# do-mpc/do-mpc

Measured on AMD Instinct MI355X. Metric: MPC steps/sec (make_step wall-time), industrial_poly robust multi-stage, higher is better.
Workload: dtype f64

## Files before the change

__graft_entry__.py:

```python
import os
import subprocess
import sys

ROOT = os.path.dirname(os.path.abspath(__file__))
if ROOT not in sys.path:
    sys.path.insert(0, ROOT)

PREBUILT = [
    ("oscillating_masses", {}),
    ("batch_reactor", {}),
    ("batch_reactor", {"n_horizon": 50}),
    ("CSTR", {}),
    ("CSTR", {"n_robust": 0, "collocation_deg": 3}),
    ("CSTR", {"track_sign": -3000.0}),
    ("industrial_poly", {}),
    ("industrial_poly", {"n_robust": 2, "uncertainty": "paired"}),
    ("industrial_poly", {"collocation_deg": 3, "collocation_ni": 2, "n_horizon": 6}),
    ("kinematic_bicycle", {}),
    ("dynamic_bicycle", {}),
    ("kite", {"n_horizon": 20}),
    ("rotating_masses", {}),
    ("CSTR", {"custom_rterm": "default_as_expression"}),
    ("CSTR", {"custom_rterm": "custom"}),
    ("oscillating_masses", {"custom_rterm": "custom"}),
    ("oscillating_masses_dae", {}),
    ("dip", {}),
    ("CSTR", {"n_robust": 0, "nl_cons_check_colloc_points": True}),
    ("dip", {"n_horizon": 40, "nl_cons_check_colloc_points": True}),
    ("CSTR", {"nl_cons_single_slack": True}),
    ("CSTR", {"nl_cons_single_slack": True, "n_robust": 2, "n_horizon": 8, "uncertainty": {"alpha": [1.0, 1.05, 0.95], "beta": [1.0]}}),
    ("CSTR", {"nl_cons_single_slack": True, "n_robust": 0, "nl_cons_check_colloc_points": True}),
    ("CSTR", {"open_loop": True, "uncertainty": {"alpha": [1.0, 1.05, 0.95], "beta": [1.0]}}),
    ("CSTR", {"open_loop": True, "n_robust": 2, "n_horizon": 6, "uncertainty": {"alpha": [1.0, 1.05], "beta": [1.0]}, "soft_T_R": False}),
    ("shape_family:s1", {}), ("shape_family:s2", {}), ("shape_family:s3", {}), ("shape_family:s4", {}), ("shape_family:s5", {}),
    ("shape_family:s6", {}), ("shape_family:s7", {}), ("shape_family:s8", {}), ("shape_family:s9", {}),
]

PREBUILT_BATCH = [
    ("industrial_poly", {}), ("industrial_poly", {"n_robust": 2, "uncertainty": "paired"}),
    ("oscillating_masses", {}), ("CSTR", {}), ("CSTR", {"n_robust": 0, "collocation_deg": 3}), ("batch_reactor", {}), ("batch_reactor", {"n_horizon": 50}),
    ("rotating_masses", {}),
]
PREBUILT_BATCH_MHE = [("rotating_masses", "build_mhe", {}, {}), ("rotating_masses", "build_mhe_w", {"process_noise": True}, {}),
                      ("rotating_masses", "build_mhe_w", {"process_noise": True}, {"scaling": "MHE_W_SCALING"})]


PREBUILT_DEFS = [("CSTR", {}, "DOMPC_FORCE_DENSE=1"), ("batch_reactor", {}, "DOMPC_FORCE_DENSE=1"),
                 ("CSTR", {}, "DOMPC_GJ_U=1e9"), ("industrial_poly", {}, "DOMPC_GJ_U=1e9"),
                 ("batch_reactor", {}, "DOMPC_REG_GJ=0"), ("batch_reactor", {}, "DOMPC_GJ_U=1e9"),
                 ("industrial_poly", {}, "DOMPC_QUAD=0"), ("CSTR", {}, "DOMPC_QUAD=0"), ("CSTR", {"n_horizon": 5, "n_robust": 0}, "DOMPC_QUAD=0")]


PREBUILT_SHARD = [
    ("CSTR", {}),
    ("industrial_poly", {"n_robust": 2, "uncertainty": "paired"}),
]


PREBUILT_MHE = [("rotating_masses", "build_mhe", {}, {}), ("rotating_masses", "build_mhe_w", {"process_noise": True}, {}),
                ("rotating_masses", "build_mhe_w", {"process_noise": True}, {"scaling": "MHE_W_SCALING"}),
                ("rotating_masses", "build_mhe", {"dae": True}, {}), ("rotating_masses", "build_mhe_w", {"process_noise": True, "dae": True}, {}),
                ("oscillating_masses", "build_mhe", {"estimation": True}, {}), ("oscillating_masses", "build_mhe", {"estimation": True, "dae": True}, {}),
                ("rotating_masses", "build_mhe_w", {"process_noise": True}, {"soft_limit": (-0.1, 0.01)}),
                ("rotating_masses", "build_mhe_w", {"process_noise": True}, {"soft_limit": (-0.1, 0.01), "nl_cons_single_slack": True}),
                ("rotating_masses", "build_mhe_w", {"process_noise": True, "input_meas_noise": False}, {})]


PREBUILT_ROUTE = [("oscillating_masses", "docstring", False, False), ("oscillating_masses", "tree", False, False),
                  ("industrial_poly", "tree", False, True), ("CSTR", "tree", False, True), ("batch_reactor", "tree", False, False),
                  ("oscillating_masses_dae", "tree", False, False), ("rotating_masses", "tree", False, False),
                  ("CSTR", "docstring", False, False), ("batch_reactor", "docstring", False, False), ("industrial_poly", "docstring", False, False),
                  ("oscillating_masses", None, True, False), ("CSTR", None, True, False), ("CSTR", "tree", True, False),
                  ("industrial_poly", None, True, False), ("industrial_poly", "tree", True, False), ("batch_reactor", None, True, False),
                  ("rotating_masses", None, True, False)]


def lowered_route_cases():
    from do_mpc_amd import controller
    from do_mpc_amd.examples import CASES
    tests = os.path.join(ROOT, "tests")
    if tests not in sys.path:
        sys.path.insert(0, tests)
    import route_cases as rc
    out = []
    orig = controller.HipIpmSolver
    controller.HipIpmSolver = _NoSolver
    try:
        for name, cost, rows, batch in PREBUILT_ROUTE:
            ex = CASES[name]
            mpc = rc.stopped_before_setup(lambda n: ex.build_mpc(ex.build_model()), name)
            mpc.prepare_nlp()
            if rows:
                rc.rows_at_three_nodes(mpc, name)
            if cost:
                rc.ADDED_COST[cost](mpc)
            mpc.create_nlp()
            out.append((f"{name} + {cost or ''}{' + rows' if rows else ''} (low-level route)", {}, mpc.generated_header, mpc.model_hash, batch))
    finally:
        controller.HipIpmSolver = orig
    return out


PREBUILT_PLANTS = ["oscillating_masses", "batch_reactor", "CSTR", "industrial_poly", "oscillating_masses_dae", "dip", "rotating_masses",
                   "triple_tank", "batch_reactor_lqr_dae", "batch_reactor_lqr_dae:build_dae_model"]
# ... 108 lines not shown
class _NoSolver:

    def __init__(self, *a, **k):
        pass


def lowered_models(which=None):
    from do_mpc_amd import controller
    from do_mpc_amd.examples import CASES
    out = []
    orig = controller.HipIpmSolver
    controller.HipIpmSolver = _NoSolver
    try:
        for name, kw in (PREBUILT if which is None else which):
            ex = CASES[name]
            mpc = ex.build_mpc(ex.build_model(), **kw)
            out.append((name, kw, mpc.generated_header, mpc.model_hash))
        if which is None:
            out += _lower_mhe(PREBUILT_MHE)
    finally:
        controller.HipIpmSolver = orig
    return out


def _lower_mhe(entries):
    from do_mpc_amd.examples import CASES
    out = []
    for name, builder, mkw, bkw in entries:
        ex = CASES[name]
        bkw = {k: (getattr(ex, v) if isinstance(v, str) else v) for k, v in bkw.items()}
        mhe = getattr(ex, builder)(ex.build_model(**mkw), **bkw)
        out.append((f"{name} ({builder})", {**mkw, **{k: "..." for k in bkw}}, mhe._mpc.generated_header, mhe._mpc.model_hash))
    return out


def lowered_mhe(entries):
    from do_mpc_amd import controller
    orig = controller.HipIpmSolver
    controller.HipIpmSolver = _NoSolver
    try:
        return _lower_mhe(entries)
    finally:
        controller.HipIpmSolver = orig


def build() -> None:
    from do_mpc_amd import build as nb
    import do_mpc_amd
    from concurrent.futures import ThreadPoolExecutor
    lib = nb.runtime_library()
    print("[build] runtime:", lib)
    jobs = [(name, kw, header, h, False, False) for name, kw, header, h in lowered_models()]
    jobs += [(name, kw, header, h, True, False) for name, kw, header, h in lowered_models(PREBUILT_SHARD)]
    jobs += [(name, kw, header, h, False, True) for name, kw, header, h in lowered_models(PREBUILT_BATCH)]
    jobs += [(name, kw, header, h, False, True) for name, kw, header, h in lowered_mhe(PREBUILT_BATCH_MHE)]
    route = lowered_route_cases()
    jobs += [(name, kw, header, h, False, False) for name, kw, header, h, _ in route]
    jobs += [(name, kw, header, h, False, True) for name, kw, header, h, batch in route if batch]
    with ThreadPoolExecutor(max_workers=max(1, min(len(jobs), (os.cpu_count() or 2) - 1))) as pool:
        outs = list(pool.map(lambda j: nb.model_code_object(j[2], j[3], shard=j[4], batch_only=j[5]), jobs))
    for (name, kw, _, _, shard, batch), co in zip(jobs, outs):
        print(f"[build] {name} {kw}{' (tree sharding)' if shard else ''}{' (batch only)' if batch else ''}: {co}")
    for name, kw, defs in PREBUILT_DEFS:
        saved = os.environ.get("DOMPC_DEFS")
        os.environ["DOMPC_DEFS"] = defs
        try:
            for _, _, header, h in lowered_models([(name, kw)]):
                print(f"[build] {name} {kw} [{defs}]: {nb.model_code_object(header, h)}")
        finally:
            if saved is None:
                del os.environ["DOMPC_DEFS"]
            else:
                os.environ["DOMPC_DEFS"] = saved
    from do_mpc_amd.examples import CASES
    from do_mpc_amd.simulator import Simulator
    for name in PREBUILT_PLANTS:
        case, _, builder = name.partition(":")
        hdr = Simulator(getattr(CASES[case], builder or "build_model")())._lower()
        co = nb.plant_code_object(hdr, hdr.rsplit('PLANT_MODEL_HASH "', 1)[1].split('"')[0])
        print(f"[build] plant {name}: {co}")
    failed = []
    for entry in PREBUILT_EKF:
        try:
            for name, kw, hdr, h in lowered_ekf([entry]):
                print(f"[build] filter {name} {kw}: {nb.ekf_code_object(hdr, h)}")
        except Exception as e:
            failed.append(entry)
            print(f"[build] filter {entry[0]} {entry[1]}: FAILED\n{e}")
    for entry in PREBUILT_EKF_DAE:
        try:
            for name, hdr, h in lowered_ekf_dae([entry]):
                print(f"[build] filter of a model with algebraic states '{name}': {nb.ekf_code_object(hdr, h)}")
        except Exception as e:
            failed.append(entry)
            print(f"[build] filter of a model with algebraic states '{entry}': FAILED\n{e}")
    failed_lqr = []
    for entry in PREBUILT_LQR:
        try:
            for label, hdr, h in lowered_lqr([entry]):
                print(f"[build] LQR design {label}: {nb.lqr_code_object(hdr, h)}")
        except Exception as e:
            failed_lqr.append(entry)
            print(f"[build] LQR design {entry}: FAILED\n{e}")
    failed_ampc = []
    for entry in PREBUILT_AMPC:
        try:
            for label, hdr, h in lowered_ampc([entry]):
                print(f"[build] approximate MPC network {label}: {nb.ampc_code_object(hdr, h)}")
        except Exception as e:
            failed_ampc.append(entry)
            print(f"[build] approximate MPC network {entry}: FAILED\n{e}")
    failed_asmpc = []
    for entry in PREBUILT_ASMPC:
        try:
            for label, hdr, h in lowered_asmpc([entry]):
                print(f"[build] sensitivity-based MPC law {label}: {nb.asmpc_code_object(hdr, h)}")
        except Exception as e:
            failed_asmpc.append(entry)
            print(f"[build] sensitivity-based MPC law {entry}: FAILED\n{e}")
    mk = os.path.join(ROOT, "oracle", "Makefile")
    if os.path.exists(mk):
        subprocess.run(["make", "-C", os.path.join(ROOT, "oracle")], check=True)
    if failed:
        raise RuntimeError(f"extended Kalman filter code objects that could not be built: {failed}")
    if failed_lqr:
        raise RuntimeError(f"LQR design code objects that could not be built: {failed_lqr}")
# ... 74 lines not shown
```

do_mpc_amd/csrc/dompc_device.hip:

```cpp
#ifndef DOMPC_HOST_EMU
#include <hip/hip_runtime.h>
#define DOMPC_CONSTANT_TABLES 1
#define DOMPC_FN __device__ static inline
#define DOMPC_CONST __device__ static constexpr
#define DOMPC_DEV __device__
#define DOMPC_HD __host__ __device__
#else
#include <stdlib.h>
#define DOMPC_FN static inline
#define DOMPC_CONST static const
#define DOMPC_DEV
#define DOMPC_HD
#endif

#ifndef DOMPC_LB
#define DOMPC_LB 2
#endif
#ifndef DOMPC_SRC_DIGEST
#define DOMPC_SRC_DIGEST 0ULL
#endif

#include DOMPC_MODEL_HEADER
#include "dompc_kernel.h"

namespace dompc {
DOMPC_HD inline void model_info(const int32_t* in, int64_t* out) {
  WsLayout L = ws_layout(in[0], in[1], in[2], in[3], in[4]);
  out[0] = NX; out[1] = NU; out[2] = NP; out[3] = NTVP; out[4] = NE; out[5] = NSE;
  out[6] = DEG; out[7] = NI; out[8] = M;
  out[9] = L.total;
  out[10] = SWEEP_BLOCK;
  out[11] = (int64_t)sizeof(KArgs);
  out[12] = RED_MAX; out[13] = ASM_N; out[14] = CUT1; out[15] = CUT2;
  out[16] = DOMPC_SHARD;
  out[17] = EL_SIZE;
  out[19] = QUAD_EDGE ? 4 : 1;
  out[18] = (int64_t)DOMPC_SRC_DIGEST;
#ifndef DOMPC_HOST_EMU
  out[20] = r16::ENABLED ? 1 : 0;
#else
  out[20] = 0;
#endif
}
}

#ifndef DOMPC_HOST_EMU
extern "C" __global__ void dompc_model_info_kernel(const int32_t* in, int64_t* out, char* hash) {
  if (threadIdx.x == 0 && blockIdx.x == 0) {
    dompc::model_info(in, out);
    const char h[] = DOMPC_MODEL_HASH;
    for (int i = 0; i < (int)sizeof(h); ++i) hash[i] = h[i];
  }
}

#ifndef DOMPC_MAXBLOCK
#define DOMPC_MAXBLOCK 256
#endif
extern "C" __global__ void __launch_bounds__(DOMPC_BLOCK_CONST ? DOMPC_BLOCK_CONST : DOMPC_MAXBLOCK, DOMPC_LB) dompc_solve_kernel(dompc::KArgs A) {
  using namespace dompc;
  const int POOL = A.pool_doubles;
  if (threadIdx.x < 32) lds_prof[threadIdx.x] = 0;
  if (threadIdx.x < 8) lds_flags[threadIdx.x] = 0;
  for (int i = threadIdx.x; i < POOL; i += DOMPC_BDIM) lds_pool[i] = (i >= A.lds_fill_lo && i < A.lds_fill_hi) ? A.lds_fill : 0.0;
  for (int i = threadIdx.x; i < 2 * MAX_FILTER; i += DOMPC_BDIM) lds_filt[i] = 0.0;
  __syncthreads();
  const bool wide = dompc::WIDE_OK && (A.mode == 0 && A.wide > 1);
  const int slot = slot_of_block(A);
  if (wide && slot >= A.batch) return;
  Thr T = make_thr(A);
  T.kp = (const void*)__builtin_amdgcn_kernarg_segment_ptr();
  if (wide && A.mode != 1) dompc::xcd_census(T);
  if (A.mode == 1) {
    const int bq = __builtin_amdgcn_readfirstlane((int)blockIdx.x);
    const int sq = slot_of_block(A);
    if (bq < A.batch) dompc::debug_newton(T, A, bq, sq);
    return;
  }
  bool first = true;
  while (true) {
    int b;
    if (wide) {
      if (!first) break;
      b = slot;
    } else {
      if (threadIdx.x == 0) lds_b = atomicAdd(A.work_counter, 1);
      __syncthreads();
      b = lds_b;
      __syncthreads();
      if (b >= A.batch) break;
    }
    first = false;
    if (A.mode == 2) dompc::sweep_problem(T, A, b, slot);
    else dompc::solve_problem(T, A, b, slot);
  }
}
// ... 65 lines not shown
```

do_mpc_amd/csrc/dompc_driver.h:

```cpp

DOMPC_DEV inline int epsg_off(const KArgs& A) { return A.node_eps_off[0]; }
DOMPC_DEV inline int epsg_n(const KArgs& A) { return A.n_opt_x - A.node_eps_off[0]; }
DOMPC_DEV inline void epsg_grad(const Thr& T, const Prob& Q) {
  const KArgs& A = *Q.A;
  const int o = epsg_off(A), nv = epsg_n(A);
  for (int j = T.tid; j < nv; j += T.nt) {
    double g = 0.0, r = 0.0;
    for (int e = 0; e < A.n_edges; ++e) {
      const int q = j - (A.node_eps_off[A.edge_parent[e]] - o);
      if (q < 0 || q >= NSE) continue;
      g += Q.sf * DOMPC_EPS_PEN[q];
      const double* yd = Q.lam + A.edge_row0[e] + NW + NX;
      for (int i = 0; i < NE; ++i)
        if (nl_slack(i) == q) r -= yd[i] * Q.sgn[e * NE1 + i];
    }
    Q.gf[o + j] = g;
    Q.rd[o + j] = g + r - Q.zl[o + j] + Q.zu[o + j];
  }
  T.sync();
}
DOMPC_DEV inline double epsg_rowsum(const Prob& Q, int j, const double* v, const double* v0) {
  const KArgs& A = *Q.A;
  const int o = epsg_off(A);
  double t = 0.0;
// ... 8 lines not shown
}
DOMPC_DEV inline void epsg_residual(const Thr& T, const Prob& Q, const double* v, int j1) {
  const KArgs& A = *Q.A;
  const int o = epsg_off(A);
  for (int e = T.tid; e < A.n_edges; e += T.nt) {
    const int jo = A.node_eps_off[A.edge_parent[e]] - o;
    const int r0 = A.edge_row0[e] + NW + NX;
    for (int i = 0; i < NE; ++i) {
      const int q = nl_slack(i);
      if (q < 0) continue;
      const double ve = v ? v[jo + q] : ((jo + q == j1) ? 1.0 : 0.0);
      Q.c[r0 + i] = Q.ct[r0 + i] - ve * Q.sgn[e * NE1 + i];
    }
  }
  T.sync();
}

DOMPC_DEV inline void solve_problem(const Thr& T, const KArgs& A, int b, int slot0) {
  const dompc_options& O = A.opt;
  int slot = slot0;
  Prob Q = make_prob(A, slot, A.p + (int64_t)b * A.n_opt_p);
  const double* x0 = A.x0 + (int64_t)b * A.n_opt_x;
  const int nX = A.n_opt_x, nSl = A.n_edges * NE;
  int status = 2, it = 0, n_reg = 0, n_ls_fail = 0, n_sweeps = 0, n_trials = 0, n_soc = 0;

  double cnt[2] = {0.0, 0.0};
  bool singular0;
  {
    double fr[1] = {0.0};
    for (int d = T.tid; d < A.n_dummy; d += T.nt) {
      const int g = A.dummy_idx[d];
      if (!(A.lbx[g] > -INFINITY) && !(A.ubx[g] < INFINITY)) fr[0] += 1.0;
    }
    const int ops[1] = {R_SUM};
    wg_reduce(T, fr, ops);
    singular0 = fr[0] > 0.0;
  }
  for (int g = T.tid; g < nX; g += T.nt) {
    double l = A.lbx[g], u = A.ubx[g];
    if (l > -INFINITY) l -= fmin(O.constr_viol_tol, O.bound_relax_factor * fmax(1.0, fabs(l)));
    if (u < INFINITY) u += fmin(O.constr_viol_tol, O.bound_relax_factor * fmax(1.0, fabs(u)));
    double xv = x0[g];
    const bool hl = l > -INFINITY, hu = u < INFINITY;
    double pl = hl ? O.bound_push * fmax(1.0, fabs(l)) : 0.0;
    double pu = hu ? O.bound_push * fmax(1.0, fabs(u)) : 0.0;
    if (hl && hu) { pl = fmin(pl, O.bound_frac * (u - l)); pu = fmin(pu, O.bound_frac * (u - l)); }
    if (hl) xv = fmax(xv, l + pl);
    if (hu) xv = fmin(xv, u - pu);
    Q.lb_own[g] = l; Q.ub_own[g] = u; Q.x[g] = xv;
    Q.zl[g] = hl ? 1.0 : 0.0; Q.zu[g] = hu ? 1.0 : 0.0;
    if (sh_cnt(A, mk_x(A, g))) cnt[0] += (hl ? 1.0 : 0.0) + (hu ? 1.0 : 0.0);
  }
  for (int r = T.tid; r < A.n_g; r += T.nt) Q.lam[r] = 0.0;
  T.sync();
  for (int d = T.tid; d < A.n_dummy; d += T.nt) {
    const int g = A.dummy_idx[d];
    if (singular0) continue;
    if (sh_cnt(A, mk_x(A, g))) cnt[0] -= (Q.lb_own[g] > -INFINITY ? 1.0 : 0.0) + (Q.ub_own[g] < INFINITY ? 1.0 : 0.0);
    Q.x[g] = fmin(fmax(x0[g], A.lbx[g]), A.ubx[g]);
    Q.lb_own[g] = -INFINITY; Q.ub_own[g] = INFINITY; Q.zl[g] = 0.0; Q.zu[g] = 0.0;
  }
  T.sync();
  if (A.lb_sh) {
    for (int g = T.tid; g < nX; g += T.nt) { A.lb_sh[g] = Q.lb_own[g]; A.ub_sh[g] = Q.ub_own[g]; }
    T.sync();
  }
  auto init_slacks = [&](bool rescale) {
    for (int e = T.tid; e < A.n_edges; e += T.nt) {
      for (int i = 0; i < NE; ++i) { Q.s[e * NE1 + i] = 0.0; if (!rescale) Q.sgn[e * NE1 + i] = 1.0; }
      if (DENSE_EDGE) dae_edge_f(Q, e, Q.x, Q.s, Q.ct); else eval_edge_f(Q, e, Q.x, Q.s, Q.ct);
      for (int i = 0; i < NE; ++i) {
        const int row = A.edge_row0[e] + NW + NX + i, si = e * NE1 + i;
        double l = A.lbg[row], u = A.ubg[row];
        if (l > -INFINITY) l -= fmin(O.constr_viol_tol, O.bound_relax_factor * fmax(1.0, fabs(l)));
        if (u < INFINITY) u += fmin(O.constr_viol_tol, O.bound_relax_factor * fmax(1.0, fabs(u)));
        l *= Q.sgn[si]; u *= Q.sgn[si];
        const bool hl = l > -INFINITY, hu = u < INFINITY;
        double pl = hl ? O.bound_push * fmax(1.0, fabs(l)) : 0.0;
        double pu = hu ? O.bound_push * fmax(1.0, fabs(u)) : 0.0;
        if (hl && hu) { pl = fmin(pl, O.bound_frac * (u - l)); pu = fmin(pu, O.bound_frac * (u - l)); }
        double sv = Q.ct[row];
        if (hl) sv = fmax(sv, l + pl);
        if (hu) sv = fmin(sv, u - pu);
        Q.s[si] = sv; Q.sl[si] = l; Q.su[si] = u;
        Q.zsl[si] = hl ? 1.0 : 0.0; Q.zsu[si] = hu ? 1.0 : 0.0;
        if (!rescale && sh_cnt(A, mk_e(A, e))) cnt[1] += (hl ? 1.0 : 0.0) + (hu ? 1.0 : 0.0);
      }
    }
    T.sync();
  };
  if (NE > 0) init_slacks(false);
  {
    const int ops[2] = {R_SUM, R_SUM};
    wg_reduce(T, cnt, ops);
  }
  const double n_bounds = cnt[0] + cnt[1];
  const double n_dual = (double)(A.n_g - DOMPC_XROW_MASKED) + n_bounds;

  double mu = O.mu_init;
  Q.sf = 1.0;
  long long c_sweep = 0, c_bwd = 0, c_fwd = 0, c_ls = 0, c_meas = 0, c_ftb = 0, c_acc = 0, c_t = 0; const long long c_start = prof_clock();
  unsigned g_sweep = 0, g_bwd = 0, g_fwd = 0, g_ls = 0, g_meas = 0, g_ftb = 0, g_acc = 0, g_t = 0; const unsigned g_start = T.gen;
  if (T.tid == 0) T.fset(6, abort_requested(A));
  auto delta_after = [&](double last) { return last == 0.0 ? O.delta_w_0 : fmax(O.delta_w_min, O.kappa_w_minus * last); };
  const bool ls_init = (NE == 0 || (!EPS_GLOBAL && !FREE_ROOT)) && O.constr_mult_init_max > 0.0;
  auto ls_slacks = [&]() {
// ... 157 lines not shown
    bad = run_sweep(T, Q, b, slot, mu, 0, singular0 ? delta_after(0.0) : 0.0);
    ++n_sweeps;
  }
  const double mu_min = fmin(O.tol, O.compl_inf_tol * Q.sf) / (O.kappa_eps + 1.0);
  double tau = fmax(O.tau_min, 1.0 - mu);
  if (KAPPA_D != 0.0) Q.mu = mu;
  Errs E = measure(T, Q, nullptr);
  const double theta0 = E.theta;
  const double theta_max = 1e4 * fmax(1.0, theta0), theta_min = 1e-4 * fmax(1.0, theta0);
  double bar_sum;
  {
    double bs[1] = {0.0};
    LogAcc La{1.0, 0, 0};
    double lin = 0.0;
    double x_[DOMPC_FW], l_[DOMPC_FW], u2_[DOMPC_FW];
#define L_(u, g) x_[u] = Q.x[g]; l_[u] = Q.lb[g]; u2_[u] = Q.ub[g];
#define B_(u, g)                                                       \
    if (sh_cnt(A, mk_x(A, g))) {                                       \
      if (l_[u] > -INFINITY) logacc_add(La, x_[u] - l_[u]);            \
      if (u2_[u] < INFINITY) logacc_add(La, u2_[u] - x_[u]);           \
      if (KAPPA_D != 0.0) { const double os_ = one_sided(l_[u], u2_[u]); lin += os_ > 0.0 ? x_[u] - l_[u] : (os_ < 0.0 ? u2_[u] - x_[u] : 0.0); } \
    }
    DOMPC_FOR4(nX, L_, B_)
#undef L_
#undef B_
    for (int g = T.tid; g < nSl; g += T.nt) {
      if (!sh_cnt(A, mk_e(A, g / NE1))) continue;
      const int si = (g / NE1) * NE1 + g % NE1;
      if (Q.sl[si] > -INFINITY) logacc_add(La, Q.s[si] - Q.sl[si]);
      if (Q.su[si] < INFINITY) logacc_add(La, Q.su[si] - Q.s[si]);
      if (KAPPA_D != 0.0) { const double os_ = one_sided(Q.sl[si], Q.su[si]); lin += os_ > 0.0 ? Q.s[si] - Q.sl[si] : (os_ < 0.0 ? Q.su[si] - Q.s[si] : 0.0); }
    }
    bs[0] = -logacc_value(La);
    if (KAPPA_D != 0.0) bs[0] += KAPPA_D * lin;
    const int ops[1] = {R_SUM};
    wg_reduce(T, bs, ops);
    bar_sum = bs[0];
  }
  int n_filt = 0;
  double delta_last = 0.0;
  int acc_count = 0;
  const double s_max = 100.0;
  double E0 = 0.0;
  int wd_count = 0, wd_iter = 0, n_watchdog = 0;
  bool in_wd = false, wd_resume = false;
  double wd_theta = 0.0, wd_phi = 0.0, wd_dphi = 0.0, wd_alpha = 0.0, wd_amax = 0.0, wd_az = 0.0, wd_delta = 0.0, wd_delta_last = 0.0, wd_bar = 0.0;
  Errs wd_E = E;
  double delta = 0.0, a_max = 1.0, a_z = 1.0, dphi = 0.0;
  for (int g = T.tid; g < nX; g += T.nt) { Q.xt[g] = Q.x[g]; Q.zlt[g] = Q.zl[g]; Q.zut[g] = Q.zu[g]; }
  for (int g = T.tid; g < A.n_g; g += T.nt) Q.lamt[g] = Q.lam[g];
  for (int g = T.tid; g < nSl; g += T.nt) { Q.st[g] = Q.s[g]; Q.zslt[g] = Q.zsl[g]; Q.zsut[g] = Q.zsu[g]; }
  T.sync();
  Comp Cp{-INFINITY, INFINITY, 0.0};

  while (true) {
    bool skip_first = false;
    if (wd_resume) {
      for (int g = T.tid; g < nX; g += T.nt) { Q.x[g] = Q.x_wd[g]; Q.zl[g] = Q.zl_wd[g]; Q.zu[g] = Q.zu_wd[g]; Q.dx[g] = Q.dx_sv[g]; }
      for (int g = T.tid; g < A.n_g; g += T.nt) { Q.lam[g] = Q.lam_wd[g]; Q.dlam[g] = Q.dlam_sv[g]; }
      for (int g = T.tid; g < nSl; g += T.nt) { Q.s[g] = Q.s_wd[g]; Q.zsl[g] = Q.zsl_wd[g]; Q.zsu[g] = Q.zsu_wd[g]; Q.ds[g] = Q.ds_sv[g]; }
      T.sync();
      E = wd_E; bar_sum = wd_bar; delta = wd_delta; delta_last = wd_delta_last; a_max = wd_amax; a_z = wd_az; dphi = wd_dphi;
      wd_resume = false;
      skip_first = true;
    } else {
    if (bad) { if (in_wd) { bad = 0; wd_resume = true; in_wd = false; wd_count = 0; continue; } status = 3; break; }
    if (T.fget(6)) { status = 6; break; }
    if (((WIDE_OK && T.nwg > 1) || sh_on(A)) && T.fget(7)) { status = 5; break; }
    const double sd = fmax(s_max, (E.sum_y + E.C.sum_z) / fmax(1.0, n_dual)) / s_max;
    const double sc = fmax(s_max, E.C.sum_z / fmax(1.0, n_bounds)) / s_max;
    const double e_c0 = comp_err(E.C, 0.0);
    E0 = fmax(E.e_d / sd, fmax(E.e_p, e_c0 / sc));
    if (!(E0 == E0) || !(E.obj == E.obj)) { if (in_wd) { wd_resume = true; in_wd = false; wd_count = 0; continue; } status = 4; break; }
    if (E0 <= O.tol && E.e_d <= O.dual_inf_tol && E.e_p <= O.constr_viol_tol && e_c0 <= O.compl_inf_tol) {
      status = 0; break;
    }
    if (E0 <= O.acceptable_tol) {
      if (++acc_count >= O.acceptable_iter) { status = 1; break; }
    } else acc_count = 0;
    if (it >= O.max_iter) { status = 2; break; }

    const double mu_before = mu;
    while (true) {
      const double Emu = fmax(E.e_d / sd, fmax(E.e_p, comp_err(E.C, mu) / sc));
      if (Emu <= O.kappa_eps * mu && mu > mu_min) {
        mu = fmax(mu_min, fmin(O.kappa_mu * mu, pow(mu, O.theta_mu)));
        tau = fmax(O.tau_min, 1.0 - mu);
        n_filt = 0;
        in_wd = false; wd_count = 0;
      } else break;
    }
    if (mu != mu_before) {
      if (QUAD_FWD && forward_adjoint(Q, mu) && !Q.lu_ok) {
        ++n_sweeps;
        if (run_sweep(T, Q, b, slot, mu, 4, Q.dsw)) { if (in_wd) { wd_resume = true; in_wd = false; wd_count = 0; continue; } status = 3; break; }
      } else {
        refresh_mu(T, Q, mu - mu_before);
        Q.rp_mu = mu;
      }
    }

    delta = 0.0;
    bool first_try = true, dir_ok = true, recs_dirty = false;
    while (true) {
      c_t = prof_clock(); g_t = T.gen;
      int fail = (singular0 && delta == 0.0) ? 1 : run_backward(T, Q, b, slot, mu, delta);
      if (EPS_GLOBAL && !fail) {
        run_forward(T, Q, b, slot, mu, delta);
        fail = epsg_build(delta);
        recs_dirty = true;
      }
      c_bwd += prof_clock() - c_t; g_bwd += T.gen - g_t;
      if (!fail) break;
      if (delta == 0.0) {
        delta = delta_after(delta_last);
      } else {
        delta *= (delta_last == 0.0 && first_try) ? O.kappa_w_plus_bar : O.kappa_w_plus;
        first_try = false;
        if (delta > O.delta_w_max) { dir_ok = false; break; }
      }
      if ((NW > 0 && delta != Q.dsw) || (EPS_GLOBAL && recs_dirty)) {
        ++n_sweeps;
        if (run_sweep(T, Q, b, slot, mu, 0, delta)) { dir_ok = false; break; }
        recs_dirty = false;
      }
    }
    if (!dir_ok) { if (in_wd) { wd_resume = true; in_wd = false; wd_count = 0; continue; } status = 3; break; }
    if (delta > 0.0) { delta_last = delta; ++n_reg; }
    c_t = prof_clock(); g_t = T.gen;
    if (EPS_GLOBAL) { if (epsg_apply(delta, Q.dlam_e)) { if (in_wd) { wd_resume = true; in_wd = false; wd_count = 0; continue; } status = 3; break; } }
    else run_forward(T, Q, b, slot, mu, delta);
    c_fwd += prof_clock() - c_t; g_fwd += T.gen - g_t;

    c_t = prof_clock(); g_t = T.gen;
    double r5[5];
    run_step_rules(T, Q, b, slot, mu, r5);
    a_max = (r5[0] > tau) ? tau / r5[0] : 1.0; dphi = r5[2];
    a_z = (r5[1] > tau) ? tau / r5[1] : 1.0;
    c_ftb += prof_clock() - c_t; g_ftb += T.gen - g_t;
    }
    auto step_rules = [&](double (&r5)[5]) { run_step_rules(T, Q, b, slot, mu, r5); };
    const double theta = E.theta;
    const double phi = E.obj + mu * bar_sum;

    c_t = prof_clock(); g_t = T.gen;
    const double gamma_theta = 1e-5, gamma_phi = 1e-8, eta_phi = 1e-8, s_theta = 1.1, s_phi = 2.3, gamma_alpha = 0.05;
    const double kappa_soc = 0.99;
    double a_min;
    if (dphi < 0.0 && theta <= theta_min)
      a_min = (theta > 0.0) ? gamma_alpha * fmin(gamma_theta, fmin(gamma_phi * theta / (-dphi),
                                                                    pow(theta, s_theta) / pow(-dphi, s_phi)))
                            : gamma_alpha * gamma_theta;
    else if (dphi < 0.0) a_min = gamma_alpha * fmin(gamma_theta, gamma_phi * theta / (-dphi));
    else a_min = gamma_alpha * gamma_theta;
    a_min = fmax(a_min, 1e-14);
    auto eval_trial = [&](double al, double az, double& obj_o, double& th_o, double& bar_o) {
      run_eval_trial(T, Q, b, slot, al, az, mu, obj_o, th_o, bar_o, Cp);
      ++n_trials;
    };
    auto acceptable_ref = [&](double th_, double ph_, double al, bool& armijo_case, double theta, double phi, double dphi) -> bool {
      armijo_case = false;
      bool ok = (ph_ == ph_) && (th_ == th_) && fabs(ph_) < INFINITY && th_ <= theta_max;
      if (ok) {
        for (int q = 0; q < n_filt; ++q)
          if (th_ >= T.filt[2 * q] && ph_ >= T.filt[2 * q + 1]) { ok = false; break; }
      }
      if (ok) {
        const bool switching = dphi < 0.0 && al * pow(-dphi, s_phi) > pow(theta, s_theta);
        const double eps_m = 10.0 * 2.220446049250313e-16 * fabs(phi);
        if (theta <= theta_min && switching) {
          armijo_case = true;
          ok = (ph_ - phi - eps_m <= eta_phi * al * dphi);
        } else {
          ok = (th_ <= (1.0 - gamma_theta) * theta) || (ph_ - phi - eps_m <= -gamma_phi * theta);
        }
      }
      return ok;
    };
    auto acceptable = [&](double th_, double ph_, double al, bool& armijo_case) -> bool { return acceptable_ref(th_, ph_, al, armijo_case, theta, phi, dphi); };
    auto soc_residual = [&](double al) {
      double c_[DOMPC_FW], ct_[DOMPC_FW];
#define L_(u, g) c_[u] = Q.c[g]; ct_[u] = Q.ct[g];
#define B_(u, g) if (mk_g(A, g)) Q.c[g] = al * c_[u] + ct_[u];
      DOMPC_FOR4(A.n_g, L_, B_)
#undef L_
#undef B_
      T.sync();
    };
    auto keep_direction = [&](bool restore) {
      for (int g = T.tid; g < nX; g += T.nt) { if (restore) Q.dx[g] = Q.dx_sv[g]; else Q.dx_sv[g] = Q.dx[g]; }
      for (int g = T.tid; g < A.n_g; g += T.nt) { if (restore) Q.dlam[g] = Q.dlam_sv[g]; else Q.dlam_sv[g] = Q.dlam[g]; }
      for (int g = T.tid; g < nSl; g += T.nt) { if (restore) Q.ds[g] = Q.ds_sv[g]; else Q.ds_sv[g] = Q.ds[g]; }
      T.sync();
    };
    double alpha = skip_first ? 0.5 * a_max : a_max;
    bool accepted = false, armijo_used = false, stale = false;
    double th_t = 0.0, obj_t = 0.0, bar_t = bar_sum;
    int n_ls = skip_first ? 1 : 0;
    bool wd_done = false, wd_augment_ref = false, wd_no_augment = false;
    if (O.watchdog_shortened_iter_trigger > 0 && !in_wd && !skip_first && wd_count >= O.watchdog_shortened_iter_trigger) {
      in_wd = true; wd_iter = 0; ++n_watchdog;
      for (int g = T.tid; g < nX; g += T.nt) { Q.x_wd[g] = Q.x[g]; Q.zl_wd[g] = Q.zl[g]; Q.zu_wd[g] = Q.zu[g]; Q.dx_sv[g] = Q.dx[g]; }
      for (int g = T.tid; g < A.n_g; g += T.nt) { Q.lam_wd[g] = Q.lam[g]; Q.dlam_sv[g] = Q.dlam[g]; }
      for (int g = T.tid; g < nSl; g += T.nt) { Q.s_wd[g] = Q.s[g]; Q.zsl_wd[g] = Q.zsl[g]; Q.zsu_wd[g] = Q.zsu[g]; Q.ds_sv[g] = Q.ds[g]; }
      T.sync();
      wd_E = E; wd_bar = bar_sum; wd_delta = delta; wd_delta_last = delta_last; wd_amax = a_max; wd_az = a_z;
      wd_theta = theta; wd_phi = phi; wd_dphi = dphi; wd_alpha = a_max;
    }
    if (in_wd) {
      eval_trial(alpha, a_z, obj_t, th_t, bar_t);
// ... 34 lines not shown
          double obj_s = 0.0, th_s = 0.0, bar_s = 0.0;
          eval_trial(a_s, az_s, obj_s, th_s, bar_s);
          bool arm_s = false;
          if (acceptable(th_s, obj_s + mu * bar_s, a_s, arm_s)) {
            accepted = true; armijo_used = arm_s; soc_ok = true;
            alpha = a_s;
            a_z = az_s;
            obj_t = obj_s; th_t = th_s; bar_t = bar_s;
            break;
          }
          if (!(th_s <= kappa_soc * th_old)) break;
          th_old = th_s;
          soc_residual(a_s);
        }
        if (soc_ok) break;
        keep_direction(true);
        stale = true;
      }
      if (!(alpha * 0.5 >= a_min)) break;
      alpha *= 0.5;
      ++n_ls;
    }
    if (bad) { if (in_wd) { bad = 0; wd_resume = true; in_wd = false; wd_count = 0; continue; } status = 3; break; }
    if (!accepted && stale) eval_trial(alpha, a_z, obj_t, th_t, bar_t);
    if (!wd_done) wd_count = n_ls > 0 ? wd_count + 1 : 0;
    if (!accepted) {
      ++n_ls_fail;
      n_filt = 0;
    } else if (!armijo_used && !wd_no_augment) {
      if (T.ltid == 0) {
        int q = n_filt < MAX_FILTER ? n_filt : MAX_FILTER - 1;
        T.filt[2 * q] = (1.0 - gamma_theta) * (wd_augment_ref ? wd_theta : theta);
        T.filt[2 * q + 1] = (wd_augment_ref ? wd_phi : phi) - gamma_phi * (wd_augment_ref ? wd_theta : theta);
      }
      if (n_filt < MAX_FILTER) ++n_filt;
      T.lsync();
    }
    bar_sum = bar_t;
    c_ls += prof_clock() - c_t; g_ls += T.gen - g_t;
    c_t = prof_clock(); g_t = T.gen;
    prob_flip(Q); slot = Q.slot;
    if (A.trace && b == 0 && T.tid == 0 && it < A.trace_cap) {
      double* tr = A.trace + 8 * it;
      tr[0] = it; tr[1] = mu; tr[2] = E0; tr[3] = E.e_p; tr[4] = E.e_d; tr[5] = accepted ? alpha : -alpha;
      tr[6] = delta; tr[7] = E.obj / Q.sf;
    }
    if (T.tid == 0) T.fset(6, abort_requested(A));
    c_acc += prof_clock() - c_t; g_acc += T.gen - g_t;
    ++it;
    c_t = prof_clock(); g_t = T.gen; bad = run_sweep(T, Q, b, slot, mu, 0, singular0 ? delta_after(delta_last) : 0.0); c_sweep += prof_clock() - c_t; g_sweep += T.gen - g_t;
    ++n_sweeps;
    if (EPS_GLOBAL) epsg_grad(T, Q);
    if (KAPPA_D != 0.0) Q.mu = mu;
    c_t = prof_clock(); g_t = T.gen; E = measure(T, Q, &Cp); c_meas += prof_clock() - c_t; g_meas += T.gen - g_t;
  }

  if (slot & SLOT_PARITY) {
    for (int g = T.tid; g < nX; g += T.nt) { Q.xt[g] = Q.x[g]; Q.zlt[g] = Q.zl[g]; Q.zut[g] = Q.zu[g]; }
    for (int g = T.tid; g < A.n_g; g += T.nt) Q.lamt[g] = Q.lam[g];
    for (int g = T.tid; g < nSl; g += T.nt) { Q.st[g] = Q.s[g]; Q.zslt[g] = Q.zsl[g]; Q.zsut[g] = Q.zsu[g]; }
    T.sync();
    prob_flip(Q); slot = Q.slot;
  }
  if (A.trace && b == 0 && T.tid == 0 && A.trace_cap > 8) { double* tr = A.trace + 8 * (A.trace_cap - 1); tr[0] = (double)c_sweep; tr[1] = (double)c_bwd; tr[2] = (double)c_fwd; tr[3] = (double)c_ls; tr[4] = (double)c_meas; tr[5] = (double)(prof_clock() - c_start); tr[6] = (double)c_ftb; tr[7] = (double)c_acc; if (T.prof) { double* t2 = A.trace + 8 * (A.trace_cap - 2); for (int i = 0; i < 8; ++i) t2[i] = (double)T.prof[i]; double* t3 = A.trace + 8 * (A.trace_cap - 3); for (int i = 0; i < 8; ++i) t3[i] = (double)T.prof[8 + i]; double* t4 = A.trace + 8 * (A.trace_cap - 4); for (int i = 0; i < 8; ++i) t4[i] = (double)T.prof[16 + i]; if (A.trace_cap > 12) { double* t5 = A.trace + 8 * (A.trace_cap - 5); for (int i = 0; i < 8; ++i) t5[i] = (double)T.prof[24 + i]; double* t6 = A.trace + 8 * (A.trace_cap - 6); t6[0] = g_sweep; t6[1] = g_bwd; t6[2] = g_fwd; t6[3] = g_ls; t6[4] = g_meas; t6[5] = T.gen - g_start; t6[6] = g_ftb; t6[7] = g_acc; } } }
  const double isf = 1.0 / Q.sf;
  if (A.x_out) for (int g = T.tid; g < nX; g += T.nt) A.x_out[(int64_t)b * nX + g] = sh_cnt(A, mk_x(A, g)) ? Q.x[g] : 0.0;
  if (A.lam_x_out) for (int g = T.tid; g < nX; g += T.nt) A.lam_x_out[(int64_t)b * nX + g] = sh_cnt(A, mk_x(A, g)) ? (Q.zu[g] - Q.zl[g]) * isf : 0.0;
  if (A.lam_g_out) for (int r = T.tid; r < A.n_g; r += T.nt) A.lam_g_out[(int64_t)b * A.n_g + r] = sh_cnt(A, mk_g(A, r)) ? Q.lam[r] * isf : 0.0;
  if (A.lam_g_out && NE > 0) {
    T.sync();
    for (int g = T.tid; g < nSl; g += T.nt) {
      const int e = g / NE1, i = g % NE1;
      if (!sh_cnt(A, mk_e(A, e))) continue;
      const int row = A.edge_row0[e] + NW + NX + i;
      A.lam_g_out[(int64_t)b * A.n_g + row] = Q.lam[row] * Q.sgn[e * NE1 + i] * isf;
    }
  }
  if (A.g_out) {
    for (int r = T.tid; r < A.n_g; r += T.nt) A.g_out[(int64_t)b * A.n_g + r] = sh_cnt(A, mk_g(A, r)) ? Q.c[r] : 0.0;
    T.sync();
    for (int g = T.tid; g < nSl; g += T.nt) {
      const int e = g / NE1, i = g % NE1;
      if (!sh_cnt(A, mk_e(A, e))) continue;
      const int row = A.edge_row0[e] + NW + NX + i;
      A.g_out[(int64_t)b * A.n_g + row] = (Q.c[row] + Q.s[e * NE1 + i]) / Q.sgn[e * NE1 + i];
    }
  }
  if (T.tid == 0) {
    if (A.f_out) A.f_out[b] = E.obj * isf;
    if (A.stats) {
      dompc_stats& S = A.stats[b];
      S.success = (status == 0 || status == 1) ? 1 : 0;
      S.status = status; S.iter_count = it; S.n_reg = n_reg; S.n_ls_fail = n_ls_fail; S.n_sweeps = n_sweeps; S.n_trials = n_trials; S.n_soc = n_soc; S.n_watchdog = n_watchdog; S.reserved0 = 0;
      S.mu = mu; S.obj = E.obj * isf; S.inf_pr = E.e_p; S.inf_du = E.e_d; S.inf_compl = comp_err(E.C, 0.0);
      S.obj_scaling = Q.sf; S.t_wall_total = 0.0;
    }
  }
  T.sync();
}

DOMPC_DEV inline void newton_slack_setup(const Thr& T, const KArgs& A, Prob& Q, int at_solution, double mu, bool reduce, double tol) {
  const dompc_options& O = A.opt;
  if (NE > 0) {
    for (int e = T.tid; e < A.n_edges; e += T.nt) {
      for (int i = 0; i < NE; ++i) { Q.s[e * NE1 + i] = 0.0; Q.sgn[e * NE1 + i] = 1.0; }
      if (DENSE_EDGE) dae_edge_f(Q, e, Q.x, Q.s, Q.ct); else eval_edge_f(Q, e, Q.x, Q.s, Q.ct);
      for (int i = 0; i < NE; ++i) {
        const int row = A.edge_row0[e] + NW + NX + i, si = e * NE1 + i;
        double l = A.lbg[row], u = A.ubg[row];
        double sv = Q.ct[row];
        if (reduce && l != u) {
          const bool act = fabs(sv - l) <= tol || fabs(sv - u) <= tol;
          l = act ? sv : -INFINITY;
          u = act ? sv : INFINITY;
        }
        const bool hl = l > -INFINITY, hu = u < INFINITY;
        double pl = hl ? O.bound_push * fmax(1.0, fabs(l)) : 0.0;
        double pu = hu ? O.bound_push * fmax(1.0, fabs(u)) : 0.0;
        if (hl && hu) { pl = fmin(pl, O.bound_frac * (u - l)); pu = fmin(pu, O.bound_frac * (u - l)); }
        if (at_solution) {
          const double lr = hl ? l - fmin(O.constr_viol_tol, O.bound_relax_factor * fmax(1.0, fabs(l))) : l;
          const double ur = hu ? u + fmin(O.constr_viol_tol, O.bound_relax_factor * fmax(1.0, fabs(u))) : u;
          const double tiny = 1e-12 * fmax(1.0, fabs(sv));
          if (hl) sv = fmax(sv, lr + tiny);
          if (hu) sv = fmin(sv, ur - tiny);
          Q.s[si] = sv; Q.sl[si] = lr; Q.su[si] = ur;
          Q.zsl[si] = hl ? mu / (sv - lr) : 0.0; Q.zsu[si] = hu ? mu / (ur - sv) : 0.0;
          continue;
        }
        if (hl) sv = fmax(sv, l + pl);
        if (hu) sv = fmin(sv, u - pu);
        Q.s[si] = sv; Q.sl[si] = l; Q.su[si] = u;
        Q.zsl[si] = hl ? 1.0 : 0.0; Q.zsu[si] = hu ? 1.0 : 0.0;
      }
    }
    T.sync();
  }
}

DOMPC_DEV inline void debug_newton(const Thr& T, const KArgs& A, int b = 0, int slot = 0) {
  Prob Q = make_prob(A, slot, A.p + (int64_t)b * A.n_opt_p);
  const int nX = A.n_opt_x;
  for (int g = T.tid; g < nX; g += T.nt) {
    Q.x[g] = A.x0[g]; Q.lb[g] = A.lbx[g]; Q.ub[g] = A.ubx[g];
    Q.zl[g] = A.dbg_zl[g]; Q.zu[g] = A.dbg_zu[g];
  }
  for (int r = T.tid; r < A.n_g; r += T.nt) Q.lam[r] = A.dbg_lam[r];
  T.sync();
  newton_slack_setup(T, A, Q, A.dbg_at_solution, A.dbg_mu, false, 0.0);
  Q.sf = 1.0;
  run_sweep(T, Q, b, slot, A.dbg_mu, 0, A.dbg_delta);
  const int fail = run_backward(T, Q, b, slot, A.dbg_mu, A.dbg_delta);
  run_forward(T, Q, b, slot, A.dbg_mu, A.dbg_delta);
  for (int g = T.tid; g < nX; g += T.nt) {
    A.dbg_dx[(int64_t)b * nX + g] = fail ? NAN : Q.dx[g];
    A.dbg_rd[(int64_t)b * nX + g] = Q.rd[g];
  }
  for (int r = T.tid; r < A.n_g; r += T.nt) {
    A.dbg_dlam[(int64_t)b * A.n_g + r] = Q.dlam[r];
    A.dbg_c[(int64_t)b * A.n_g + r] = Q.c[r];
  }
  T.sync();
}

enum { SENS_REDUCE = 1 };
DOMPC_DEV inline void sens_newton(const Thr& T, const KArgs& A, int b, int slot) {
  const dompc_options& O = A.opt;
  const int q = b / A.sn_R, r = b % A.sn_R;
  Prob Q = make_prob(A, slot, A.p + (int64_t)b * A.n_opt_p);
  const int nX = A.n_opt_x;
  const double* xin = A.sn_x + (int64_t)q * nX;
  const double* lin = A.sn_lam + (int64_t)q * A.n_g;
  const double mu = A.sn_mu[q];
  const bool reduce = (A.sn_flags & SENS_REDUCE) != 0;
  const double tol = A.sn_tol;
  double bad[1] = {(mu > 0.0 && mu < INFINITY) ? 0.0 : 1.0};
  for (int g = T.tid; g < nX; g += T.nt) {
    const double xv = xin[g], l0 = A.lbx[g], u0 = A.ubx[g];
    const bool hl = l0 > -INFINITY, hu = u0 < INFINITY;
    double lr = hl ? l0 - fmin(O.constr_viol_tol, O.bound_relax_factor * fmax(1.0, fabs(l0))) : l0;
    double ur = hu ? u0 + fmin(O.constr_viol_tol, O.bound_relax_factor * fmax(1.0, fabs(u0))) : u0;
    const double dl = hl ? xv - lr : 1.0, du = hu ? ur - xv : 1.0;
    if (!(dl > 0.0) || !(du > 0.0)) bad[0] = 1.0;
    double zl = hl ? mu / dl : 0.0, zu = hu ? mu / du : 0.0;
    if (reduce) {
      const bool lo = fabs(xv - l0) <= tol, up = fabs(xv - u0) <= tol;
      if (!lo && !up) { zl = 0.0; zu = 0.0; lr = -INFINITY; ur = INFINITY; }
      if (lo) zl = fmax(zl, 1e3);
      if (up) zu = fmax(zu, 1e3);
    }
    Q.x[g] = xv; Q.lb[g] = lr; Q.ub[g] = ur; Q.zl[g] = zl; Q.zu[g] = zu;
  }
  for (int i = T.tid; i < A.n_g; i += T.nt) Q.lam[i] = lin[i];
  {
    const int ops[1] = {R_MAX};
    wg_reduce(T, bad, ops);
  }
  T.sync();
  double* D = A.sn_D + (int64_t)b * A.sn_nsel;
  int fail = bad[0] != 0.0;
  if (!fail) {
    newton_slack_setup(T, A, Q, 1, mu, reduce, tol);
    Q.sf = 1.0;
    run_sweep(T, Q, b, slot, mu, 0, 0.0);
    fail = run_backward(T, Q, b, slot, mu, 0.0);
    run_forward(T, Q, b, slot, mu, 0.0);
  }
  for (int i = T.tid; i < A.sn_nsel; i += T.nt) {
    const double v = fail ? NAN : Q.dx[A.sn_sel[i]];
    D[i] = v;
    if (!(fabs(v) < INFINITY)) A.sn_ok[q] = 0;
  }
  if (fail && T.tid == 0) A.sn_ok[q] = 0;
  if (r == 0) {
    double m[1] = {0.0};
    if (!fail) {
      for (int g = T.tid; g < nX; g += T.nt) Q.dx_sv[g] = 1.0;
      T.sync();
      for (int i = T.tid; i < A.n_dummy; i += T.nt) Q.dx_sv[A.dummy_idx[i]] = 0.0;
      T.sync();
      for (int g = T.tid; g < nX; g += T.nt) if (Q.dx_sv[g] != 0.0) m[0] = fmax(m[0], fabs(Q.dx[g]));
    }
    const int ops[1] = {R_MAX};
    wg_reduce(T, m, ops);
    if (T.tid == 0) A.sn_res[q] = fail ? NAN : m[0];
  }
  T.sync();
}

DOMPC_HD inline double sens_step(int lin, double fd_step, double pj) { return (lin ? 1.0 : fd_step) * fmax(1.0, fabs(pj)); }
DOMPC_DEV inline void sens_prep_item(const KArgs& A, int64_t it) {
  const int np = A.n_opt_p;
  const int64_t b = it / np;
  const int k = (int)(it % np), q = (int)(b / A.sn_R), r = (int)(b % A.sn_R);
  double v = A.sn_p[(int64_t)q * np + k];
  const int j = A.sn_rows[2 * r], kind = A.sn_rows[2 * r + 1];
  if (kind != 0 && j == k) {
    const double h = sens_step(kind == 1, A.sn_fd_step, v);
    v = kind < 0 ? v - h : v + h;
  }
  A.sn_prow[it] = v;
  if (k == 0 && r == 0) A.sn_ok[q] = 1;
}
DOMPC_DEV inline void sens_finish_item(const KArgs& A, int64_t it) {
  const int nc = A.sn_ncols, ns = A.sn_nsel;
  const int c = (int)(it % nc), i = (int)((it / nc) % ns), q = (int)(it / ((int64_t)nc * ns));
  const int j = A.sn_cols[3 * c], ip = A.sn_cols[3 * c + 1], im = A.sn_cols[3 * c + 2];
  const double* D = A.sn_D + (int64_t)q * A.sn_R * ns;
  const double h = sens_step(im < 0, A.sn_fd_step, A.sn_p[(int64_t)q * A.n_opt_p + j]);
  const double v = im < 0 ? (D[(int64_t)ip * ns + i] - D[i]) / h : (D[(int64_t)ip * ns + i] - D[(int64_t)im * ns + i]) / (2.0 * h);
  A.sn_S[it] = A.sn_ok[q] ? v : NAN;
}

constexpr int SWEEP_BLOCK = NX * NA + NX + NA * NA + NA;

DOMPC_DEV inline void sweep_problem(const Thr& T, const KArgs& A, int b, int slot) {
  Prob Q = make_prob(A, slot, A.p + (int64_t)b * A.n_opt_p);
  const int nX = A.n_opt_x;
  const double* xin = A.sw_x + (int64_t)b * nX;
  const double* lin = A.sw_lam + (int64_t)b * A.n_g;
  for (int g = T.tid; g < nX; g += T.nt) {
    Q.x[g] = xin[g]; Q.lb[g] = -INFINITY; Q.ub[g] = INFINITY; Q.zl[g] = 0.0; Q.zu[g] = 0.0;
  }
  for (int r = T.tid; r < A.n_g; r += T.nt) Q.lam[r] = lin[r];
  for (int g = T.tid; g < A.n_edges * NE; g += T.nt) {
    const int si = (g / NE1) * NE1 + g % NE1;
    Q.s[si] = 0.0; Q.sl[si] = -INFINITY; Q.su[si] = INFINITY; Q.zsl[si] = 0.0; Q.zsu[si] = 0.0; Q.sgn[si] = 1.0;
  }
  T.sync();
  Q.sf = 1.0;
  run_sweep(T, Q, b, slot, 0.0);
  double* gout = A.sw_g + (int64_t)b * A.n_g;
  for (int r = T.tid; r < A.n_g; r += T.nt) gout[r] = Q.c[r];
  double* bl = A.sw_blocks + (int64_t)b * A.n_edges * SWEEP_BLOCK;
  for (int it = T.tid; A.sw_blocks && it < A.n_edges * SWEEP_BLOCK; it += T.nt) {
    const int e = it / SWEEP_BLOCK, i = it % SWEEP_BLOCK;
    const double* S_ = Q.ES(e);
    double v;
    if (i < NX * NA) v = S_[ES_AB + i];
    else if (i < NX * NA + NX) v = S_[ES_CV + i - NX * NA];
    else if (i < NX * NA + NX + NA * NA) v = S_[ES_QT + symi((i - NX * NA - NX) / NA, (i - NX * NA - NX) % NA, NA)];
    else v = S_[ES_QV + i - NX * NA - NX - NA * NA];
    bl[it] = v;
  }
  T.sync();
}
```

do_mpc_amd/csrc/dompc_edge.h:

```cpp

template <bool SPLIT>
DOMPC_DEV inline double eval_edge_f_t(const Prob& Q, int e, const double* xv, const double* sv, double* cv, int part) {
  constexpr int REST = NI * DEG;
  const KArgs& A = *Q.A;
  const int n = A.edge_parent[e], cn = A.edge_child[e], k = A.edge_level[e];
  const double* xn = xv + A.node_x_off[n];
  const double* un = xv + A.node_u_off[n];
  const double* xc = xv + A.node_x_off[cn];
  const double* w = xv + A.edge_w_off[e];
  const double* pp = Q.P + A.p_off_p + A.edge_pidx[e] * NP;
  const double* tvp = Q.P + A.p_off_tvp + k * NTVP;
  const int row0 = A.edge_row0[e];
  const double om = A.edge_omega[e] * Q.sf;
  double f[NX];
  if (M == 0) {
    dompc_dyn_f(xn, un, nullptr, tvp, pp, f);
    double rl[NX];
    for (int a = 0; a < NX; ++a) rl[a] = f[a] - xc[a];
    for (int a = 0; a < NX; ++a) cv[row0 + a] = rl[a];
  } else {
    (void)REST;
    for (int i = 0; i < NI; ++i) {
      const double* xi0 = (i == 0) ? xn : w + slot_of(i, 0) * NX;
      const int rb = row0 + i * (DEG + 1) * NX;
      for (int j = 1; j <= DEG; ++j) {
        if (SPLIT && part != i * DEG + (j - 1)) continue;
        const double* xij = w + slot_of(i, j) * NX;
        dompc_dyn_f(xij, un, nullptr, tvp, pp, f);
        double rl[NX];
#pragma unroll
        for (int a = 0; a < NX; ++a) {
          double xp = DOMPC_C[0 * (DEG + 1) + j] * xi0[a];
          for (int r = 1; r <= DEG; ++r) xp += DOMPC_C[r * (DEG + 1) + j] * w[slot_of(i, r) * NX + a];
          rl[a] = f[a] - xp;
        }
#pragma unroll
        for (int a = 0; a < NX; ++a) cv[rb + (j - 1) * NX + a] = rl[a];
      }
      if (SPLIT && part != REST) continue;
      const double* xnext = w + next_slot(i) * NX;
      double rl[NX];
#pragma unroll
      for (int a = 0; a < NX; ++a) {
        double xf = DOMPC_D[0] * xi0[a];
        for (int r = 1; r <= DEG; ++r) xf += DOMPC_D[r] * w[slot_of(i, r) * NX + a];
        rl[a] = xnext[a] - xf;
      }
#pragma unroll
      for (int a = 0; a < NX; ++a) cv[rb + DEG * NX + a] = rl[a];
    }
    if (SPLIT && part != REST) return 0.0;
    double rl[NX];
#pragma unroll
    for (int a = 0; a < NX; ++a) rl[a] = w[(M - 1) * NX + a] - xc[a];
#pragma unroll
    for (int a = 0; a < NX; ++a) cv[row0 + NW + a] = rl[a];
  }
  double obj = om * lterm_f_e(Q, e, xn, un, nullptr, tvp, pp);
  if (k == A.N - 1) obj += om * mterm_f_e(Q, e, xc, Q.P + A.p_off_tvp + (k + 1) * NTVP, pp);
  if (RT_CUSTOM) obj += edge_rterm_f(Q, e, xv);
  if (NE > 0) {
    double d[NE1];
    nlcons_f_e(Q, e, xn, un, nullptr, tvp, pp, d);
    const double* eps = (NSE > 0) ? xv + A.node_eps_off[n] : nullptr;
    for (int i = 0; i < NE; ++i) {
      if (nl_slack(i) >= 0) d[i] -= eps[nl_slack(i)];
      d[i] *= Q.sgn[e * NE1 + i];
      cv[row0 + NW + NX + i] = d[i] - sv[e * NE1 + i];
    }
    for (int q = 0; q < NSE; ++q) obj += Q.sf * DOMPC_EPS_PEN[q] * eps[q];
  }
  return obj;
}
DOMPC_PHASE double eval_edge_f(const Prob& Q, int e, const double* xv, const double* sv, double* cv) { return eval_edge_f_t<false>(Q, e, xv, sv, cv, -1); }

DOMPC_DEV inline const double* uprev_ptr(const Prob& Q, int n, const double* xv, double* tmp) {
  const KArgs& A = *Q.A;
  const int pn = A.node_parent[n];
  if (pn >= 0) return xv + A.node_u_off[pn];
  for (int i = 0; i < NU; ++i) tmp[i] = Q.P[A.p_off_uprev + i] / DOMPC_SU[i];
  return tmp;
}
DOMPC_DEV inline double node_rweight(const Prob& Q, int n) {
  const KArgs& A = *Q.A;
  const int cc = A.node_child_count[n];
  return cc > 0 ? cc * A.edge_omega[A.node_child_start[n]] * Q.sf : 0.0;
}
DOMPC_DEV inline double node_rterm_f(const Prob& Q, int n, const double* xv) {
  const KArgs& A = *Q.A;
  if (RT_CUSTOM) return 0.0;
  if (A.node_u_off[n] < 0) return 0.0;
  double tmp[NU];
  const double* up = uprev_ptr(Q, n, xv, tmp);
  const double* u = xv + A.node_u_off[n];
  const double rw = node_rweight(Q, n);
  double v = 0.0;
  for (int i = 0; i < NU; ++i) v += rw * DOMPC_RTERM[i] * (u[i] - up[i]) * (u[i] - up[i]);
  return v;
}

DOMPC_DEV inline double edge_rterm_f(const Prob& Q, int e, const double* xv) {
  const KArgs& A = *Q.A;
  const int n = A.edge_parent[e];
  double tmp[NU > 0 ? NU : 1];
  const double* up = uprev_ptr(Q, n, xv, tmp);
  return A.edge_omega[e] * Q.sf * dompc_rterm_f(xv + A.node_x_off[n], xv + A.node_u_off[n], up, Q.P + A.p_off_tvp + A.edge_level[e] * NTVP,
                                                Q.P + A.p_off_p + A.edge_pidx[e] * NP);
}
DOMPC_DEV inline void edge_rterm_eval(const Prob& Q, int e, ldsd* dst) {
  const KArgs& A = *Q.A;
  const int n = A.edge_parent[e];
  const double om = A.edge_omega[e] * Q.sf, omh = (Q.soc & 2) ? 0.0 : om;
  double tmp[NU > 0 ? NU : 1], out[RT_LEN > 0 ? RT_LEN : 1];
  const double* up = uprev_ptr(Q, n, Q.x, tmp);
  dompc_rterm(Q.x + A.node_x_off[n], Q.x + A.node_u_off[n], up, Q.P + A.p_off_tvp + A.edge_level[e] * NTVP,
              Q.P + A.p_off_p + A.edge_pidx[e] * NP, out, out + 1, out + 1 + NR);
  for (int i = 0; i < 1 + NR; ++i) dst[i] = om * out[i];
  for (int i = 0; i < NR_T; ++i) dst[1 + NR + i] = omh * out[1 + NR + i];
}
DOMPC_DEV inline void edge_rterm_store(const ldsd* src, double* S_, int lane, int GS) {
  for (int i = lane; i < NU; i += GS) S_[ES_RTUP + i] = src[1 + NA + i];
  for (int i = lane; i < NR_T; i += GS) S_[ES_RTH + i] = src[1 + NR + i];
}

constexpr int NC = NW + NA + 1;
static_assert(NW <= 128, "collocation block larger than 128 unknowns per edge is not supported (pivot key / used mask of the in-LDS elimination)");
static_assert(NI >= 2 || NW <= 64, "single finite element: at most 64 unknowns per edge (one extended column per lane of the register-resident elimination)");
static_assert(!DENSE_EDGE || NW <= 64, "dense edge path (algebraic states, rows at the collocation points, estimators): at most 64 unknowns per edge (one row per lane in its pivot search)");
constexpr int MX_LD = (NI == 1) ? NA + 1 : NC;
constexpr int MX_W = (NI == 1) ? 0 : NW;
#ifndef DOMPC_HOST_EMU
constexpr bool TILE_CONDENSE = (NI == 1) && (DEG >= 1) && (NA <= 16) && !DENSE_EDGE;
#else
constexpr bool TILE_CONDENSE = false;
#endif
constexpr int EL_MX = 0;
constexpr int GJ_LDS = (NI == 1 && DEG >= 1) ? 4 * (((DEG * NX + 3) / 4) * 4) + 256 : 0;
constexpr int EL_T1 = EL_MX + (NW * MX_LD > GJ_LDS ? NW * MX_LD : GJ_LDS);
constexpr int EL_T0 = EL_T1 + (TILE_CONDENSE ? NW : NW * NA);
// ... 236 lines not shown
```

do_mpc_amd/csrc/dompc_factor.h:

```cpp

#ifndef DOMPC_HOST_EMU
#ifndef DOMPC_GJ_U
#define DOMPC_GJ_U 0.01
#endif
constexpr int GJ_R = DEG * NX, GJ_RP = ((GJ_R + 3) / 4) * 4, GJ_NRHS = NA + 1;
constexpr int GJ_NC = GJ_RP + GJ_NRHS + GJ_R;
constexpr bool MFMA_GJ = (NI == 1) && (DEG >= 1) && !DENSE_EDGE && (GJ_RP <= 32) && (GJ_NC <= 64);
constexpr int GJ_MT = (GJ_RP + 15) / 16, GJ_NT = (GJ_NC + 15) / 16;
static_assert(!MFMA_GJ || GJ_RP * 4 + 256 <= EL_T1 - EL_MX, "the panel buffer and the dual-residual row share the W | w0 region of the edge working set");

constexpr bool GJ_PACK = (GJ_MT == 2) && (GJ_RP == 20) && (GJ_NT <= 4);
constexpr int GJ_MTF = GJ_PACK ? 1 : GJ_MT;

struct GjCol { int kind, sl, b; };
__device__ inline GjCol gj_col(int ni, int lc) {
  constexpr int R = GJ_R, RP = GJ_RP, NRHS = GJ_NRHS;
  const int col = 16 * ni + lc;
  GjCol c{4, 0, 0};
  if (col < R) { c.kind = 0; c.sl = col / NX; c.b = col - c.sl * NX; }
  else if (col < RP) { c.kind = 4; c.b = col; }
  else if (col < RP + NA) { c.kind = 1; c.b = col - RP; }
  else if (col == RP + NA) { c.kind = 2; }
  else if (col < RP + NRHS + R) { c.kind = 3; c.b = col - (RP + NRHS); }
  return c;
// ... 370 lines not shown
        }
        if (lane == lk && !(best > 1e-300)) badl = 1;
#ifndef DOMPC_HOST_EMU
        pr = __builtin_amdgcn_readlane(pr, lk);
#endif
#pragma unroll
        for (int q = 0; q < CPX; ++q) {
          const double t = bc[q][kk];
          double nk = t;
#pragma unroll
          for (int r = kk + 1; r < R; ++r) {
            const bool hit = (r == pr);
            nk = hit ? bc[q][r] : nk;
            bc[q][r] = hit ? t : bc[q][r];
          }
          bc[q][kk] = nk;
        }
      } else {
        double m = 0.0;
#pragma unroll
        for (int r = kk + 1; r < R; ++r) m = fmax(m, fabs(bc[qk][r]));
        const double akk = fabs(bc[qk][kk]);
        if (lane == lk && !(akk >= GJ_U * m && akk > 1e-300)) badl = 1;
      }
      double f[RA];
#pragma unroll
      for (int r = 0; r < R; ++r) f[r] = lane_bcast(bc[qk][r], lk);
      const double pinv = fast_rcp((fabs(f[kk]) > 1e-300) ? f[kk] : 1.0);
#pragma unroll
      for (int q = 0; q < CPX; ++q) {
        const double prow = bc[q][kk] * pinv;
#pragma unroll
        for (int r = 0; r < R; ++r)
          if (r != kk) bc[q][r] = fma(-f[r], prow, bc[q][r]);
        bc[q][kk] = prow;
      }
    }
#ifndef DOMPC_HOST_EMU
    return __ballot(badl) != 0ull;
#else
    return badl;
#endif
  };
  if (MODE != 1) fetch_cols();
  auto dual_pieces = [&](auto col_dot) {
#pragma unroll
    for (int q = 0; q < CPX; ++q) {
      const int cx = lane + q * GS;
      double t = col_dot(q, cx);
      if (cx < R) {
        t -= DOMPC_D[cx / NX + 1] * Ld[EL_T0 + R + cx % NX];
        const int gi = woff + cx;
        const double xv = vx[q][0], l = vx[q][1], u = vx[q][2], zl_ = vx[q][3], zu_ = vx[q][4];
        Q.gf[gi] = 0.0;
        Q.rd[gi] = t - zl_ + zu_;
        Ld[EL_RW + cx] = t + bar_grad(xv, l, u, mu, !(Q.soc & 2));
        Ld[EL_BB + cx] = bar_grad(xv, l, u, 1.0);
        Ld[EL_SG + cx] = sigma_of(xv, l, u, zl_, zu_);
      } else if (cx < R + NA) {
        const int yb = cx - R;
        if (yb < NX) t -= DOMPC_D[0] * Ld[EL_T0 + R + yb];
        Ld[EL_RY + yb] = t;
      }
    }
    for (int a = lane; a < NX; a += GS) {
      const int col = R + a, gi = woff + col;
      const double t = Ld[EL_T0 + R + a] + (GS > 1 ? nu_a : nu_e[a]);
      double xv, l, u, zl_, zu_;
      if (GS > 1) { xv = ex[0]; l = ex[1]; u = ex[2]; zl_ = ex[3]; zu_ = ex[4]; }
      else { xv = Q.x[gi]; l = Q.lb[gi]; u = Q.ub[gi]; zl_ = Q.zl[gi]; zu_ = Q.zu[gi]; }
      Q.gf[gi] = 0.0;
      Q.rd[gi] = t - zl_ + zu_;
      Ld[EL_RW + col] = t + bar_grad(xv, l, u, mu, !(Q.soc & 2));
      Ld[EL_BB + col] = bar_grad(xv, l, u, 1.0);
      Ld[EL_SG + col] = sigma_of(xv, l, u, zl_, zu_);
    }
  };
  if (act && MODE == 0) {
    build_cols();
    dual_pieces([&](int q, int) {
      double t = 0.0;
#pragma unroll
      for (int r = 0; r < R; ++r) t += bc[q][r] * Ld[EL_T0 + r];
      return t;
    });
  }
#ifndef DOMPC_HOST_EMU
  if constexpr (MODE == 1) {
    __builtin_amdgcn_fence(__ATOMIC_ACQ_REL, "wavefront");
    __builtin_amdgcn_wave_barrier();
    if (edge_factor_mfma(Q, e, lane, Ld, [&](const ldsd* du) {
          dual_pieces([&](int, int cx) {
            const int c_ = cx < R ? cx : (cx < R + NA ? GJ_RP + (cx - R) : 0);
            return (double)du[c_] + (double)du[64 + c_] + (double)du[128 + c_] + (double)du[192 + c_];
          });
        })) return 2;
    {
      __builtin_amdgcn_fence(__ATOMIC_ACQ_REL, "wavefront");
      __builtin_amdgcn_wave_barrier();
      for (int it = lane; it < NX * NRHS; it += GS) {
        const int a_ = it / NRHS, c = it % NRHS;
        double t = (c == NA) ? -Ld[EL_T1 + R + a_] : ((c == a_) ? DOMPC_D[0] : 0.0);
#pragma unroll
        for (int s_ = 1; s_ <= DEG; ++s_) t += DOMPC_D[s_] * Ld[EL_MX + ((s_ - 1) * NX + a_) * MX_LD + MX_W + c];
        Ld[EL_MX + (R + a_) * MX_LD + MX_W + c] = t;
      }
      return 0;
    }
  } else if constexpr (MODE == 2) {
    build_cols();
    if (eliminate(true)) fail = 1;
  } else
#endif
  if (act) {
    if (eliminate(false)) {
      fetch_cols();
      build_cols();
      if (eliminate(true)) fail = 1;
    }
  }
  if (act) {
#pragma unroll
    for (int q = 0; q < CPX; ++q) {
      const int cx = lane + q * GS;
// ... 312 lines not shown
          const double* pt = mo + MO_PT + p * PT_STRIDE;
          double xp = DOMPC_C[0 * (DEG + 1) + j] * xi0[a];
          for (int r = 1; r <= DEG; ++r) xp += DOMPC_C[r * (DEG + 1) + j] * w[slot_of(i, r) * NX + a];
          const double res = Q.soc ? Q.c[row0 + row] : pt[a] - xp;
          gp_res[q2] = res;
          Mr[NW + NA] = res;
          for (int b = 0; b < NX; ++b) Mr[sl * NX + b] += pt[NX + a * NA + b];
          for (int b = 0; b < NU; ++b) Mr[NW + NX + b] = pt[NX + a * NA + NX + b];
          for (int r = 0; r <= DEG; ++r) {
            const double cr = DOMPC_C[r * (DEG + 1) + j];
            if (i == 0 && r == 0) Mr[NW + a] -= cr;
            else Mr[slot_of(i, r) * NX + a] -= cr;
          }
        } else {
          const int ns_ = next_slot(i);
          double xf = DOMPC_D[0] * xi0[a];
          for (int r = 1; r <= DEG; ++r) xf += DOMPC_D[r] * w[slot_of(i, r) * NX + a];
          const double res = Q.soc ? Q.c[row0 + row] : w[ns_ * NX + a] - xf;
          gp_res[q2] = res;
          Mr[NW + NA] = res;
          Mr[ns_ * NX + a] += 1.0;
          for (int r = 0; r <= DEG; ++r) {
            if (i == 0 && r == 0) Mr[NW + a] -= DOMPC_D[0];
            else Mr[slot_of(i, r) * NX + a] -= DOMPC_D[r];
          }
        }
      }
    }
    T.gsync();
    if (act) {
#pragma unroll
      for (int q = 0; q < G_WPL; ++q) {
        const int col = lane + q * GS;
        if (col >= NW) continue;
        double t = 0.0;
#pragma unroll 6
        for (int r = 0; r < NW; ++r) t += Ld[EL_MX + r * NC + col] * Ld[EL_T0 + r];
        if (col >= (M - 1) * NX) t += nu_e[col - (M - 1) * NX];
        const double xv = gp_x[q], l = gp_l[q], u = gp_u[q];
        gp_x[q] = t - gp_zl[q] + gp_zu[q];
        Ld[EL_RW + col] = t + bar_grad(xv, l, u, mu, !(Q.soc & 2));
        Ld[EL_BB + col] = bar_grad(xv, l, u, 1.0);
        Ld[EL_SG + col] = sigma_of(xv, l, u, gp_zl[q], gp_zu[q]);
      }
      for (int b = lane; b < NA; b += GS) {
        double t = 0.0;
#pragma unroll 6
        for (int r = 0; r < NW; ++r) t += Ld[EL_MX + r * NC + NW + b] * Ld[EL_T0 + r];
        Ld[EL_RY + b] = t;
      }
#pragma unroll
      for (int q = 0; q < G_WPL; ++q) {
        const int col = lane + q * GS;
        if (col < NW) { Q.gf[woff + col] = 0.0; Q.rd[woff + col] = gp_x[q]; }
      }
      if (!Q.soc) {
#pragma unroll
        for (int q2 = 0; q2 < G_RWL; ++q2) {
          const int it = lane + q2 * GS;
          if (it < G_ROWS) Q.c[row0 + it] = gp_res[q2];
        }
#pragma unroll
        for (int q = 0; q < G_XPL; ++q) {
          const int a = lane + q * GS;
          if (a < NX) Q.c[row0 + NW + a] = gp_ce[q];
        }
      }
    }
    T.gsync();
    DOMPC_PH(1)
    bool gj_done = false;
#ifndef DOMPC_HOST_EMU
#ifndef DOMPC_REG_GJ
#define DOMPC_REG_GJ 1
#endif
    if constexpr ((DOMPC_REG_GJ != 0) && NC <= 64 && NW <= 40 && NW > NX) {
      if (GS == 64) {
        constexpr int GJ_STEPS = NW - NX;
        constexpr int EL_ROWS = (DEG + 1) * NX;
        const int cc_ = lane < NC ? lane : 0;
        double col[NW1];
#pragma unroll
        for (int r = 0; r < NW; ++r) col[r] = act ? Ld[EL_MX + r * NC + cc_] : 1.0;
        int bad = 0;
#pragma unroll
        for (int kk = 0; kk < GJ_STEPS; ++kk) {
          const int pos = kk % EL_ROWS;
          const int grp0 = kk - pos + (pos < DEG * NX ? 0 : DEG * NX);
          const int grp1 = kk - pos + (pos < DEG * NX ? DEG * NX : EL_ROWS);
          const int hi_ = pos < DEG * NX ? kk - pos + EL_ROWS : (kk - pos + 2 * EL_ROWS < NW ? kk - pos + 2 * EL_ROWS : NW);
          double f[NW1];
#pragma unroll
          for (int r = 0; r < NW; ++r) f[r] = (r >= grp0 && r < hi_) ? lane_bcast(col[r], kk) : 0.0;
          double m = 0.0;
#pragma unroll
          for (int r = 0; r < NW; ++r) if (r > kk && r < grp1) m = fmax(m, fabs(f[r]));
          const double akk = fabs(f[kk]);
          bad |= (int)!(akk >= DOMPC_GJ_U * m && akk > 1e-300);
          const double pinv = fast_rcp(akk > 1e-300 ? f[kk] : 1.0);
          const bool own = lane == kk;
          const double prow = own ? pinv : col[kk] * pinv;
#pragma unroll
          for (int r = 0; r < NW; ++r) if (r >= grp0 && r < hi_ && r != kk) col[r] = fma(-f[r], prow, own ? 0.0 : col[r]);
          col[kk] = prow;
        }
        if (!act) bad = 0;
        if (__builtin_amdgcn_readfirstlane(bad) == 0) {
// ... 435 lines not shown
```

do_mpc_amd/csrc/dompc_forward.h:

```cpp


#ifndef DOMPC_ADJ_MU
#define DOMPC_ADJ_MU 10.0
#endif
DOMPC_DEV inline bool forward_adjoint(const Prob& Q, double mu) {
  constexpr bool ok = NI == 1 && M > 0 && DEG > 0 && !DENSE_EDGE && !RT_CUSTOM && !FREE_ROOT && !EPS_GLOBAL;
  return ok && !sh_on(*Q.A) && !(Q.soc & 2) && mu > 0.0 && mu <= DOMPC_ADJ_MU * Q.A->opt.tol;
}
template <bool ADJ>
DOMPC_PHASE void riccati_forward_t(const Thr& T, const Prob& Q, double mu, double delta) {
  const KArgs& A = *Q.A;
  const int GS = T.gs, ng = T.nt / GS, gid = group_index(T.tid, GS), lane = T.tid % GS;
  ldsd* Ld = T.edge_lds + (int64_t)(T.ltid / GS) * EL_SIZE;
  constexpr int FW_K = NV * NA + NV, FW_AB = NX * NA + NX, FW_N = FW_K + 2 * FW_AB;
  constexpr int FW_PL = (FW_N + GS_C - 1) / GS_C;
  constexpr int RF_DX = 0, RF_DV = RF_DX + NA, RF_DY = RF_DV + NV, RF_DNU = RF_DY + NA, RF_DW = RF_DNU + NX,
                RF_RHS = RF_DW + NW1, RF_G = RF_RHS + NW1, RF_DXN = RF_G + NW1, RF_IN = RF_DXN + NA;
  static_assert(RF_IN + FW_N <= EL_SIZE, "forward working set must fit the per-group LDS region");
  static_assert(RF_IN + FW_N <= RF_EW, "the staged edge records start behind the step vectors and chain-step operands");
  long long pc0 = prof_clock();
#if DOMPC_PROFILE
#define DOMPC_PF(i) if (T.prof && T.tid == 0) { const long long pc1 = prof_clock(); T.prof[i] += pc1 - pc0; pc0 = pc1; }
#else
#define DOMPC_PF(i)
#endif
  (void)pc0;
  const int cl = A.chain_level < A.N ? A.chain_level : A.N;
#ifndef DOMPC_HOST_EMU
  const bool root_fused = cl >= 1 && !SHARD;
#else
  const bool root_fused = false;
#endif
  if (!root_fused) {
    if (T.tid == 0) {
      double* Nd = Q.ND(0);
      const int xo = A.node_x_off[0];
      if (FREE_ROOT) {
        for (int a = 0; a < NX; ++a) Q.dx[xo + a] = Nd[ND_DXT + a];
      } else {
        for (int a = 0; a < NX; ++a) { Nd[ND_DXT + a] = -Q.c[a]; Q.dx[xo + a] = -Q.c[a]; }
      }
      for (int a = NX; a < NA; ++a) Nd[ND_DXT + a] = 0.0;
    }
    T.sync();
  }
  auto node_step = [&](int n) {
    const double* Nd = Q.ND(n);
    if (root_fused && n == 0) {
      const int xo = A.node_x_off[0];
      for (int a = lane; a < NA; a += GS) {
        const double t = a < NX ? (FREE_ROOT ? Nd[ND_DXT + a] : -Q.c[a]) : 0.0;
        Ld[RF_DX + a] = t;
        if (!FREE_ROOT || a >= NX) Q.ND(0)[ND_DXT + a] = t;
        if (a < NX) Q.dx[xo + a] = t;
      }
    } else
    for (int a = lane; a < NA; a += GS) Ld[RF_DX + a] = Nd[ND_DXT + a];
    T.gsync();
    for (int i = lane; i < NV; i += GS) {
      double t = Nd[ND_KV + i];
#pragma unroll
      for (int a = 0; a < NA; ++a) t += Nd[ND_K + i * NA + a] * Ld[RF_DX + a];
      Ld[RF_DV + i] = t;
      if (i < NU) Q.dx[A.node_u_off[n] + i] = t;
      else Q.dx[A.node_eps_off[n] + i - NU] = t;
    }
    T.gsync();
    const int cs = A.node_child_start[n], cc = A.node_child_count[n];
    for (int it = lane; it < cc * NA; it += GS) {
      const int e = cs + it / NA, a = it % NA, cn = A.edge_child[e];
      if (!mk_e(A, e)) continue;
      const double* S_ = Q.ES(e);
      double t;
      if (a < NX) {
        t = S_[ES_CV + a];
#pragma unroll
        for (int b = 0; b < NX; ++b) t += S_[ES_AB + a * NA + b] * Ld[RF_DX + b];
#pragma unroll
        for (int b = 0; b < NU; ++b) t += S_[ES_AB + a * NA + NX + b] * Ld[RF_DV + b];
        Q.dx[A.node_x_off[cn] + a] = t;
      } else {
        t = Ld[RF_DV + a - NX];
      }
      Q.ND(cn)[ND_DXT + a] = t;
    }
    T.gsync();
  };
  auto load_step = [&](int n, double (&v)[FW_PL]) {
    const int e = A.node_child_start[n];
    const double *Nd = Q.ND(n), *S_ = Q.ES(e), *Nc = Q.ND(A.edge_child[e]);
#pragma unroll
    for (int q = 0; q < FW_PL; ++q) {
      const int i = lane + q * GS;
      double x = 0.0;
      if (i < NV * NA) x = Nd[ND_K + i];
      else if (i < FW_K) x = Nd[ND_KV + i - NV * NA];
      else if (i < FW_K + NX * NA) x = S_[ES_AB + i - FW_K];
      else if (i < FW_K + FW_AB) x = S_[ES_CV + i - FW_K - NX * NA];
      else if (i < FW_K + FW_AB + NX * NA) x = Nc[ND_P + i - FW_K - FW_AB];
      else if (i < FW_N) x = Nc[ND_PV + i - FW_K - FW_AB - NX * NA];
      v[q] = x;
    }
  };
  auto chain_step = [&](int n, const double (&v)[FW_PL]) {
    const int e = A.node_child_start[n], cn = A.edge_child[e];
#pragma unroll
    for (int q = 0; q < FW_PL; ++q) {
      const int i = lane + q * GS;
      if (i < FW_N) Ld[RF_IN + i] = v[q];
    }
    T.gsync();
    const ldsd *K_ = Ld + RF_IN, *KV_ = K_ + NV * NA, *AB_ = Ld + RF_IN + FW_K, *CV_ = AB_ + NX * NA,
               *PC_ = Ld + RF_IN + FW_K + FW_AB, *PV_ = PC_ + NX * NA;
    for (int i = lane; i < NV; i += GS) {
      double t = KV_[i];
#pragma unroll
      for (int a = 0; a < NA; ++a) t += K_[i * NA + a] * Ld[RF_DX + a];
      Ld[RF_DV + i] = t;
      if (i < NU) Q.dx[A.node_u_off[n] + i] = t;
      else Q.dx[A.node_eps_off[n] + i - NU] = t;
    }
    T.gsync();
    for (int a = lane; a < NA; a += GS) {
      double t;
      if (a < NX) {
        t = CV_[a];
#pragma unroll
        for (int b = 0; b < NX; ++b) t += AB_[a * NA + b] * Ld[RF_DX + b];
#pragma unroll
        for (int b = 0; b < NU; ++b) t += AB_[a * NA + NX + b] * Ld[RF_DV + b];
        Q.dx[A.node_x_off[cn] + a] = t;
      } else {
        t = Ld[RF_DV + a - NX];
      }
      Q.ND(cn)[ND_DXT + a] = t;
      Ld[RF_DXN + a] = t;
    }
    T.gsync();
    for (int a = lane; a < NX; a += GS) {
      double t = PV_[a];
#pragma unroll
      for (int b = 0; b < NA; ++b) t += PC_[a * NA + b] * Ld[RF_DXN + b];
      Q.dlam[A.edge_row0[e] + NW + a] = t;
    }
    for (int a = lane; a < NA; a += GS) Ld[RF_DX + a] = Ld[RF_DXN + a];
    T.gsync();
  };
  for (int k = 0; k < cl; ++k) {
    const int n0 = A.level_node_start[k], n1 = A.level_node_start[k + 1];
    for (int n = n0 + gid; n < n1; n += ng)
      if (mk_n(A, n)) node_step(n);
    T.sync();
  }
#ifndef DOMPC_HOST_EMU
  constexpr int FW4_PL = (FW_N + 15) / 16;
  constexpr bool FW4 = FW4_NEED > 0;
  static_assert(!FW4 || (FW4_CH == ((3 * 16 + FW_N + 1) / 2) * 2 && 4 * FW4_CH <= EL_SIZE), "four chains must fit the wavefront's LDS region");
  if (FW4 && GS == 64) {
    const int S = A.level_node_start[A.N + 1] - A.level_node_start[A.N];
    const int c4 = lane >> 4, ll = lane & 15;
    ldsd* C = Ld + c4 * FW4_CH;
    ldsd *DX = C, *DV = C + 16, *DXN = C + 32, *IN = C + 48;
    struct Ix { int uo, eo, xoc, row0; unsigned ndc; };
    const int cw = (S + ng - 1) / ng < 4 ? (S + ng - 1) / ng : 4;
    const bool deep = cw == 1;
    const int kstep = deep ? 4 : 1;
    for (int s0 = cw * gid; s0 < S && cl < A.N; s0 += cw * ng) {
      const bool here = deep || (c4 < cw && s0 + c4 < S);
      const int sc = deep ? s0 : (here ? s0 + c4 : S - 1);
#ifdef DOMPC_FW_NOSTORE
      const bool on_chain = false;
#else
      const bool on_chain = here && mk_n(A, A.level_node_start[A.N] + sc);
#endif
      ldsd *DXs = deep ? Ld : DX, *DVs = deep ? Ld + 16 : DV, *DXNs = deep ? Ld + 32 : DXN;
      double v[FW4_PL];
      auto load4 = [&](int kb, Ix& ix) {
        int n_[4], e_[4], cn_[4], uo_[4], eo_[4], xoc_[4], row0_[4];
#pragma unroll
        for (int q = 0; q < 4; ++q) {
          const int kq_ = deep ? kb + q : kb;
          const int kq = kq_ < A.N ? kq_ : A.N - 1;
          const int scq = deep ? s0 : ((q < cw && s0 + q < S) ? s0 + q : S - 1);
          n_[q] = A.level_node_start[kq];
          cn_[q] = A.level_node_start[kq + 1] + scq;
          e_[q] = scq;
        }
#pragma unroll
        for (int q = 0; q < 4; ++q) { e_[q] += A.node_child_start[n_[q]]; n_[q] += deep ? s0 : ((q < cw && s0 + q < S) ? s0 + q : S - 1); }
#pragma unroll
        for (int q = 0; q < 4; ++q) {
          uo_[q] = A.node_u_off[n_[q]]; eo_[q] = NS > 0 ? A.node_eps_off[n_[q]] : 0; xoc_[q] = A.node_x_off[cn_[q]]; row0_[q] = A.edge_row0[e_[q]];
        }
        auto pick = [&](const int (&a)[4]) { return c4 == 0 ? a[0] : (c4 == 1 ? a[1] : (c4 == 2 ? a[2] : a[3])); };
        const unsigned nd0 = (unsigned)pick(n_) * (unsigned)ND_SIZE, es0 = (unsigned)pick(e_) * (unsigned)ES_SIZE, nc0 = (unsigned)pick(cn_) * (unsigned)ND_SIZE;
        const int uo = pick(uo_), eo = pick(eo_), xoc = pick(xoc_), row0 = pick(row0_);
#pragma unroll
        for (int q = 0; q < FW4_PL; ++q) {
          const int i = ll + 16 * q;
          double x = 0.0;
          if (i < NV * NA) x = ldoff(Q.nd, nd0 + (unsigned)(ND_K + i));
          else if (i < FW_K) x = ldoff(Q.nd, nd0 + (unsigned)(ND_KV + i - NV * NA));
          else if (i < FW_K + NX * NA) x = ldoff(Q.es, es0 + (unsigned)(ES_AB + i - FW_K));
          else if (i < FW_K + FW_AB) x = ldoff(Q.es, es0 + (unsigned)(ES_CV + i - FW_K - NX * NA));
          else if (i < FW_K + FW_AB + NX * NA) x = ldoff(Q.nd, nc0 + (unsigned)(ND_P + i - FW_K - FW_AB));
          else if (i < FW_N) x = ldoff(Q.nd, nc0 + (unsigned)(ND_PV + i - FW_K - FW_AB - NX * NA));
          v[q] = x;
        }
        ix.uo = uo; ix.eo = eo; ix.xoc = xoc; ix.row0 = row0; ix.ndc = nc0;
      };
      Ix cur, nxt;
      load4(cl, cur);
      if (ll < NA && (!deep || c4 == 0)) DXs[ll] = ldoff(Q.nd, (unsigned)(A.level_node_start[cl] + sc) * (unsigned)ND_SIZE + (unsigned)(ND_DXT + ll));
      for (int k = cl; k < A.N; k += kstep) {
#pragma unroll
        for (int q = 0; q < FW4_PL; ++q) {
          const int i = ll + 16 * q;
          if (i < FW_N) IN[i] = v[q];
        }
        if (k + kstep < A.N) load4(k + kstep, nxt);
        T.gsync();
        const ldsd *K_ = IN, *KV_ = K_ + NV * NA, *AB_ = IN + FW_K, *CV_ = AB_ + NX * NA, *PC_ = IN + FW_K + FW_AB, *PV_ = PC_ + NX * NA;
        for (int qd = 0; qd < kstep; ++qd) {
          const bool act = !deep || (c4 == qd && k + qd < A.N);
          const bool on = on_chain && act;
          if (act && ll < NV) {
            double t = KV_[ll];
#pragma unroll
            for (int a = 0; a < NA; ++a) t += K_[ll * NA + a] * DXs[a];
            DVs[ll] = t;
            if (on) {
              if (ll < NU) Q.dx[cur.uo + ll] = t;
              else Q.dx[cur.eo + ll - NU] = t;
            }
          }
          T.gsync();
          if (act && ll < NA) {
            double t;
            if (ll < NX) {
              t = CV_[ll];
#pragma unroll
              for (int b = 0; b < NX; ++b) t += AB_[ll * NA + b] * DXs[b];
#pragma unroll
              for (int b = 0; b < NU; ++b) t += AB_[ll * NA + NX + b] * DVs[b];
              if (on) Q.dx[cur.xoc + ll] = t;
// ... 613 lines not shown
```

do_mpc_amd/csrc/dompc_kargs.h:

```cpp
#pragma once
#include <stdint.h>
#include "../../include/dompc_ipm.h"

namespace dompc {
enum { WIDE_BAR_STRIDE = 64 };
enum { EP_PARENT = 0, EP_CHILD, EP_LEVEL, EP_WOFF, EP_PIDX, EP_ROW0, EP_XOFF_PARENT, EP_UOFF_PARENT, EP_XOFF_CHILD, EP_EPSOFF_PARENT,
       EP_OMEGA_LO, EP_OMEGA_HI, EP_N = 16 };
#if defined(DOMPC_CONSTANT_TABLES)
typedef const __attribute__((address_space(4))) int32_t* itab_t;
typedef const __attribute__((address_space(4))) double* dtab_t;
#else
typedef const int32_t* itab_t;
typedef const double* dtab_t;
#endif
struct KArgs {
  itab_t level_node_start, node_level, node_x_off, node_u_off, node_eps_off;
  itab_t node_child_start, node_child_count, node_parent, node_in_edge;
  itab_t edge_parent, edge_child, edge_pidx, edge_w_off, edge_row0, edge_level;
  dtab_t edge_omega;
  itab_t dummy_idx;
  itab_t edge_pack;
  int32_t N, n_nodes, n_edges, n_dummy, n_opt_x, n_opt_p, n_g, e_pad;
  int32_t p_off_tvp, p_off_p, p_off_uprev;
  int32_t chain_level;
  const double *x0, *lbx, *ubx, *lbg, *ubg, *p;
  double *x_out, *g_out, *lam_x_out, *lam_g_out, *f_out;
  dompc_stats* stats;
  int32_t batch, n_slots;
  double* ws;
  int64_t ws_stride;
  int32_t* work_counter;
  dompc_options opt;
  int32_t mode;
  int32_t dbg_at_solution;
  const double *dbg_lam, *dbg_zl, *dbg_zu;
  double dbg_mu, dbg_delta;
  double *dbg_dx, *dbg_dlam, *dbg_rd, *dbg_c;
  double* trace;
  int32_t trace_cap, trace_pad;
  int32_t wide;
  int32_t pool_doubles;
  uint32_t* wide_bar;
  double* wide_partials;
  int32_t* wide_flags;
  const double *sw_x, *sw_lam;
  double *sw_g, *sw_blocks;
  const int8_t *x_mask, *g_mask, *e_mask, *n_mask;
  const int32_t* node_cut;
  int32_t n_cut, cut_level, shard_rank, shard_world;
  double* xbuf;
  int32_t xbuf_len;
  int32_t wide_spread;
  volatile uint32_t* x_req;
  volatile uint32_t* x_ack;
  volatile uint32_t* x_count;
  void (*x_callback)(void* ctx, double* buf, int32_t count);
  void* x_ctx;
  const int32_t* abort_flag;
  double lds_fill;
  int32_t lds_fill_lo, lds_fill_hi;
  double *lb_sh, *ub_sh;
  const double *sn_x, *sn_lam, *sn_mu, *sn_p;
  const int32_t* sn_sel;
  const int32_t* sn_rows;
  const int32_t* sn_cols;
  int32_t sn_nsel, sn_R, sn_ncols, sn_flags;
  double sn_tol, sn_fd_step;
  double* sn_prow;
  double* sn_D;
  double *sn_S, *sn_res;
  int32_t* sn_ok;
};


// ... 2 lines not shown
```

do_mpc_amd/csrc/dompc_phases.h:

```cpp

template <bool FINE>
DOMPC_DEV inline double trial_edges(const Thr& T, const Prob& Q) {
  const KArgs& A = *Q.A;
  double f = 0.0;
  if (FINE && !DENSE_EDGE && M > 0) {
    constexpr int NPC = NI * DEG + 1;
    for (int it = T.tid; it < A.n_edges * NPC; it += T.nt) {
      const int e = it % A.n_edges, q = it / A.n_edges;
      const double fe = eval_edge_f_t<true>(Q, e, Q.xt, Q.st, Q.ct, q == 0 ? NI * DEG : q - 1);
      f += fe;
    }
  } else
  for (int e = T.tid; e < A.n_edges; e += T.nt) {
    const int m = mk_e(A, e);
    if (!m) continue;
    const double fe = DENSE_EDGE ? dae_edge_f(Q, e, Q.xt, Q.st, Q.ct) : eval_edge_f(Q, e, Q.xt, Q.st, Q.ct);
    if (sh_cnt(A, m)) f += fe;
  }
  for (int n = T.tid; n < A.n_nodes; n += T.nt)
    if (sh_cnt(A, mk_n(A, n))) f += node_rterm_f(Q, n, Q.xt);
  return f;
}
DOMPC_DEV inline void step_rules_pass(const Thr& T, const Prob& Q, double mu, double (&r5)[5]) {
  const KArgs& A = *Q.A;
  const int nX = A.n_opt_x, nSl = A.n_edges * NE;
  for (int i = 0; i < 5; ++i) r5[i] = 0.0;
  {
    double x_[DOMPC_FW], l_[DOMPC_FW], u2_[DOMPC_FW], d_[DOMPC_FW], gf_[DOMPC_FW], zl_[DOMPC_FW], zu_[DOMPC_FW];
#define L_(u, g) x_[u] = Q.x[g]; l_[u] = Q.lb[g]; u2_[u] = Q.ub[g]; d_[u] = Q.dx[g]; gf_[u] = Q.gf[g]; zl_[u] = Q.zl[g]; zu_[u] = Q.zu[g];
#define B_(u, g)                                                                               \
    if (sh_cnt(A, mk_x(A, g))) {                                                           \
      const double xv = x_[u], l = l_[u], ub_ = u2_[u], d = d_[u];                         \
      double gphi = gf_[u];                                                                \
      if (l > -INFINITY) {                                                                 \
        const double r = fast_rcp(xv - l);                                                 \
        r5[0] = fmax(r5[0], -d * r);                                \
        r5[1] = fmax(r5[1], 1.0 + r * d - mu * r * fast_rcp(zl_[u]));         \
        gphi -= mu * r;                                                                    \
      }                                                                                    \
      if (ub_ < INFINITY) {                                                                \
        const double r = fast_rcp(ub_ - xv);                                               \
        r5[0] = fmax(r5[0], d * r);                                                        \
        r5[1] = fmax(r5[1], 1.0 - r * d - mu * r * fast_rcp(zu_[u]));                      \
        gphi += mu * r;                                                                    \
      }                                                                                    \
      if (KAPPA_D != 0.0) gphi += KAPPA_D * mu * one_sided(l, ub_);                        \
      r5[2] += gphi * d;                                                                   \
    }
    DOMPC_FOR4(nX, L_, B_)
#undef L_
#undef B_
  }
  for (int g = T.tid; g < nSl; g += T.nt) {
    if (!sh_cnt(A, mk_e(A, g / NE1))) continue;
    const int si = (g / NE1) * NE1 + g % NE1;
    const double sv = Q.s[si], l = Q.sl[si], u = Q.su[si], d = Q.ds[si];
    double gphi = 0.0;
    if (l > -INFINITY) {
      const double r = fast_rcp(sv - l);
      r5[0] = fmax(r5[0], -d * r);
      r5[1] = fmax(r5[1], 1.0 + r * d - mu * r * fast_rcp(Q.zsl[si]));
      gphi -= mu * r;
    }
    if (u < INFINITY) {
      const double r = fast_rcp(u - sv);
      r5[0] = fmax(r5[0], d * r);
      r5[1] = fmax(r5[1], 1.0 - r * d - mu * r * fast_rcp(Q.zsu[si]));
      gphi += mu * r;
    }
    if (KAPPA_D != 0.0) gphi += KAPPA_D * mu * one_sided(l, u);
    r5[2] += gphi * d;
  }
  const int ops[5] = {R_MAX, R_MAX, R_SUM, R_SUM, R_SUM};
  wg_reduce(T, r5, ops);
}
template <bool FINE>
DOMPC_DEV inline void eval_trial_pass(const Thr& T, const Prob& Q, double al, double a_z, double mu, double& obj_o, double& th_o, double& bar_o, Comp& Cp) {
  const KArgs& A = *Q.A;
  const int nX = A.n_opt_x, nSl = A.n_edges * NE;
  const double ks = 1e10;
  double r3[3] = {0.0, 0.0, 0.0};
  LogAcc La{1.0, 0, 0};
  double lin = 0.0;
  Cp = Comp{-INFINITY, INFINITY, 0.0};
  {
    double x_[DOMPC_FW], d_[DOMPC_FW], l_[DOMPC_FW], u2_[DOMPC_FW], zl_[DOMPC_FW], zu_[DOMPC_FW];
#define L_(u, g) x_[u] = Q.x[g]; d_[u] = Q.dx[g]; l_[u] = Q.lb[g]; u2_[u] = Q.ub[g]; zl_[u] = Q.zl[g]; zu_[u] = Q.zu[g];
#define B_(u, g)                                                                               \
    if (mk_x(A, g)) {                                                                      \
      const double xt_ = x_[u] + al * d_[u];                                               \
      const double xv = xt_, l = l_[u], ub_ = u2_[u];                                      \
      const bool cnt_ = sh_cnt(A, mk_x(A, g));                                             \
      Q.xt[g] = xt_;                                                                       \
      if (cnt_) {                                                                          \
        if (l_[u] > -INFINITY) logacc_add(La, xt_ - l_[u]);                                \
        if (u2_[u] < INFINITY) logacc_add(La, u2_[u] - xt_);                               \
        if (KAPPA_D != 0.0) { const double os_ = one_sided(l_[u], u2_[u]); lin += os_ > 0.0 ? xt_ - l_[u] : (os_ < 0.0 ? u2_[u] - xt_ : 0.0); } \
      }                                                                                    \
      if (l > -INFINITY) {                                                                 \
        const double ro = fast_rcp(x_[u] - l);                       \
        const double z = zl_[u] + a_z * (mu * ro - zl_[u] - zl_[u] * ro * d_[u]);          \
        const double dd = xv - l, mr = mu * fast_rcp(dd);                                  \
        const double zn = fmax(fmin(z, ks * mr), mr * (1.0 / ks));                         \
        Q.zlt[g] = zn;                                                                     \
        if (cnt_) comp_add(Cp, dd * zn, zn);                                               \
      }                                                                                    \
      if (ub_ < INFINITY) {                                                                \
        const double ro = fast_rcp(ub_ - x_[u]);                                           \
        const double z = zu_[u] + a_z * (mu * ro - zu_[u] + zu_[u] * ro * d_[u]);          \
        const double dd = ub_ - xv, mr = mu * fast_rcp(dd);                                \
        const double zn = fmax(fmin(z, ks * mr), mr * (1.0 / ks));                         \
        Q.zut[g] = zn;                                                                     \
        if (cnt_) comp_add(Cp, dd * zn, zn);                                               \
      }                                                                                    \
    }
    DOMPC_FOR4(nX, L_, B_)
#undef L_
#undef B_
  }
  for (int g = T.tid; g < nSl; g += T.nt) {
    if (!mk_e(A, g / NE1)) continue;
    const int si = (g / NE1) * NE1 + g % NE1;
    const double so = Q.s[si], dsv = Q.ds[si];
    const double sv = so + al * dsv;
    const bool cnt_ = sh_cnt(A, mk_e(A, g / NE1));
    Q.st[si] = sv;
    const double l = Q.sl[si], u = Q.su[si];
    if (l > -INFINITY) {
      const double z = Q.zsl[si] + a_z * dz_lo(so, l, Q.zsl[si], dsv, mu);
      const double zn = fmax(fmin(z, ks * mu / (sv - l)), mu / (ks * (sv - l)));
      Q.zslt[si] = zn;
      if (cnt_) comp_add(Cp, (sv - l) * zn, zn);
    }
    if (u < INFINITY) {
      const double z = Q.zsu[si] + a_z * dz_up(so, u, Q.zsu[si], dsv, mu);
      const double zn = fmax(fmin(z, ks * mu / (u - sv)), mu / (ks * (u - sv)));
      Q.zsut[si] = zn;
      if (cnt_) comp_add(Cp, (u - sv) * zn, zn);
    }
  }
  {
    double y_[DOMPC_FW], dy_[DOMPC_FW];
#define L_(u, g) y_[u] = Q.lam[g]; dy_[u] = Q.dlam[g];
#define B_(u, g) if (mk_g(A, g)) Q.lamt[g] = y_[u] + al * dy_[u];
    DOMPC_FOR4(A.n_g, L_, B_)
#undef L_
#undef B_
  }
  T.sync();
  for (int g = T.tid; g < NX; g += T.nt) Q.ct[g] = FREE_ROOT ? 0.0 : Q.xt[A.node_x_off[0] + g] - Q.P[g] / DOMPC_SX[g];
  if (FREE_ROOT && T.tid == 0) r3[0] += Q.sf * dompc_aterm_f(Q.xt + A.node_x_off[0], Q.P, Q.P + A.p_off_tvp, Q.P + A.p_off_p);
  r3[0] += trial_edges<FINE>(T, Q);
  T.sync();
  {
    double c_[DOMPC_FW];
#define L_(u, g) c_[u] = Q.ct[g];
#define B_(u, g) if (sh_cnt(A, mk_g(A, g))) r3[1] += fabs(c_[u]);
    DOMPC_FOR4(A.n_g, L_, B_)
#undef L_
#undef B_
  }
  for (int g = T.tid; g < nSl; g += T.nt) {
    if (!sh_cnt(A, mk_e(A, g / NE1))) continue;
    const int si = (g / NE1) * NE1 + g % NE1;
    if (Q.sl[si] > -INFINITY) logacc_add(La, Q.st[si] - Q.sl[si]);
    if (Q.su[si] < INFINITY) logacc_add(La, Q.su[si] - Q.st[si]);
    if (KAPPA_D != 0.0) { const double os_ = one_sided(Q.sl[si], Q.su[si]); lin += os_ > 0.0 ? Q.st[si] - Q.sl[si] : (os_ < 0.0 ? Q.su[si] - Q.st[si] : 0.0); }
  }
  r3[2] = -logacc_value(La);
  if (KAPPA_D != 0.0) r3[2] += KAPPA_D * lin;
  const int ops[3] = {R_SUM, R_SUM, R_SUM};
  wg_reduce(T, r3, ops);
  obj_o = r3[0]; th_o = r3[1]; bar_o = r3[2];
}
struct PhaseRet { unsigned gen, nred, xseq; int rc; };
struct PhaseRet3 { unsigned gen, nred, xseq; double v0, v1, v2; };
struct PhaseRet6 { unsigned gen, nred, xseq; double v0, v1, v2, c0, c1, c2; };
#ifndef DOMPC_HOST_EMU
#define DOMPC_PHASE_PROLOGUE                                                        \
  const KArgs A = kernel_args(kp);                                                  \
  Thr T = make_thr(A);                                                              \
  T.kp = kp;                                                                        \
  T.gen = ufl(gen); T.nred = ufl(nred); T.xseq = ufl(xseq);                         \
  Prob Q = make_prob(A, ufl(slot), A.p + (int64_t)ufl(b) * A.n_opt_p);              \
  Q.sf = ufl(sf);
__device__ __attribute__((noinline)) PhaseRet phase_sweep(const void* kp, int b, int slot, double sf, double mu, double dsw, int soc, unsigned gen, unsigned nred, unsigned xseq) {
  DOMPC_PHASE_PROLOGUE
  Q.soc = ufl(soc);
  prob_bounds(Q);
  Q.dsw = ufl(dsw);
  const int rc = sweep<false>(T, Q, ufl(mu));
  return PhaseRet{T.gen, T.nred, T.xseq, rc};
}
__device__ __attribute__((noinline)) PhaseRet phase_sweep_fine(const void* kp, int b, int slot, double sf, double mu, double dsw, int soc, unsigned gen, unsigned nred, unsigned xseq) {
  DOMPC_PHASE_PROLOGUE
  Q.soc = ufl(soc);
  prob_bounds(Q);
  Q.dsw = ufl(dsw);
  const int rc = sweep<true>(T, Q, ufl(mu));
  return PhaseRet{T.gen, T.nred, T.xseq, rc};
}
__device__ __attribute__((noinline)) PhaseRet phase_backward(const void* kp, int b, int slot, double sf, double mu, double delta, double dsw, int mode, unsigned gen, unsigned nred, unsigned xseq) {
  DOMPC_PHASE_PROLOGUE
  Q.dsw = ufl(dsw);
  Q.soc = ufl(mode);
  prob_bounds(Q);
  const int rc = riccati_backward(T, Q, ufl(mu), ufl(delta));
  return PhaseRet{T.gen, T.nred, T.xseq, rc};
}
__device__ __attribute__((noinline)) PhaseRet phase_forward(const void* kp, int b, int slot, double sf, double mu, double delta, double dsw, unsigned gen, unsigned nred, unsigned xseq) {
  DOMPC_PHASE_PROLOGUE
  Q.dsw = ufl(dsw);
  riccati_forward_t<false>(T, Q, ufl(mu), ufl(delta));
  return PhaseRet{T.gen, T.nred, T.xseq, 0};
}
__device__ __attribute__((noinline)) PhaseRet phase_forward_adj(const void* kp, int b, int slot, double sf, double mu, double delta, double dsw, unsigned gen, unsigned nred, unsigned xseq) {
  DOMPC_PHASE_PROLOGUE
  Q.dsw = ufl(dsw);
  riccati_forward_t<true>(T, Q, ufl(mu), ufl(delta));
  return PhaseRet{T.gen, T.nred, T.xseq, 0};
}
__device__ __attribute__((noinline)) PhaseRet3 phase_step_rules(const void* kp, int b, int slot, double sf, double mu, unsigned gen, unsigned nred, unsigned xseq) {
  DOMPC_PHASE_PROLOGUE
  double r5[5];
  step_rules_pass(T, Q, ufl(mu), r5);
  return PhaseRet3{T.gen, T.nred, T.xseq, r5[0], r5[1], r5[2]};
}
__device__ __attribute__((noinline)) PhaseRet6 phase_eval_trial(const void* kp, int b, int slot, double sf, double al, double a_z, double mu, unsigned gen, unsigned nred, unsigned xseq) {
  DOMPC_PHASE_PROLOGUE
  double o = 0.0, th = 0.0, br = 0.0;
  Comp C;
  eval_trial_pass<false>(T, Q, ufl(al), ufl(a_z), ufl(mu), o, th, br, C);
  return PhaseRet6{T.gen, T.nred, T.xseq, o, th, br, C.smax, C.smin, C.sum_z};
}
__device__ __attribute__((noinline)) PhaseRet6 phase_eval_trial_fine(const void* kp, int b, int slot, double sf, double al, double a_z, double mu, unsigned gen, unsigned nred, unsigned xseq) {
  DOMPC_PHASE_PROLOGUE
  double o = 0.0, th = 0.0, br = 0.0;
  Comp C;
  eval_trial_pass<true>(T, Q, ufl(al), ufl(a_z), ufl(mu), o, th, br, C);
  return PhaseRet6{T.gen, T.nred, T.xseq, o, th, br, C.smax, C.smin, C.sum_z};
}
#undef DOMPC_PHASE_PROLOGUE
#define DOMPC_PHASE_CALL(fn, ...)                                                   \
  const auto r_ = fn(T.kp, b, slot, Q.sf, __VA_ARGS__, T.gen, T.nred, T.xseq);            \
  T.gen = ufl(r_.gen); T.nred = ufl(r_.nred); T.xseq = ufl(r_.xseq);
#endif
#ifndef DOMPC_REPEAT_PHASE
#define DOMPC_REPEAT_PHASE 0
#endif
DOMPC_DEV inline int run_sweep(const Thr& T, Prob& Q, int b, int slot, double mu, int soc = 0, double dsw = 0.0) {
  Q.dsw = dsw;
  Q.lu_ok = lu_store_rule(*Q.A, mu, soc) ? 1 : 0;
  Q.rp_soc = soc; Q.rp_mu = mu;
#ifndef DOMPC_HOST_EMU
  if (fine_items(T, *Q.A)) { DOMPC_PHASE_CALL(phase_sweep_fine, mu, dsw, soc) return ufl(r_.rc); }
  if (DOMPC_REPEAT_PHASE & 1) { DOMPC_PHASE_CALL(phase_sweep, mu, dsw, soc) }
  DOMPC_PHASE_CALL(phase_sweep, mu, dsw, soc)
  return ufl(r_.rc);
#else
  (void)b; (void)slot;
  Q.soc = soc;
  prob_bounds(Q);
  const int rc = fine_items(T, *Q.A) ? sweep<true>(T, Q, mu) : sweep<false>(T, Q, mu);
  Q.soc = 0;
  prob_bounds(Q);
  return rc;
#endif
}
DOMPC_DEV inline int run_backward(const Thr& T, const Prob& Q, int b, int slot, double mu, double delta, int mode = 0) {
#ifndef DOMPC_HOST_EMU
  if (DOMPC_REPEAT_PHASE & 2) {
    { DOMPC_PHASE_CALL(phase_backward, mu, delta, Q.dsw, mode) }
    { DOMPC_PHASE_CALL(phase_sweep, Q.rp_mu, Q.dsw, Q.rp_soc) }
  }
  DOMPC_PHASE_CALL(phase_backward, mu, delta, Q.dsw, mode)
  return ufl(r_.rc);
#else
  (void)b; (void)slot;
  Prob Qm = Q;
  Qm.soc = mode;
  prob_bounds(Qm);
  return riccati_backward(T, Qm, mu, delta);
#endif
}
DOMPC_DEV inline void run_step_rules(const Thr& T, const Prob& Q, int b, int slot, double mu, double (&r5)[5]) {
#ifndef DOMPC_HOST_EMU
  if (DOMPC_REPEAT_PHASE & 16) { DOMPC_PHASE_CALL(phase_step_rules, mu) }
  DOMPC_PHASE_CALL(phase_step_rules, mu)
  r5[0] = ufl(r_.v0); r5[1] = ufl(r_.v1); r5[2] = ufl(r_.v2); r5[3] = 0.0; r5[4] = 0.0;
#else
  (void)b; (void)slot;
  step_rules_pass(T, Q, mu, r5);
#endif
}
DOMPC_DEV inline void run_eval_trial(const Thr& T, const Prob& Q, int b, int slot, double al, double a_z, double mu, double& obj_o, double& th_o, double& bar_o, Comp& Cp) {
#ifndef DOMPC_HOST_EMU
  if (fine_items(T, *Q.A)) { DOMPC_PHASE_CALL(phase_eval_trial_fine, al, a_z, mu) obj_o = ufl(r_.v0); th_o = ufl(r_.v1); bar_o = ufl(r_.v2); Cp = Comp{r_.c0, r_.c1, r_.c2}; return; }
  if (DOMPC_REPEAT_PHASE & 8) { DOMPC_PHASE_CALL(phase_eval_trial, al, a_z, mu) }
  DOMPC_PHASE_CALL(phase_eval_trial, al, a_z, mu)
  obj_o = ufl(r_.v0); th_o = ufl(r_.v1); bar_o = ufl(r_.v2); Cp = Comp{r_.c0, r_.c1, r_.c2};
#else
  (void)b; (void)slot;
  if (fine_items(T, *Q.A)) eval_trial_pass<true>(T, Q, al, a_z, mu, obj_o, th_o, bar_o, Cp); else eval_trial_pass<false>(T, Q, al, a_z, mu, obj_o, th_o, bar_o, Cp);
#endif
}
DOMPC_DEV inline void run_forward(const Thr& T, const Prob& Q, int b, int slot, double mu, double delta) {
#ifndef DOMPC_HOST_EMU
  if (forward_adjoint(Q, mu)) {
    DOMPC_PHASE_CALL(phase_forward_adj, mu, delta, Q.dsw)
  } else {
    if (DOMPC_REPEAT_PHASE & 4) { DOMPC_PHASE_CALL(phase_forward, mu, delta, Q.dsw) }
    DOMPC_PHASE_CALL(phase_forward, mu, delta, Q.dsw)
  }
#else
  (void)b; (void)slot;
  if (forward_adjoint(Q, mu)) riccati_forward_t<true>(T, Q, mu, delta);
  else riccati_forward_t<false>(T, Q, mu, delta);
#endif
}
```

do_mpc_amd/csrc/dompc_quad.h:

```cpp
#if !defined(DOMPC_HOST_EMU) && DOMPC_DEG >= 1 && DOMPC_M >= 1 && DOMPC_NI == 1 && DOMPC_NX + DOMPC_NU + 2 <= 16 && DOMPC_DEG * DOMPC_DEG * DOMPC_NX <= 64

using dompc_lanes::rbc;
using dompc_lanes::pin;
using dompc_lanes::fmac_rbc;
using dompc_lanes::sfor;

struct MoRef { int kind, off; };
constexpr MoRef moref_in(int d, const int* vidx, int nv, const int* cidx, int nc, int base) {
  for (int k = 0; k < nv; ++k) if (vidx[k] == d) return MoRef{2, base + k};
  for (int k = 0; k < nc; ++k) if (cidx[k] == d) return MoRef{1, k};
  return MoRef{0, 0};
}
constexpr MoRef moref_dyn(int p, int d) { return moref_in(d, DOMPC_DYN_VIDX, DOMPC_DYN_NV, DOMPC_DYN_CIDX, DOMPC_DYN_NC, p * DOMPC_DYN_NV); }
constexpr MoRef moref_lt(int d) { return moref_in(d, DOMPC_LT_VIDX, DOMPC_LT_NV, DOMPC_LT_CIDX, DOMPC_LT_NC, MOC_LT); }
constexpr MoRef moref_nl(int d) { return moref_in(d, DOMPC_NL_VIDX, DOMPC_NL_NV, DOMPC_NL_CIDX, DOMPC_NL_NC, MOC_NL); }
constexpr MoRef moref_mt(int d) { return moref_in(d, DOMPC_MT_VIDX, DOMPC_MT_NV, DOMPC_MT_CIDX, DOMPC_MT_NC, MOC_MT); }
template <int KIND, int OFF>
__device__ inline double mo_dyn_val(const ldsd* rec) { if constexpr (KIND == 2) return rec[OFF]; else if constexpr (KIND == 1) return DOMPC_DYN_CVAL[OFF]; else return 0.0; }
template <int KIND, int OFF>
__device__ inline double mo_lt_val(const ldsd* rec) { if constexpr (KIND == 2) return rec[OFF]; else if constexpr (KIND == 1) return DOMPC_LT_CVAL[OFF]; else return 0.0; }
template <int KIND, int OFF>
__device__ inline double mo_nl_val(const ldsd* rec) { if constexpr (KIND == 2) return rec[OFF]; else if constexpr (KIND == 1) return DOMPC_NL_CVAL[OFF]; else return 0.0; }
template <int KIND, int OFF>
__device__ inline double mo_mt_val(const ldsd* rec) { if constexpr (KIND == 2) return rec[OFF]; else if constexpr (KIND == 1) return DOMPC_MT_CVAL[OFF]; else return 0.0; }
// ... 199 lines not shown
  sfor<R>([&](auto K_) {
    constexpr int k = K_, sk = k / NX, bk = k % NX;
    constexpr int rt1 = (4 * (k / 4 + 1) < R) ? 4 * (k / 4 + 1) : R;
    QD_SB();
    const bool own = (j == bk);
    double m = 0.0;
#pragma unroll
    for (int r = k + 1; r < rt1; ++r) m = fmax(m, fabs(bc[sk][r]));
    const double akk = fabs(bc[sk][k]);
    bad |= (int)(own & !(akk >= GJ_U * m && akk > 1e-300));
    const double pl = fast_rcp((akk > 1e-300) ? bc[sk][k] : 1.0);
    const double pinv = rbc<bk>(pl);
    sig[sk] = own ? -pl : sig[sk];
    double pm[DEG];
#pragma unroll
    for (int s = 0; s < DEG; ++s) {
      const double prow = bc[s][k] * pinv;
      pm[s] = (s == sk && own) ? 0.0 : -prow;
      bc[s][k] = (s == sk && own) ? -1.0 : prow;
      pin(pm[s]);
    }
    asm volatile("s_nop 1");
    sfor<R>([&](auto R_) {
      constexpr int r = R_;
      if constexpr (r != k) {
        sfor<DEG>([&](auto S_) { constexpr int s = S_; if constexpr (s != sk) fmac_rbc<bk>(bc[s][r], bc[sk][r], pm[s]); });
        fmac_rbc<bk>(bc[sk][r], bc[sk][r], pm[sk]);
      }
    });
#pragma unroll
    for (int s = 0; s < DEG; ++s)
#pragma unroll
      for (int r = 0; r < R; ++r) pin(bc[s][r]);
  });
  QD_SB();
#pragma unroll
  for (int s = 0; s < DEG; ++s)
#pragma unroll
    for (int r = 0; r < R; ++r) bc[s][r] *= sig[s];
  QD_SB();
  if (__ballot(bad) != 0ull) return 2;
  QD_PH(2)
  QD_SB();
  if (st_x) {
    if (!soc) {
#pragma unroll
      for (int jj = 0; jj < DEG; ++jj) Q.c[pk.row0 + jj * NX + (int)b] = res[jj];
      Q.c[pk.row0 + R + (int)b] = rc;
      Q.c[pk.row0 + NW + (int)b] = ce;
    }
#pragma unroll
    for (int s = 0; s < M; ++s) {
      const int gi = pk.woff + s * NX + (int)b;
      Q.gf[gi] = 0.0;
      Q.rd[gi] = RDv[s];
    }
    double* ew = Q.ew + (int64_t)e * EW_SIZE;
    if (store_lu) {
#pragma unroll
      for (int s = 0; s < DEG; ++s)
#pragma unroll
        for (int r = 0; r < R; ++r) ew[EW_LU + r * LU_N + s * NX + (int)b] = bc[s][r];
    }
#pragma unroll
    for (int s = 0; s < M; ++s) {
      ew[EW_SIGW + s * NX + (int)b] = SGv[s] + Q.dsw;
      ew[EW_RW + s * NX + (int)b] = RWv[s];
    }
  }
  if (e0n >= 0) stage_quad(Q, e0n, lane, Ld, bank ^ 1);
  {
    const int en = (e0n >= 0 ? e0n : e0) + g;
    pkn = qd_pack(A, en < A.n_edges ? en : A.n_edges - 1, Q.sf);
  }
  double Wc[NW];
  {
#pragma unroll
    for (int r = 0; r < R; ++r) {
      double t = (isx ? DOMPC_C[0 * (DEG + 1) + 1] : -1.0) * bc[0][r];
#pragma unroll
      for (int s = 1; s < DEG; ++s) t = fma(isx ? DOMPC_C[0 * (DEG + 1) + s + 1] : 0.0, bc[s][r], t);
      Wc[r] = t;
    }
    sfor<NX>([&](auto A_) {
      constexpr int a = A_;
      const double rcb = rbc<a>(rc);
      double t = (j == NA) ? -rcb : ((j == a) ? DOMPC_D[0] : 0.0);
#pragma unroll
      for (int s = 1; s <= DEG; ++s) t = fma(DOMPC_D[s], Wc[(s - 1) * NX + a], t);
      Wc[R + a] = t;
    });
  }
#pragma unroll
  for (int r = 0; r < NW; ++r) pin(Wc[r]);
  double* S_ = Q.es + (int64_t)e * ES_SIZE;
  {
    double cv = 0.0;
    sfor<NX>([&](auto A_) {
      constexpr int a = A_;
      if (act && j < NA) S_[ES_AB + a * NA + j] = Wc[R + a];
      const double w0a = rbc<NA>(Wc[R + a]);
      cv = (j == a) ? w0a + ce : cv;
    });
    pin(cv);
    if (st_x) S_[ES_CV + (int)b] = cv;
  }
  QD_PH(7)
// ... 573 lines not shown
```

do_mpc_amd/csrc/dompc_riccati.h:

```cpp

DOMPC_DEV inline int ycol(int yj) { return yj < NX ? yj : NA + (yj - NX); }

namespace rb {
constexpr int RB_QO = 0, RB_QOV = RB_QO + NYT * NYT;
constexpr int RB_QF = RB_QOV + NYT, RB_QFV = RB_QF + NYT * NYT;
constexpr int RB_PC = RB_QFV + NYT, RB_PCV = RB_PC + NA * NA;
constexpr int RB_AT = RB_PCV + NA, RB_CT = RB_AT + NA * NA;
constexpr int RB_TP = RB_CT + NA, RB_TV = RB_TP + NA * NA;
constexpr int RB_K = RB_TV + NA, RB_KV = RB_K + NV * NA;
constexpr int RB_ACL = RB_KV + NV, RB_CCL = RB_ACL + NA * NA;
constexpr int RB_PN = RB_CCL + NA, RB_PNV = RB_PN + NA * NA;
constexpr int RB_NL = RB_PNV + NA;
constexpr int RB_SIZE = RB_NL + NE * (NA + 4);
}

DOMPC_DEV inline int yidx(int i) { return (i < NX) ? i : ((i >= NA && i < NA + NU) ? NX + (i - NA) : -1); }

constexpr int RN_IPL = (NYT * NYT + GS_C - 1) / GS_C;
constexpr int RN_VPL = (NYT + GS_C - 1) / GS_C;
constexpr int RN_NE1 = NE > 0 ? NE : 1;
constexpr int RN_NLN = NE * (NA + 4);
constexpr int RN_NLP = NE > 0 ? (RN_NLN + GS_C - 1) / GS_C : 1;
constexpr int RN_ABN = NX * (NA + 1);
constexpr int RN_ABP = (RN_ABN + GS_C - 1) / GS_C;
struct NodePre {
  double qt[RN_IPL];
  double pv[RN_VPL][10];
  double nl[RN_NLP];
  double ab[RN_ABP];
};

DOMPC_DEV inline double node_nl_load(const Prob& Q, int e, int it) {
  if (it < NE * NA) return Q.EW(e, EW_JD + it);
  const int j = it - NE * NA, kind = j / RN_NE1, q = j % RN_NE1;
  const double* S_ = Q.ES(e);
  return kind == 0 ? S_[ES_SIGS + q] : kind == 1 ? S_[ES_RDN + q] : kind == 2 ? S_[ES_RSN + q]
                   : Q.lam[Q.A->edge_row0[e] + NW + NX + q];
}

DOMPC_DEV inline void node_prefetch(const Prob& Q, int n, double delta, int lane, int GS, NodePre& R) {
  const KArgs& A = *Q.A;
  const int e = A.node_child_start[n];
  const double* S_ = Q.ES(e);
  const int xo = A.node_x_off[n], uo = A.node_u_off[n];
  const int eo = NS > 0 ? A.node_eps_off[n] : -1;
  const int ie = A.node_in_edge[n], pn = A.node_parent[n];
  (void)delta;
#pragma unroll
  for (int q = 0; q < RN_IPL; ++q) {
    const int it = lane + q * GS;
    const int itc = it < NYT * NYT ? it : 0;
    const int yi = yidx(itc / NYT), yj = yidx(itc % NYT);
    const int idx = (yi >= 0 && yj >= 0) ? symi(yi, yj, NA) : 0;
    R.qt[q] = S_[ES_QT + idx];
  }
#pragma unroll
  for (int v = 0; v < RN_VPL; ++v) {
    const int i0 = lane + v * GS;
    const int i = i0 < NYT ? i0 : 0;
    const int yi = yidx(i);
    const bool is_up = (i >= NX && i < NA);
    const int g = (i < NX) ? xo + i : (is_up ? uo + (i - NX) : (i < NA + NU ? uo + (i - NA) : eo + (i - NA - NU)));
    R.pv[v][0] = Q.x[g];
    R.pv[v][1] = Q.lb[g];
    R.pv[v][2] = Q.ub[g];
    R.pv[v][3] = Q.zl[g];
    R.pv[v][4] = Q.zu[g];
    R.pv[v][5] = (i < NX) ? ((ie >= 0) ? Q.lam[A.edge_row0[ie] + NW + i] : Q.lam[i]) : 0.0;
    const int iu = is_up ? i - NX : (i >= NA && i < NA + NU ? i - NA : 0);
    const bool hu = i >= NX && i < NA + NU;
    R.pv[v][6] = hu ? (pn >= 0 ? Q.x[A.node_u_off[pn] + iu] : Q.P[A.p_off_uprev + iu] / DOMPC_SU[iu]) : 0.0;
    R.pv[v][7] = 0.0;
    R.pv[v][8] = yi >= 0 ? S_[ES_QV + yi] : 0.0;
    R.pv[v][9] = 0.0;
  }
  if (NE > 0) {
#pragma unroll
    for (int q = 0; q < RN_NLP; ++q) {
      const int it = lane + q * GS;
      R.nl[q] = it < RN_NLN ? node_nl_load(Q, e, it) : 0.0;
    }
  }
#pragma unroll
  for (int q = 0; q < RN_ABP; ++q) {
    const int it = lane + q * GS;
    const int itc = it < RN_ABN ? it : 0;
    const int i = itc / (NA + 1), j = itc % (NA + 1);
    R.ab[q] = (j < NA) ? S_[ES_AB + i * NA + j] : S_[ES_CV + i];
  }
}

DOMPC_DEV inline int riccati_node(const Thr& T, const Prob& Q, int n, double mu, double delta, ldsd* Ld, int lane, int GS,
                                  bool child_staged, const NodePre& R) {
  using namespace rb;
  const KArgs& A = *Q.A;
  double* Nd = Q.ND(n);
  const int cs = A.node_child_start[n], cc = A.node_child_count[n];
  const double rw = node_rweight(Q, n);
  const double rwh = (Q.soc & 2) ? 0.0 : rw;
  long long pc0 = prof_clock();
#if DOMPC_PROFILE
#define DOMPC_PN(i) if (T.prof && T.tid == 0) { const long long pc1 = prof_clock(); T.prof[i] += pc1 - pc0; pc0 = pc1; }
#else
#define DOMPC_PN(i)
#endif
  double qacc[RN_IPL];
#pragma unroll
  for (int q = 0; q < RN_IPL; ++q) {
    const int it = lane + q * GS;
    const int itc = it < NYT * NYT ? it : 0;
    const int yi = yidx(itc / NYT), yj = yidx(itc % NYT);
    const bool valid = it < NYT * NYT && yi >= 0 && yj >= 0;
    const int idx = valid ? symi(yi, yj, NA) : 0;
    double v = R.qt[q];
    for (int c = 1; c < cc; ++c) v += Q.ES(cs + c)[ES_QT + idx];
    qacc[q] = valid ? v : 0.0;
  }
  double gvv[RN_VPL], dgv[RN_VPL];
#pragma unroll
  for (int v = 0; v < RN_VPL; ++v) {
    const int i0 = lane + v * GS;
    const int i = i0 < NYT ? i0 : 0;
    const int yi = yidx(i);
    const bool is_up = (i >= NX && i < NA);
    const double xv = R.pv[v][0], lo = R.pv[v][1], hi = R.pv[v][2], zlo = R.pv[v][3], zhi = R.pv[v][4];
    const double upv = R.pv[v][6];
    double dg, gv;
    if (is_up) {
      if (RT_CUSTOM) {
        dg = 0.0; gv = 0.0;
        for (int c = 0; c < cc; ++c) gv += Q.ES(cs + c)[ES_RTUP + (i - NX)];
      } else {
        dg = 2.0 * rwh * DOMPC_RTERM[i - NX];
        gv = -2.0 * rw * DOMPC_RTERM[i - NX] * (xv - upv);
      }
    } else {
      dg = sigma_of(xv, lo, hi, zlo, zhi) + delta;
      gv = bar_grad(xv, lo, hi, mu, !(Q.soc & 2));
      if (i < NX) gv += (A.node_in_edge[n] >= 0) ? -R.pv[v][5] : R.pv[v][5];
      else if (i < NA + NU) {
        if (!RT_CUSTOM) {
          dg += 2.0 * rwh * DOMPC_RTERM[i - NA];
          gv += 2.0 * rw * DOMPC_RTERM[i - NA] * (xv - upv);
        }
      } else {
        gv += cc * Q.sf * DOMPC_EPS_PEN[i - NA - NU];
      }
    }
    gv += R.pv[v][8];
    if (FREE_ROOT && n == 0 && i0 < NX) gv += Nd[ND_AT + 1 + i];
    if (yi >= 0)
      for (int c = 1; c < cc; ++c) gv += Q.ES(cs + c)[ES_QV + yi];
    gvv[v] = gv;
    dgv[v] = dg;
  }
  if (NE > 0) {
    constexpr int NL_JD = RB_NL, NL_SG = RB_NL + NE * NA, NL_RD = NL_SG + NE, NL_RS = NL_RD + NE, NL_YD = NL_RS + NE;
    for (int c = 0; c < cc; ++c) {
#pragma unroll
      for (int q = 0; q < RN_NLP; ++q) {
        const int it = lane + q * GS;
        if (it < RN_NLN) Ld[RB_NL + it] = (c == 0) ? R.nl[q] : node_nl_load(Q, cs + c, it);
      }
      T.gsync();
#pragma unroll
      for (int v = 0; v < RN_VPL; ++v) {
        const int i0 = lane + v * GS;
        const int i = i0 < NYT ? i0 : 0;
        const int yi = yidx(i);
        double gv = gvv[v];
        for (int q = 0; q < NE; ++q) {
          const double sg = Ld[NL_SG + q] + delta;
          double ji = 0.0;
          if (yi >= 0) ji = Ld[NL_JD + q * NA + yi];
          else if (i >= NA + NU && nl_slack(q) == i - NA - NU) { ji = -Q.sgn[(cs + c) * NE1 + q]; gv += ji * Ld[NL_YD + q]; }
          gv += ji * (sg * Ld[NL_RD + q] + Ld[NL_RS + q]);
        }
        gvv[v] = gv;
      }
#pragma unroll
      for (int q = 0; q < RN_IPL; ++q) {
        const int it = lane + q * GS;
        const int itc = it < NYT * NYT ? it : 0;
        const int i = itc / NYT, j = itc % NYT;
        const int yi = yidx(i), yj = yidx(j);
        double v = qacc[q];
        for (int qq = 0; qq < NE; ++qq) {
          const double sg = Ld[NL_SG + qq] + delta;
          double ji = 0.0, jj = 0.0;
          if (yi >= 0) ji = Ld[NL_JD + qq * NA + yi];
          else if (i >= NA + NU && nl_slack(qq) == i - NA - NU) ji = -Q.sgn[(cs + c) * NE1 + qq];
          if (yj >= 0) jj = Ld[NL_JD + qq * NA + yj];
// ... 429 lines not shown
  }
  for (int it = lane; it < NV * NA; it += GS) Ld[RB_K + it] = Nd[ND_K + it];
  for (int it = lane; it < NV; it += GS) Ld[RB_KV + it] = Nd[ND_KV + it];
  T.gsync();
  for (int it = lane; it < NA * (NA + 1); it += GS) {
    const int i = it / (NA + 1), j = it % (NA + 1);
    if (j < NA) {
      double t = Ld[RB_QO + i * NYT + j];
      for (int q = 0; q < NV; ++q) {
        t += Ld[RB_QO + i * NYT + NA + q] * Ld[RB_K + q * NA + j];
        t += Ld[RB_K + q * NA + i] * Ld[RB_QO + (NA + q) * NYT + j];
        double t2 = 0.0;
        for (int w = 0; w < NV; ++w) t2 += Ld[RB_QO + (NA + q) * NYT + NA + w] * Ld[RB_K + w * NA + j];
        t += Ld[RB_K + q * NA + i] * t2;
      }
      Nd[ND_P + i * NA + j] = t + X2[i * NA + j];
    } else {
      double t = Ld[RB_QOV + i];
      for (int w = 0; w < NV; ++w) t += Ld[RB_QO + i * NYT + NA + w] * Ld[RB_KV + w];
      for (int q = 0; q < NV; ++q) {
        double t2 = Ld[RB_QOV + NA + q];
        for (int w = 0; w < NV; ++w) t2 += Ld[RB_QO + (NA + q) * NYT + NA + w] * Ld[RB_KV + w];
        t += Ld[RB_K + q * NA + i] * t2;
      }
      Nd[ND_PV + i] = t + X2[NA * NA + i];
    }
  }
  T.gsync();
  return 0;
}

}
#include "dompc_riccati16.h"
namespace dompc {

DOMPC_PHASE int riccati_backward(const Thr& T, const Prob& Q, double mu, double delta) {
#ifndef DOMPC_HOST_EMU
  if constexpr (R16_ENABLED) return r16::backward(T, Q, mu, delta);
#endif
  using namespace rb;
  const KArgs& A = *Q.A;
  static_assert(!RB_IN_LDS || RB_SIZE <= EL_SIZE, "node working set must fit the per-group LDS region");
  const int GS = T.gs, ng = T.nt / GS, gid = group_index(T.tid, GS), lane = T.tid % GS;
  ldsd* Ld = T.edge_lds + (int64_t)(T.ltid / GS) * EL_SIZE;
  const int FSET = T.flag_begin(0);
  {
    const int n0 = A.level_node_start[A.N], n1 = A.level_node_start[A.N + 1];
    for (int it = T.tid; it < (n1 - n0) * NA * (NA + 1); it += T.nt) {
      const int n = n0 + it / (NA * (NA + 1));
      if (!mk_n(A, n)) continue;
      const int r = it % (NA * (NA + 1));
      const int i = r / (NA + 1), j = r % (NA + 1);
      double* Nd = Q.ND(n);
      const int ie = A.node_in_edge[n];
      const double* S_ = Q.ES(ie);
      const int xo = A.node_x_off[n];
      if (j < NA) {
        double v = 0.0;
        if (i < NX && j < NX) {
          v = S_[ES_MH + i * NX + j];
          if (i == j) v += sigma_of(Q.x[xo + i], Q.lb[xo + i], Q.ub[xo + i], Q.zl[xo + i], Q.zu[xo + i]) + delta;
        }
        Nd[ND_P + i * NA + j] = v;
      } else {
        double v = 0.0;
        if (i < NX)
          v = S_[ES_MG + i] - Q.lam[A.edge_row0[ie] + NW + i] + bar_grad(Q.x[xo + i], Q.lb[xo + i], Q.ub[xo + i], mu, !(Q.soc & 2));
        Nd[ND_PV + i] = v;
      }
    }
    T.sync();
  }
  const int cl = A.chain_level < A.N ? A.chain_level : A.N;
  {
    const int S = A.level_node_start[A.N + 1] - A.level_node_start[A.N];
    for (int s_ = gid; s_ < S; s_ += ng) {
      if (!mk_n(A, A.level_node_start[A.N] + s_)) continue;
      bool staged = false;
      NodePre R;
      if (A.N - 1 >= cl) node_prefetch(Q, A.level_node_start[A.N - 1] + s_, delta, lane, GS, R);
      for (int k = A.N - 1; k >= cl; --k) {
        NodePre Rn;
        if (k > cl) node_prefetch(Q, A.level_node_start[k - 1] + s_, delta, lane, GS, Rn);
        if (staged) {
          for (int it = lane; it < NA * NA; it += GS) Ld[RB_PC + it] = Ld[RB_PN + it];
          for (int it = lane; it < NA; it += GS) Ld[RB_PCV + it] = Ld[RB_PNV + it];
          T.gsync();
        }
        if (riccati_node(T, Q, A.level_node_start[k] + s_, mu, delta, Ld, lane, GS, staged, R)) { T.fset(0, FSET); break; }
        staged = true;
        if (k > cl) R = Rn;
      }
    }
    T.sync();
    if ((T.fget(0) == FSET) && !sh_on(A)) return 1;
  }
  for (int k = cl - 1; k >= 0; --k) {
    const int n0 = A.level_node_start[k], n1 = A.level_node_start[k + 1];
    if (sh_on(A) && k == A.cut_level - 1) {
      for (int n = n0 + gid; n < n1; n += ng) riccati_cut_node(T, Q, n, mu, delta, Ld, lane, GS, 1);
      T.xchg(x_c1(A), A.n_cut * CUT1);
      for (int n = n0 + gid; n < n1; n += ng)
        if (riccati_cut_node(T, Q, n, mu, delta, Ld, lane, GS, 2)) T.fset(0, FSET);
      T.sync();
      double* fl = A.xbuf + x_c2(A) + A.n_cut * CUT2;
      for (int w = T.tid; w < A.shard_world; w += T.nt) fl[w] = (w == A.shard_rank && (T.fget(0) == FSET)) ? 1.0 : 0.0;
      T.xchg(x_c2(A), A.n_cut * CUT2 + A.shard_world);
      for (int n = n0 + gid; n < n1; n += ng) riccati_cut_node(T, Q, n, mu, delta, Ld, lane, GS, 3);
      int bad = 0;
      for (int w = 0; w < A.shard_world; ++w) bad |= (fl[w] != 0.0);
      T.sync();
      if (bad) return 1;
      continue;
    }
    for (int n = n0 + gid; n < n1; n += ng) {
      if (!mk_n(A, n)) continue;
      NodePre R;
      node_prefetch(Q, n, delta, lane, GS, R);
      if (riccati_node(T, Q, n, mu, delta, Ld, lane, GS, false, R)) T.fset(0, FSET);
    }
// ... 40 lines not shown
```

do_mpc_amd/csrc/dompc_riccati16.h:

```cpp
#pragma once

namespace dompc {
namespace r16 {
constexpr bool ENABLED = R16_ENABLED;

#ifndef DOMPC_HOST_EMU
constexpr int KB_A = (NA + 3) / 4, KB_Y = (NYT + 3) / 4;
constexpr int KB_H = (NA + 4) / 4;
constexpr int HR = NA / 4, HG = NA % 4;
static_assert(!R16_ENABLED || NA <= 15, "the homogeneous row / column needs NA <= 15");
template <int KB>
__device__ inline d4 tmul(const d4& At, const d4& B) { return tile_mul<KB>(At, B); }
__device__ inline double rl(double v, int src) { return lane_bcast(v, src); }

__device__ inline int yz(int i) { return (i < NX) ? i : ((i >= NA && i < NA + NU) ? NX + (i - NA) : -1); }

__device__ inline d4 col_to_tile(double vc, int lane, int col, int nrow) {
  const int g = lane >> 4, j = lane & 15;
  d4 t;
#pragma unroll
  for (int r = 0; r < 4; ++r) {
    const double s = __shfl(vc, g + 4 * r);
    t[r] = (j == col && g + 4 * r < nrow) ? s : 0.0;
  }
  return t;
}

typedef d4 Val;

__device__ inline void load_edge(const Prob& Q, int e, int lane, d4& F, d4& cvr, double& fu) {
  const int g = lane >> 4, j = lane & 15;
  const double* S_ = Q.ES(e);
  const int yj = yz(j);
#pragma unroll
  for (int r = 0; r < 4; ++r) {
    const int i = g + 4 * r;
    double fv = 0.0;
    if (i < NX) { if (yj >= 0 && j < NYT) fv = S_[ES_AB + i * NA + yj]; }
    else if (i < NA) fv = (j == NA + (i - NX)) ? 1.0 : 0.0;
    F[r] = fv;
    cvr[r] = (i < NX) ? S_[ES_CV + i] : 0.0;
  }
  double v = 0.0;
  if (g < NU) { if (j < NX) v = S_[ES_AB + j * NA + NX + g]; else if (j < NA) v = (g == j - NX) ? 1.0 : 0.0; }
  fu = v;
}

__device__ inline d4 load_qt(const Prob& Q, int e, int lane) {
  const int g = lane >> 4, j = lane & 15;
  const double* S_ = Q.ES(e);
  const int yj = yz(j);
  d4 t;
#pragma unroll
  for (int r = 0; r < 4; ++r) {
    const int i = g + 4 * r;
    const int yi = yz(i);
    const bool valid = i < NYT && j < NYT && yi >= 0 && yj >= 0;
    t[r] = valid ? S_[ES_QT + symi(yi, yj, NA)] : 0.0;
  }
  return t;
}

__device__ inline Val load_val(const Prob& Q, int n, int lane) {
  const int g = lane >> 4, j = lane & 15;
  const double* Nd = Q.ND(n);
  Val V;
#pragma unroll
  for (int r = 0; r < 4; ++r) {
    const int i = g + 4 * r;
    double v = (i < NA && j < NA) ? Nd[ND_P + i * NA + j] : 0.0;
    if (i < NA && j == NA) v = Nd[ND_PV + i];
    if (i == NA && j < NA) v = Nd[ND_PV + j];
    V[r] = v;
  }
  return V;
}
__device__ inline void store_val(const Prob& Q, int n, const Val& V, int lane) {
  const int g = lane >> 4, j = lane & 15;
  double* Nd = Q.ND(n);
#pragma unroll
  for (int r = 0; r < 4; ++r) {
    const int i = g + 4 * r;
    if (i < NA && j < NA) Nd[ND_P + i * NA + j] = V[r];
    if (i < NA && j == NA) Nd[ND_PV + i] = V[r];
  }
}

__device__ inline Val leaf(const Prob& Q, int n, double mu, double delta, int lane) {
  const KArgs& A = *Q.A;
  const int g = lane >> 4, j = lane & 15;
  const int ie = A.node_in_edge[n];
  const double* S_ = Q.ES(ie);
  const int xo = A.node_x_off[n];
  const int jj = j < NX ? j : 0;
  const double xv = Q.x[xo + jj], lo = Q.lb[xo + jj], hi = Q.ub[xo + jj];
  const double dg = sigma_of(xv, lo, hi, Q.zl[xo + jj], Q.zu[xo + jj]) + delta;
  const double gv = (j < NX) ? S_[ES_MG + jj] - Q.lam[A.edge_row0[ie] + NW + jj] + bar_grad(xv, lo, hi, mu, !(Q.soc & 2)) : 0.0;
  Val V = col_to_tile(gv, lane, NA, NX);
#pragma unroll
  for (int r = 0; r < 4; ++r) {
    const int i = g + 4 * r;
    double v = (i < NX && j < NX) ? S_[ES_MH + i * NX + j] : 0.0;
    if (i == j && j < NX) v += dg;
    if (i == NA && j < NX) v = gv;
    V[r] += v;
  }
  return V;
}

constexpr int ES_STAGE = R16_STAGE;
static_assert(ES_QV + NA <= ES_STAGE && ES_QT + NA_T <= ES_QV && ES_CV + NX <= ES_QT,
              "the staged head of the edge record must contain A, B, c, Q~, q~ + r_y");
static_assert(!R16_ENABLED || 2 * ES_STAGE <= EL_SIZE, "two staging buffers must fit the wavefront's LDS region");
struct NodeIn { double xv, lo, hi, zlo, zhi, nu, upv; };
__device__ inline void stage_edge(const Prob& Q, int e, int lane, ldsd* dst) {
  const double* S_ = Q.ES(e);
#pragma unroll
  for (int q = 0; q < ES_STAGE / 128; ++q)
    __builtin_amdgcn_global_load_lds((const __attribute__((address_space(1))) void*)(S_ + 128 * q + 2 * lane),
                                     (__attribute__((address_space(3))) void*)(dst + 128 * q), 16, 0, 0);
}
__device__ inline void staged_ready() { asm volatile("s_waitcnt vmcnt(0)" ::: "memory"); }
__device__ inline void load_node(const Prob& Q, int n, int lane, NodeIn& R) {
  const KArgs& A = *Q.A;
  const int j = lane & 15;
  const int xo = A.node_x_off[n], uo = A.node_u_off[n];
  const int ie = A.node_in_edge[n], pn = A.node_parent[n];
  const bool is_up = (j >= NX && j < NA);
  const int jj = j < NYT ? j : 0;
  const int eo = NS > 0 ? A.node_eps_off[n] : 0;
  const bool is_eps = NS > 0 && jj >= NA + NU;
  const int gi = (jj < NX) ? xo + jj : (is_up ? uo + (jj - NX) : (is_eps ? eo + (jj - NA - NU) : uo + (jj - NA)));
  R.xv = Q.x[gi]; R.lo = Q.lb[gi]; R.hi = Q.ub[gi]; R.zlo = Q.zl[gi]; R.zhi = Q.zu[gi];
  const int iu = is_up ? jj - NX : ((jj >= NA && !is_eps) ? jj - NA : 0);
  R.upv = (jj >= NX && !is_eps) ? (pn >= 0 ? Q.x[A.node_u_off[pn] + iu] : Q.P[A.p_off_uprev + iu] / tab_sel(DOMPC_SU, iu)) : 0.0;
  R.nu = (jj < NX) ? ((ie >= 0) ? Q.lam[A.edge_row0[ie] + NW + jj] : Q.lam[jj]) : 0.0;
}
__device__ inline void staged_tiles(const ldsd* Ls, int lane, d4& qt, d4& F, d4& cvr, double& fu, double& qv) {
  const int g = lane >> 4, j = lane & 15;
  const int yj = yz(j);
#pragma unroll
  for (int r = 0; r < 4; ++r) {
    const int i = g + 4 * r;
    const int yi = yz(i);
    const bool valid = i < NYT && j < NYT && yi >= 0 && yj >= 0;
    const double q_ = Ls[ES_QT + (valid ? symi(yi, yj, NA) : 0)];
    qt[r] = valid ? q_ : 0.0;
    const double ab = Ls[ES_AB + ((i < NX && yj >= 0) ? i * NA + yj : 0)];
    double fv = (i < NX && yj >= 0 && j < NYT) ? ab : 0.0;
    if (i >= NX && i < NA) fv = (j == NA + (i - NX)) ? 1.0 : 0.0;
    F[r] = fv;
    const double cv = Ls[ES_CV + (i < NX ? i : 0)];
    cvr[r] = (i < NX) ? cv : 0.0;
  }
  {
    const double ab = Ls[ES_AB + ((j < NX && g < NU) ? j * NA + NX + g : 0)];
    double v = (g < NU && j < NX) ? ab : 0.0;
    if (g < NU && j >= NX && j < NA) v = (g == j - NX) ? 1.0 : 0.0;
    fu = v;
  }
  const int yjj = (j < NYT) ? yj : -1;
  qv = (yjj >= 0) ? Ls[ES_QV + (yjj >= 0 ? yjj : 0)] : 0.0;
}

__device__ inline int node(const Prob& Q, int n, double mu, double delta, int lane, const NodeIn& R, const ldsd* Ls, const Val* first, Val& out) {
  const KArgs& A = *Q.A;
  const int g = lane >> 4, j = lane & 15;
  const int cs = A.node_child_start[n], cc = A.node_child_count[n];
  const double rw = node_rweight(Q, n);
  const double rwh = (Q.soc & 2) ? 0.0 : rw;
  long long pc0 = prof_clock();
#if DOMPC_PROFILE
#define R16_PN(i) if (threadIdx.x == 0) { const long long pc1 = prof_clock(); lds_prof[i] += pc1 - pc0; pc0 = pc1; }
#else
#define R16_PN(i)
#endif
  d4 qt_s, F, cvr;
  double fu, qv_s;
  staged_tiles(Ls, lane, qt_s, F, cvr, fu, qv_s);
  R16_PN(12)
  double dg = 0.0, gv = 0.0;
  {
    const int ie = A.node_in_edge[n];
    const bool is_up = (j >= NX && j < NA);
    const int jj = j < NYT ? j : 0;
    const bool is_eps = NS > 0 && jj >= NA + NU;
    const int iu = is_up ? jj - NX : ((jj >= NA && !is_eps) ? jj - NA : 0);
    const double xv = R.xv, lo = R.lo, hi = R.hi, upv = R.upv;
    if (is_up) {
      dg = 2.0 * rwh * tab_sel(DOMPC_RTERM, iu);
      gv = -2.0 * rw * tab_sel(DOMPC_RTERM, iu) * (xv - upv);
    } else {
      dg = sigma_of(xv, lo, hi, R.zlo, R.zhi) + delta;
      gv = bar_grad(xv, lo, hi, mu, !(Q.soc & 2));
      if (jj < NX) {
        gv += (ie >= 0) ? -R.nu : R.nu;
      } else if (is_eps) {
        if constexpr (NS > 0) gv += cc * Q.sf * tab_sel(DOMPC_EPS_PEN, jj - NA - NU);
      } else {
        dg += 2.0 * rwh * tab_sel(DOMPC_RTERM, iu);
        gv += 2.0 * rw * tab_sel(DOMPC_RTERM, iu) * (xv - upv);
      }
    }
    const int yjj = yz(jj);
    gv += qv_s;
    if (yjj >= 0)
      for (int c = 1; c < cc; ++c) gv += Q.ES(cs + c)[ES_QV + yjj];
    if constexpr (NE > 0) {
      for (int c = 0; c < cc; ++c) {
        const int e = cs + c;
        const double* S_ = Q.ES(e);
#pragma unroll
        for (int q = 0; q < NE; ++q) {
          const double sg = S_[ES_SIGS + q] + delta;
          const bool slack_here = NS > 0 && jj >= NA + NU && nl_slack(q) == jj - NA - NU;
          const double jc = (yjj >= 0) ? Q.EW(e, EW_JD + q * NA + yjj) : (slack_here ? -Q.sgn[e * NE1 + q] : 0.0);
          gv += jc * (sg * S_[ES_RDN + q] + S_[ES_RSN + q]);
          if (slack_here) gv += jc * Q.lam[A.edge_row0[e] + NW + NX + q];
        }
      }
    }
    if (j >= NYT) { dg = 0.0; gv = 0.0; }
  }
  R16_PN(13)
  d4 QO = qt_s;
  for (int c = 1; c < cc; ++c) QO += load_qt(Q, cs + c, lane);
#pragma unroll
  for (int r = 0; r < 4; ++r) {
    const int i = g + 4 * r;
    if (i == j) QO[r] += dg;
    else if ((i >= NX && i < NA && j == i + NU) || (j >= NX && j < NA && i == j + NU))
      QO[r] -= 2.0 * rwh * tab_sel(DOMPC_RTERM, (i < j ? i : j) - NX);
  }
  R16_PN(14)
  if constexpr (NE > 0) {
    const int jz = j < NYT ? j : 0, yj = yz(jz);
// ... 81 lines not shown
      }
    };
    solve(qv);
    solve(qx);
#pragma unroll
    for (int u = 0; u < NV; ++u) { kv[u] = -qv[u]; Kj[u] = (j < NA) ? -qx[u] : 0.0; }
  }
  R16_PN(10)
  d4 Lc;
#pragma unroll
  for (int r = 0; r < 4; ++r) {
    const int k = g + 4 * r;
    double v = (k < NA) ? ((k == j) ? 1.0 : 0.0) : 0.0;
#pragma unroll
    for (int u = 0; u < NV; ++u)
      if (k == NA + u) v = (j == NA) ? kv[u] : Kj[u];
    Lc[r] = v;
  }
  double bK = 0.0;
#pragma unroll
  for (int u = 0; u < NV; ++u)
    if (g == u) bK = (j == NA) ? kv[u] : Kj[u];
  {
    const d4 U = tmul<KB_Y>(QO, Lc) + qo0;
    out = tmul<KB_Y>(Lc, U);
    double t = gv;
#pragma unroll
    for (int u = 0; u < NV; ++u) t += Kj[u] * rl(gv, NA + u);
    if (g == HG && j < NA) out[HR] += t;
  }
  R16_PN(11)
  for (int c = cc - 1; c >= 0; --c) {
    if (c != cc - 1) {
      load_edge(Q, cs + c, lane, F, cvr, fu);
      Vc = (c == 0 && first) ? *first : load_val(Q, A.edge_child[cs + c], lane);
    }
    d4 Fy;
#pragma unroll
    for (int r = 0; r < 4; ++r) Fy[r] = (j < NA) ? F[r] : ((j == NA) ? ((g + 4 * r == NA) ? 1.0 : cvr[r]) : 0.0);
    const d4 Acl = __builtin_amdgcn_mfma_f64_16x16x4f64(fu, bK, Fy, 0, 0, 0);
    const d4 T2 = tmul<KB_H>(Vc, Acl);
    out += tmul<KB_H>(Acl, T2);
  }
  R16_PN(24)
  staged_ready();
  R16_PN(25)
  double* Nd = Q.ND(n);
  if (g == 0 && j < NA)
#pragma unroll
    for (int u = 0; u < NV; ++u) Nd[ND_K + u * NA + j] = Kj[u];
  if (lane == 0)
#pragma unroll
    for (int u = 0; u < NV; ++u) Nd[ND_KV + u] = kv[u];
  store_val(Q, n, out, lane);
  R16_PN(26)
#undef R16_PN
  return bad;
}

__device__ inline int backward(const Thr& T, const Prob& Q, double mu, double delta) {
  const KArgs& A = *Q.A;
  const int ng = T.nt / 64, gid = group_index(T.tid, 64), lane = T.tid % 64;
  ldsd* Ld = T.edge_lds + (int64_t)(T.ltid / 64) * EL_SIZE;
  const int FSET = T.flag_begin(0);
  const int cl = A.chain_level < A.N ? A.chain_level : A.N;
  const int S = A.level_node_start[A.N + 1] - A.level_node_start[A.N];
  for (int s_ = gid; s_ < S; s_ += ng) {
    NodeIn in;
    int buf = 0;
    if (A.N - 1 >= cl) {
      const int n1 = A.level_node_start[A.N - 1] + s_;
      load_node(Q, n1, lane, in);
      stage_edge(Q, A.node_child_start[n1], lane, Ld);
    }
    Val V = leaf(Q, A.level_node_start[A.N] + s_, mu, delta, lane);
    store_val(Q, A.level_node_start[A.N] + s_, V, lane);
    staged_ready();
    for (int k = A.N - 1; k >= cl; --k) {
      NodeIn nx;
#if DOMPC_PROFILE
      const long long pcl = prof_clock();
#endif
      if (k > cl) {
        const int np = A.level_node_start[k - 1] + s_;
        load_node(Q, np, lane, nx);
        stage_edge(Q, A.node_child_start[np], lane, Ld + (buf ^ 1) * ES_STAGE);
      }
#if DOMPC_PROFILE
      if (threadIdx.x == 0) lds_prof[27] += prof_clock() - pcl;
#endif
      Val Vn;
      if (node(Q, A.level_node_start[k] + s_, mu, delta, lane, in, Ld + buf * ES_STAGE, &V, Vn)) { T.fset(0, FSET); break; }
      V = Vn;
      if (k > cl) in = nx;
      buf ^= 1;
    }
  }
  T.sync();
  if ((T.fget(0) == FSET)) return 1;
  for (int k = cl - 1; k >= 0; --k) {
    const int n0 = A.level_node_start[k], n1 = A.level_node_start[k + 1];
    for (int n = n0 + gid; n < n1; n += ng) {
      NodeIn in;
      load_node(Q, n, lane, in);
      stage_edge(Q, A.node_child_start[n], lane, Ld);
      staged_ready();
      Val Vn;
      if (node(Q, n, mu, delta, lane, in, Ld, nullptr, Vn)) T.fset(0, FSET);
    }
    T.sync();
    if ((T.fget(0) == FSET)) return 1;
  }
  return 0;
}
#endif

}
}
```

do_mpc_amd/csrc/dompc_runtime.cpp:

```cpp
#include <chrono>
#include <dlfcn.h>
#include <cmath>
#include <thread>

#include "dompc_host.h"
#include "dompc_kargs.h"

#ifdef DOMPC_HOST_EMU
extern "C" void dompc_hostemu_model_info(const int32_t* in, int64_t* out, char* hash);
extern "C" void dompc_hostemu_run(const dompc::KArgs* A);
#endif

static thread_local std::string g_create_error;
static const int BATCH_ONE_WAVE = 4096;

struct dompc_handle : dompc_host::Context {
  dompc_problem_desc d;
  std::string code_path;
  int32_t e_pad = 0, n_slots = 0, block = 256, occupancy = 0, n_leaves = 1;
  bool batch_object_stale = false;
  bool block_auto = true;
  int32_t slots64 = 0, slots256 = 0;
  int64_t ws_stride = 0, sweep_block = 0, el_size = 0, edges_per_wave = 1, riccati_kind = 0;
  dompc::KArgs base;
// ... 263 lines not shown
    if (hipModuleOccupancyMaxActiveBlocksPerMultiprocessor(&occ, h->fn_solve, block, lds) == hipSuccess &&
        hipDeviceGetAttribute(&cus, hipDeviceAttributeMultiprocessorCount, d.device) == hipSuccess && occ > 0 && cus > 0)
      resident = occ * cus;
    h->occupancy = occ;
#endif
    return resident;
  };
  h->slots64 = resident_at(64);
  h->slots256 = resident_at(fit_block(h, 256));
  {
    const int resident = h->block_auto ? (max_batch >= BATCH_ONE_WAVE ? h->slots64 : h->slots256) : resident_at(h->block);
    h->n_slots = d.n_slots > 0 ? d.n_slots : (max_batch < resident ? max_batch : resident);
  }
  if (const char* se = getenv("DOMPC_SLOTS")) { const int v = atoi(se); if (v >= 1) h->n_slots = v; }
  if (h->n_slots < 1) h->n_slots = 1;
#ifdef DOMPC_HOST_EMU
  h->n_slots = 1;
#endif
  dompc::KArgs& A = h->base;
  memset(&A, 0, sizeof(A));
  int rc = 0;
  rc |= upload(h, &A.level_node_start, d.level_node_start, d.N + 2);
  rc |= upload(h, &A.node_level, d.node_level, d.n_nodes);
  rc |= upload(h, &A.node_x_off, d.node_x_off, d.n_nodes);
  rc |= upload(h, &A.node_u_off, d.node_u_off, d.n_nodes);
  rc |= upload(h, &A.node_eps_off, d.node_eps_off, d.n_nodes);
  rc |= upload(h, &A.node_child_start, d.node_child_start, d.n_nodes);
  rc |= upload(h, &A.node_child_count, d.node_child_count, d.n_nodes);
  rc |= upload(h, &A.node_parent, d.node_parent, d.n_nodes);
  rc |= upload(h, &A.node_in_edge, d.node_in_edge, d.n_nodes);
  rc |= upload(h, &A.edge_parent, d.edge_parent, d.n_edges);
  rc |= upload(h, &A.edge_child, d.edge_child, d.n_edges);
  rc |= upload(h, &A.edge_pidx, d.edge_pidx, d.n_edges);
  rc |= upload(h, &A.edge_w_off, d.edge_w_off, d.n_edges);
  rc |= upload(h, &A.edge_row0, d.edge_row0, d.n_edges);
  rc |= upload(h, &A.edge_level, d.edge_level, d.n_edges);
  rc |= upload(h, &A.edge_omega, d.edge_omega, d.n_edges);
  rc |= upload(h, &A.dummy_idx, d.dummy_idx, d.n_dummy);
  if (rc) return fail(1);
  {
    std::vector<int32_t> pack((size_t)d.n_edges * dompc::EP_N, 0);
    for (int e = 0; e < d.n_edges; ++e) {
      int32_t* q = pack.data() + (size_t)e * dompc::EP_N;
      const int n = d.edge_parent[e], cn = d.edge_child[e];
      q[dompc::EP_PARENT] = n; q[dompc::EP_CHILD] = cn; q[dompc::EP_LEVEL] = d.edge_level[e]; q[dompc::EP_WOFF] = d.edge_w_off[e];
      q[dompc::EP_PIDX] = d.edge_pidx[e]; q[dompc::EP_ROW0] = d.edge_row0[e];
      q[dompc::EP_XOFF_PARENT] = d.node_x_off[n]; q[dompc::EP_UOFF_PARENT] = d.node_u_off[n]; q[dompc::EP_XOFF_CHILD] = d.node_x_off[cn];
      q[dompc::EP_EPSOFF_PARENT] = d.node_eps_off ? d.node_eps_off[n] : -1;
      int64_t ob;
      memcpy(&ob, &d.edge_omega[e], sizeof ob);
      q[dompc::EP_OMEGA_LO] = (int32_t)(uint32_t)(ob & 0xffffffffll); q[dompc::EP_OMEGA_HI] = (int32_t)(uint32_t)((uint64_t)ob >> 32);
    }
    if (upload(h, &A.edge_pack, pack.data(), pack.size())) return fail(1);
  }
  A.N = d.N; A.n_nodes = d.n_nodes; A.n_edges = d.n_edges; A.n_dummy = d.n_dummy;
  A.n_opt_x = d.n_opt_x; A.n_opt_p = d.n_opt_p; A.n_g = d.n_g; A.e_pad = h->e_pad;
  A.p_off_tvp = d.p_off_tvp; A.p_off_p = d.p_off_p; A.p_off_uprev = d.p_off_uprev;
  {
    const int32_t* ls = desc->level_node_start;
    const int S = ls[d.N + 1] - ls[d.N];
    h->n_leaves = S > 0 ? S : 1;
    int cl = d.N;
    for (int k = d.N - 1; k >= 0; --k) {
      bool ok = (ls[k + 1] - ls[k]) == S;
      for (int s = 0; ok && s < S; ++s) {
        const int n = ls[k] + s;
        ok = desc->node_child_count[n] == 1 && desc->edge_child[desc->node_child_start[n]] == ls[k + 1] + s &&
             desc->node_child_start[n] == desc->node_child_start[ls[k]] + s;
      }
      if (!ok) break;
      cl = k;
    }
    A.chain_level = cl;
  }
  A.opt = d.opts;
  if (const char* mi = getenv("DOMPC_MAX_ITER")) A.opt.max_iter = atoi(mi);
  if (const char* lf = getenv("DOMPC_LDS_FILL")) {
    double v = 0.0; int lo = 0, hi = 1 << 30;
    sscanf(lf, "%lf,%d,%d", &v, &lo, &hi);
    A.lds_fill = v; A.lds_fill_lo = lo; A.lds_fill_hi = hi;
  }
  A.n_slots = h->n_slots;
  A.ws_stride = h->ws_stride;
#ifndef DOMPC_HOST_EMU
  {
    void* dw = nullptr;
    if (hipHostGetDevicePointer(&dw, h->abort_word, 0) != hipSuccess) { h->error = "hipHostGetDevicePointer failed"; return fail(1); }
    A.abort_flag = (const int32_t*)dw;
  }
#else
  A.abort_flag = h->abort_word;
#endif
  if (h->alloc((void**)&A.ws, sizeof(double) * (size_t)h->ws_stride * h->n_slots)) return fail(1);
#ifndef DOMPC_HOST_EMU
  if (const char* fill = getenv("DOMPC_WS_FILL")) {
    if (hipMemset(A.ws, atoi(fill), sizeof(double) * (size_t)h->ws_stride * h->n_slots) != hipSuccess) { h->error = "hipMemset failed"; return fail(1); }
  }
#endif
  if (h->alloc((void**)&A.work_counter, 64)) return fail(1);
  A.lb_sh = A.ub_sh = nullptr;
  {
    const char* sb = getenv("DOMPC_SHARED_BOUNDS");
    if (!sb || atoi(sb) != 0) {
      if (h->alloc((void**)&A.lb_sh, sizeof(double) * (size_t)d.n_opt_x)) return fail(1);
      if (h->alloc((void**)&A.ub_sh, sizeof(double) * (size_t)d.n_opt_x)) return fail(1);
    }
// ... 544 lines not shown
```

do_mpc_amd/csrc/dompc_sweep.h:

```cpp


template <bool FINE>
DOMPC_DEV inline int sweep(const Thr& T, Prob& Q, double mu) {
  const KArgs& A = *Q.A;
  const int FSET = T.flag_begin(1);
  long long pc0 = prof_clock();
#if DOMPC_PROFILE
#define DOMPC_PS(i) if (T.prof && T.tid == 0) { const long long pc1 = prof_clock(); T.prof[i] += pc1 - pc0; pc0 = pc1; }
#else
#define DOMPC_PS(i)
#endif
  (void)pc0;
  if (!Q.soc)
    for (int g = T.tid; g < NX; g += T.nt) Q.c[g] = FREE_ROOT ? 0.0 : Q.x[A.node_x_off[0] + g] - Q.P[g] / DOMPC_SX[g];
  if (FREE_ROOT && T.tid == 0) {
    double* at = Q.ND(0) + ND_AT;
    double hp[NX_T > 0 ? NX_T : 1], gr[NX > 0 ? NX : 1], val = 0.0;
    dompc_aterm(Q.x + A.node_x_off[0], Q.P, Q.P + A.p_off_tvp, Q.P + A.p_off_p, &val, gr, hp);
    const double wh = (Q.soc & 2) ? 0.0 : Q.sf;
    at[0] = Q.sf * val;
    for (int a = 0; a < NX; ++a) at[1 + a] = Q.sf * gr[a];
    for (int a = 0; a < NX; ++a)
      for (int b = 0; b < NX; ++b) at[1 + NX + a * NX + b] = wh * hp[symi(a, b, NX)];
  }
// ... 74 lines not shown
      for (int r = lane; r < NW; r += GS) {
        const int gi = wvar(woff, zoff, r);
        Q.EW(e, EW_RW + r) += dmu * bar_grad(Q.x[gi], Q.lb[gi], Q.ub[gi], 1.0);
      }
      double* S_ = Q.ES(e);
      for (int a = lane; a < NA; a += GS) S_[ES_QV + a] += dmu * S_[ES_QVB + a];
    }
    if (NE > 0) {
      double* S_ = Q.ES(e);
      for (int i = lane; i < NE; i += GS) {
        const int si = e * NE1 + i;
        S_[ES_RSN + i] += dmu * bar_grad(Q.s[si], Q.sl[si], Q.su[si], 1.0);
      }
    }
  }
  T.sync();
}

DOMPC_DEV inline double dz_lo(double x, double l, double z, double d, double mu) { return mu / (x - l) - z - z / (x - l) * d; }
DOMPC_DEV inline double dz_up(double x, double u, double z, double d, double mu) { return mu / (u - x) - z + z / (u - x) * d; }

struct LogAcc { double m; int e; int bad; };
DOMPC_DEV inline void logacc_add(LogAcc& L, double a) {
  if (!(a > 0.0) || !(a < INFINITY)) L.bad = 1;
  int ea = 0;
  const double fa = frexp(a, &ea);
  L.m *= fa;
  L.e += ea;
  if (L.m < 0x1p-500) { int em = 0; L.m = frexp(L.m, &em); L.e += em; }
}
DOMPC_DEV inline double logacc_value(const LogAcc& L) { return L.bad ? NAN : log(L.m) + (double)L.e * 0.6931471805599453; }

struct Comp { double smax, smin, sum_z; };
DOMPC_DEV inline void comp_add(Comp& C, double s, double z) { C.smax = fmax(C.smax, s); C.smin = fmin(C.smin, s); C.sum_z += z; }
DOMPC_DEV inline double comp_err(const Comp& C, double mu) { return C.smax >= C.smin ? fmax(C.smax - mu, mu - C.smin) : 0.0; }

#ifndef DOMPC_FW
#define DOMPC_FW 8
#endif
#define DOMPC_FOR4(n, LOAD, BODY)                                              \
  for (int g0_ = T.tid; g0_ < (n); g0_ += DOMPC_FW * T.nt) {                   \
    _Pragma("unroll") for (int u_ = 0; u_ < DOMPC_FW; ++u_) {                  \
      const int g_ = g0_ + u_ * T.nt;                                          \
      const int gc_ = g_ < (n) ? g_ : g0_;                                     \
      LOAD(u_, gc_)                                                            \
    }                                                                          \
    _Pragma("unroll") for (int u_ = 0; u_ < DOMPC_FW; ++u_) {                  \
      const int g_ = g0_ + u_ * T.nt;                                          \
      if (g_ < (n)) { BODY(u_, g_) }                                           \
    }                                                                          \
  }

struct Errs { double e_d, e_p, sum_y, obj, theta; Comp C; };
DOMPC_PHASE Errs measure(const Thr& T, const Prob& Q, const Comp* pre) {
  const KArgs& A = *Q.A;
  double v[8] = {0, 0, 0, 0, 0, 0, 0, 0};
  Comp C = pre ? *pre : Comp{-INFINITY, INFINITY, 0.0};
  if (pre) {
    double rd_[DOMPC_FW];
#define L_(u, g) rd_[u] = Q.rd[g]; if (KAPPA_D != 0.0) rd_[u] += KAPPA_D * Q.mu * one_sided(Q.lb[g], Q.ub[g]);
#define B_(u, g) if (sh_cnt(A, mk_x(A, g))) v[0] = fmax(v[0], fabs(rd_[u]));
    DOMPC_FOR4(A.n_opt_x, L_, B_)
#undef L_
#undef B_
  } else {
    double rd_[DOMPC_FW], x_[DOMPC_FW], l_[DOMPC_FW], u2_[DOMPC_FW], zl_[DOMPC_FW], zu_[DOMPC_FW];
#define L_(u, g) rd_[u] = Q.rd[g]; x_[u] = Q.x[g]; l_[u] = Q.lb[g]; u2_[u] = Q.ub[g]; zl_[u] = Q.zl[g]; zu_[u] = Q.zu[g];
#define B_(u, g)                                                                   \
    if (sh_cnt(A, mk_x(A, g))) {                                                   \
      v[0] = fmax(v[0], fabs(rd_[u] + (KAPPA_D != 0.0 ? KAPPA_D * Q.mu * one_sided(l_[u], u2_[u]) : 0.0)));  \
      if (l_[u] > -INFINITY) comp_add(C, (x_[u] - l_[u]) * zl_[u], zl_[u]);        \
      if (u2_[u] < INFINITY) comp_add(C, (u2_[u] - x_[u]) * zu_[u], zu_[u]);       \
    }
    DOMPC_FOR4(A.n_opt_x, L_, B_)
#undef L_
#undef B_
  }
  for (int g = T.tid; g < A.n_edges * NE; g += T.nt) {
    const int e = g / NE1, i = g % NE1;
    if (!sh_cnt(A, mk_e(A, e))) continue;
    const int si = e * NE1 + i;
    const double yd = Q.lam[A.edge_row0[e] + NW + NX + i];
    v[0] = fmax(v[0], fabs(-yd - Q.zsl[si] + Q.zsu[si] + (KAPPA_D != 0.0 ? KAPPA_D * Q.mu * one_sided(Q.sl[si], Q.su[si]) : 0.0)));
    if (!pre) {
      const double l = Q.sl[si], u = Q.su[si];
      if (l > -INFINITY) comp_add(C, (Q.s[si] - l) * Q.zsl[si], Q.zsl[si]);
      if (u < INFINITY) comp_add(C, (u - Q.s[si]) * Q.zsu[si], Q.zsu[si]);
    }
  }
  {
    double c_[DOMPC_FW], y_[DOMPC_FW];
#define L_(u, g) c_[u] = Q.c[g]; y_[u] = Q.lam[g];
#define B_(u, g) if (sh_cnt(A, mk_g(A, g))) { v[1] = fmax(v[1], fabs(c_[u])); v[2] += fabs(y_[u]); v[4] += fabs(c_[u]); }
    DOMPC_FOR4(A.n_g, L_, B_)
#undef L_
#undef B_
  }
  for (int e = T.tid; e < A.n_edges; e += T.nt)
    if (sh_cnt(A, mk_e(A, e))) v[3] += Q.ES(e)[ES_OBJ];
  for (int n = T.tid; n < A.n_nodes; n += T.nt)
    if (sh_cnt(A, mk_n(A, n))) v[3] += node_rterm_f(Q, n, Q.x);
  if (FREE_ROOT && T.tid == 0) v[3] += Q.ND(0)[ND_AT];
  v[5] = C.smax; v[6] = -C.smin; v[7] = C.sum_z;
  const int ops[8] = {R_MAX, R_MAX, R_SUM, R_SUM, R_SUM, R_MAX, R_MAX, R_SUM};
  wg_reduce(T, v, ops);
  Errs E;
  E.e_d = v[0]; E.e_p = v[1]; E.sum_y = v[2]; E.obj = v[3]; E.theta = v[4];
  E.C.smax = v[5]; E.C.smin = -v[6]; E.C.sum_z = v[7];
  return E;
}
```

Measured before the change: 10310.

## Pack per-node tree indices into one table and fuse multiplier-sum into trial pass

Adds a host-built node_pack table that holds each node's offsets, parent, child and row indices in one 16-int record. Device code reads that record instead of chasing several separate index arrays, and a compile flag can switch the old path back on. It also accumulates the sum of |lambda| during the trial line-search pass so measure can skip reloading lam. The gf zeroing moves out of the factor loops into init paths, and the Riccati store_val writes only the rows needed. Together these aim to cut scattered global loads and redundant memory passes per IPM iteration. The cost is extra table memory and more code paths to keep consistent.

```diff
diff --git a/__graft_entry__.py b/__graft_entry__.py
--- a/__graft_entry__.py
+++ b/__graft_entry__.py
@@ -50,6 +50,9 @@
                  ("batch_reactor", {}, "DOMPC_REG_GJ=0"), ("batch_reactor", {}, "DOMPC_GJ_U=1e9"),
                  ("industrial_poly", {}, "DOMPC_QUAD=0"), ("CSTR", {}, "DOMPC_QUAD=0"), ("CSTR", {"n_horizon": 5, "n_robust": 0}, "DOMPC_QUAD=0")]
 
+PREBUILT_NODE_PACK = [("industrial_poly", {}), ("CSTR", {})] + [("shape_family:s%d" % i, {}) for i in range(1, 10)]
+PREBUILT_BATCH_FAMILY = [("shape_family:s%d" % i, {}) for i in range(1, 10)]
+
 
 PREBUILT_SHARD = [
     ("CSTR", {}),
@@ -264,7 +267,7 @@
     print("[build] runtime:", lib)
     jobs = [(name, kw, header, h, False, False) for name, kw, header, h in lowered_models()]
     jobs += [(name, kw, header, h, True, False) for name, kw, header, h in lowered_models(PREBUILT_SHARD)]
-    jobs += [(name, kw, header, h, False, True) for name, kw, header, h in lowered_models(PREBUILT_BATCH)]
+    jobs += [(name, kw, header, h, False, True) for name, kw, header, h in lowered_models(PREBUILT_BATCH + PREBUILT_BATCH_FAMILY)]
     jobs += [(name, kw, header, h, False, True) for name, kw, header, h in lowered_mhe(PREBUILT_BATCH_MHE)]
     route = lowered_route_cases()
     jobs += [(name, kw, header, h, False, False) for name, kw, header, h, _ in route]
@@ -284,6 +287,19 @@
                 del os.environ["DOMPC_DEFS"]
             else:
                 os.environ["DOMPC_DEFS"] = saved
+    saved = os.environ.get("DOMPC_DEFS")
+    os.environ["DOMPC_DEFS"] = "DOMPC_NODE_PACK=0"
+    try:
+        jobs = [(name, kw, header, h, batch) for name, kw, header, h in lowered_models(PREBUILT_NODE_PACK) for batch in (False, True)]
+        with ThreadPoolExecutor(max_workers=max(1, min(len(jobs), (os.cpu_count() or 2) - 1))) as pool:
+            outs = list(pool.map(lambda j: nb.model_code_object(j[2], j[3], batch_only=j[4]), jobs))
+        for (name, kw, _, _, batch), co in zip(jobs, outs):
+            print(f"[build] {name} {kw} [DOMPC_NODE_PACK=0]{' (batch only)' if batch else ''}: {co}")
+    finally:
+        if saved is None:
+            del os.environ["DOMPC_DEFS"]
+        else:
+            os.environ["DOMPC_DEFS"] = saved
     from do_mpc_amd.examples import CASES
     from do_mpc_amd.simulator import Simulator
     for name in PREBUILT_PLANTS:
diff --git a/do_mpc_amd/csrc/dompc_device.hip b/do_mpc_amd/csrc/dompc_device.hip
--- a/do_mpc_amd/csrc/dompc_device.hip
+++ b/do_mpc_amd/csrc/dompc_device.hip
@@ -41,6 +41,7 @@
 #else
   out[20] = 0;
 #endif
+  out[21] = NW;
 }
 }
 
diff --git a/do_mpc_amd/csrc/dompc_driver.h b/do_mpc_amd/csrc/dompc_driver.h
--- a/do_mpc_amd/csrc/dompc_driver.h
+++ b/do_mpc_amd/csrc/dompc_driver.h
@@ -84,6 +84,7 @@
     if (sh_cnt(A, mk_x(A, g))) cnt[0] += (hl ? 1.0 : 0.0) + (hu ? 1.0 : 0.0);
   }
   for (int r = T.tid; r < A.n_g; r += T.nt) Q.lam[r] = 0.0;
+  gf_zero_edge_unknowns(T, Q);
   T.sync();
   for (int d = T.tid; d < A.n_dummy; d += T.nt) {
     const int g = A.dummy_idx[d];
@@ -347,6 +348,7 @@
   for (int g = T.tid; g < nSl; g += T.nt) { Q.st[g] = Q.s[g]; Q.zslt[g] = Q.zsl[g]; Q.zsut[g] = Q.zsu[g]; }
   T.sync();
   Comp Cp{-INFINITY, INFINITY, 0.0};
+  double Sy = 0.0;
 
   while (true) {
     bool skip_first = false;
@@ -450,7 +452,7 @@
     else a_min = gamma_alpha * gamma_theta;
     a_min = fmax(a_min, 1e-14);
     auto eval_trial = [&](double al, double az, double& obj_o, double& th_o, double& bar_o) {
-      run_eval_trial(T, Q, b, slot, al, az, mu, obj_o, th_o, bar_o, Cp);
+      run_eval_trial(T, Q, b, slot, al, az, mu, obj_o, th_o, bar_o, Cp, Sy);
       ++n_trials;
     };
     auto acceptable_ref = [&](double th_, double ph_, double al, bool& armijo_case, double theta, double phi, double dphi) -> bool {
@@ -591,7 +593,7 @@
     ++n_sweeps;
     if (EPS_GLOBAL) epsg_grad(T, Q);
     if (KAPPA_D != 0.0) Q.mu = mu;
-    c_t = prof_clock(); g_t = T.gen; E = measure(T, Q, &Cp); c_meas += prof_clock() - c_t; g_meas += T.gen - g_t;
+    c_t = prof_clock(); g_t = T.gen; E = measure(T, Q, &Cp, Sy); c_meas += prof_clock() - c_t; g_meas += T.gen - g_t;
   }
 
   if (slot & SLOT_PARITY) {
@@ -685,6 +687,7 @@
     Q.zl[g] = A.dbg_zl[g]; Q.zu[g] = A.dbg_zu[g];
   }
   for (int r = T.tid; r < A.n_g; r += T.nt) Q.lam[r] = A.dbg_lam[r];
+  gf_zero_edge_unknowns(T, Q);
   T.sync();
   newton_slack_setup(T, A, Q, A.dbg_at_solution, A.dbg_mu, false, 0.0);
   Q.sf = 1.0;
@@ -731,6 +734,7 @@
     Q.x[g] = xv; Q.lb[g] = lr; Q.ub[g] = ur; Q.zl[g] = zl; Q.zu[g] = zu;
   }
   for (int i = T.tid; i < A.n_g; i += T.nt) Q.lam[i] = lin[i];
+  gf_zero_edge_unknowns(T, Q);
   {
     const int ops[1] = {R_MAX};
     wg_reduce(T, bad, ops);
@@ -802,6 +806,7 @@
     Q.x[g] = xin[g]; Q.lb[g] = -INFINITY; Q.ub[g] = INFINITY; Q.zl[g] = 0.0; Q.zu[g] = 0.0;
   }
   for (int r = T.tid; r < A.n_g; r += T.nt) Q.lam[r] = lin[r];
+  gf_zero_edge_unknowns(T, Q);
   for (int g = T.tid; g < A.n_edges * NE; g += T.nt) {
     const int si = (g / NE1) * NE1 + g % NE1;
     Q.s[si] = 0.0; Q.sl[si] = -INFINITY; Q.su[si] = INFINITY; Q.zsl[si] = 0.0; Q.zsu[si] = 0.0; Q.sgn[si] = 1.0;
diff --git a/do_mpc_amd/csrc/dompc_edge.h b/do_mpc_amd/csrc/dompc_edge.h
--- a/do_mpc_amd/csrc/dompc_edge.h
+++ b/do_mpc_amd/csrc/dompc_edge.h
@@ -74,6 +74,40 @@
 }
 DOMPC_PHASE double eval_edge_f(const Prob& Q, int e, const double* xv, const double* sv, double* cv) { return eval_edge_f_t<false>(Q, e, xv, sv, cv, -1); }
 
+#ifndef DOMPC_NODE_PACK
+#define DOMPC_NODE_PACK 1
+#endif
+constexpr bool NODE_PACK = DOMPC_NODE_PACK != 0;
+DOMPC_DEV inline int np_of(const KArgs& A, int n, int f) { return A.node_pack[n * NP_N + f]; }
+DOMPC_DEV inline int node_xoff(const KArgs& A, int n) { return NODE_PACK ? np_of(A, n, NP_XOFF) : A.node_x_off[n]; }
+DOMPC_DEV inline int node_uoff(const KArgs& A, int n) { return NODE_PACK ? np_of(A, n, NP_UOFF) : A.node_u_off[n]; }
+DOMPC_DEV inline int node_epsoff(const KArgs& A, int n) { return NODE_PACK ? np_of(A, n, NP_EPSOFF) : A.node_eps_off[n]; }
+DOMPC_DEV inline int node_inedge(const KArgs& A, int n) { return NODE_PACK ? np_of(A, n, NP_INEDGE) : A.node_in_edge[n]; }
+DOMPC_DEV inline int node_cstart(const KArgs& A, int n) { return NODE_PACK ? np_of(A, n, NP_CHILD_START) : A.node_child_start[n]; }
+DOMPC_DEV inline int node_ccount(const KArgs& A, int n) { return NODE_PACK ? np_of(A, n, NP_CHILD_COUNT) : A.node_child_count[n]; }
+DOMPC_DEV inline int node_nurow(const KArgs& A, int n) {
+  if (NODE_PACK) return np_of(A, n, NP_NUROW);
+  const int ie = A.node_in_edge[n];
+  return ie >= 0 ? A.edge_row0[ie] + NW : 0;
+}
+DOMPC_DEV inline int node_uoff_parent(const KArgs& A, int n) {
+  if (NODE_PACK) return np_of(A, n, NP_UOFF_PARENT);
+  const int pn = A.node_parent[n];
+  return pn >= 0 ? A.node_u_off[pn] : -1;
+}
+DOMPC_DEV inline int node_child0(const KArgs& A, int n) { return NODE_PACK ? np_of(A, n, NP_CHILD0) : A.edge_child[A.node_child_start[n]]; }
+DOMPC_DEV inline int node_xoff_child0(const KArgs& A, int n) {
+  return NODE_PACK ? np_of(A, n, NP_XOFF_CHILD0) : A.node_x_off[A.edge_child[A.node_child_start[n]]];
+}
+DOMPC_DEV inline int node_row0_child0(const KArgs& A, int n) { return NODE_PACK ? np_of(A, n, NP_ROW0_CHILD0) : A.edge_row0[A.node_child_start[n]]; }
+
+DOMPC_DEV inline void gf_zero_edge_unknowns(const Thr& T, const Prob& Q) {
+  const KArgs& A = *Q.A;
+  constexpr int NW1 = NW > 0 ? NW : 1;
+  if (!DENSE_EDGE && NW > 0)
+    for (int it = T.tid; it < A.n_edges * NW; it += T.nt) Q.gf[A.edge_w_off[it / NW1] + it % NW1] = 0.0;
+}
+
 DOMPC_DEV inline const double* uprev_ptr(const Prob& Q, int n, const double* xv, double* tmp) {
   const KArgs& A = *Q.A;
   const int pn = A.node_parent[n];
@@ -83,8 +117,8 @@
 }
 DOMPC_DEV inline double node_rweight(const Prob& Q, int n) {
   const KArgs& A = *Q.A;
-  const int cc = A.node_child_count[n];
-  return cc > 0 ? cc * A.edge_omega[A.node_child_start[n]] * Q.sf : 0.0;
+  const int cc = node_ccount(A, n);
+  return cc > 0 ? cc * A.edge_omega[NODE_PACK ? np_of(A, n, NP_RW_EDGE) : A.node_child_start[n]] * Q.sf : 0.0;
 }
 DOMPC_DEV inline double node_rterm_f(const Prob& Q, int n, const double* xv) {
   const KArgs& A = *Q.A;
diff --git a/do_mpc_amd/csrc/dompc_factor.h b/do_mpc_amd/csrc/dompc_factor.h
--- a/do_mpc_amd/csrc/dompc_factor.h
+++ b/do_mpc_amd/csrc/dompc_factor.h
@@ -446,7 +446,6 @@
         t -= DOMPC_D[cx / NX + 1] * Ld[EL_T0 + R + cx % NX];
         const int gi = woff + cx;
         const double xv = vx[q][0], l = vx[q][1], u = vx[q][2], zl_ = vx[q][3], zu_ = vx[q][4];
-        Q.gf[gi] = 0.0;
         Q.rd[gi] = t - zl_ + zu_;
         Ld[EL_RW + cx] = t + bar_grad(xv, l, u, mu, !(Q.soc & 2));
         Ld[EL_BB + cx] = bar_grad(xv, l, u, 1.0);
@@ -463,7 +462,6 @@
       double xv, l, u, zl_, zu_;
       if (GS > 1) { xv = ex[0]; l = ex[1]; u = ex[2]; zl_ = ex[3]; zu_ = ex[4]; }
       else { xv = Q.x[gi]; l = Q.lb[gi]; u = Q.ub[gi]; zl_ = Q.zl[gi]; zu_ = Q.zu[gi]; }
-      Q.gf[gi] = 0.0;
       Q.rd[gi] = t - zl_ + zu_;
       Ld[EL_RW + col] = t + bar_grad(xv, l, u, mu, !(Q.soc & 2));
       Ld[EL_BB + col] = bar_grad(xv, l, u, 1.0);
@@ -882,7 +880,7 @@
 #pragma unroll
       for (int q = 0; q < G_WPL; ++q) {
         const int col = lane + q * GS;
-        if (col < NW) { Q.gf[woff + col] = 0.0; Q.rd[woff + col] = gp_x[q]; }
+        if (col < NW) Q.rd[woff + col] = gp_x[q];
       }
       if (!Q.soc) {
 #pragma unroll
diff --git a/do_mpc_amd/csrc/dompc_forward.h b/do_mpc_amd/csrc/dompc_forward.h
--- a/do_mpc_amd/csrc/dompc_forward.h
+++ b/do_mpc_amd/csrc/dompc_forward.h
@@ -62,11 +62,11 @@
 #pragma unroll
       for (int a = 0; a < NA; ++a) t += Nd[ND_K + i * NA + a] * Ld[RF_DX + a];
       Ld[RF_DV + i] = t;
-      if (i < NU) Q.dx[A.node_u_off[n] + i] = t;
-      else Q.dx[A.node_eps_off[n] + i - NU] = t;
+      if (i < NU) Q.dx[node_uoff(A, n) + i] = t;
+      else Q.dx[node_epsoff(A, n) + i - NU] = t;
     }
     T.gsync();
-    const int cs = A.node_child_start[n], cc = A.node_child_count[n];
+    const int cs = node_cstart(A, n), cc = node_ccount(A, n);
     for (int it = lane; it < cc * NA; it += GS) {
       const int e = cs + it / NA, a = it % NA, cn = A.edge_child[e];
       if (!mk_e(A, e)) continue;
@@ -78,7 +78,7 @@
         for (int b = 0; b < NX; ++b) t += S_[ES_AB + a * NA + b] * Ld[RF_DX + b];
 #pragma unroll
         for (int b = 0; b < NU; ++b) t += S_[ES_AB + a * NA + NX + b] * Ld[RF_DV + b];
-        Q.dx[A.node_x_off[cn] + a] = t;
+        Q.dx[node_xoff(A, cn) + a] = t;
       } else {
         t = Ld[RF_DV + a - NX];
       }
@@ -87,8 +87,7 @@
     T.gsync();
   };
   auto load_step = [&](int n, double (&v)[FW_PL]) {
-    const int e = A.node_child_start[n];
-    const double *Nd = Q.ND(n), *S_ = Q.ES(e), *Nc = Q.ND(A.edge_child[e]);
+    const double *Nd = Q.ND(n), *S_ = Q.ES(node_cstart(A, n)), *Nc = Q.ND(node_child0(A, n));
 #pragma unroll
     for (int q = 0; q < FW_PL; ++q) {
       const int i = lane + q * GS;
@@ -103,7 +102,7 @@
     }
   };
   auto chain_step = [&](int n, const double (&v)[FW_PL]) {
-    const int e = A.node_child_start[n], cn = A.edge_child[e];
+    const int cn = node_child0(A, n);
 #pragma unroll
     for (int q = 0; q < FW_PL; ++q) {
       const int i = lane + q * GS;
@@ -117,8 +116,8 @@
 #pragma unroll
       for (int a = 0; a < NA; ++a) t += K_[i * NA + a] * Ld[RF_DX + a];
       Ld[RF_DV + i] = t;
-      if (i < NU) Q.dx[A.node_u_off[n] + i] = t;
-      else Q.dx[A.node_eps_off[n] + i - NU] = t;
+      if (i < NU) Q.dx[node_uoff(A, n) + i] = t;
+      else Q.dx[node_epsoff(A, n) + i - NU] = t;
     }
     T.gsync();
     for (int a = lane; a < NA; a += GS) {
@@ -129,7 +128,7 @@
         for (int b = 0; b < NX; ++b) t += AB_[a * NA + b] * Ld[RF_DX + b];
 #pragma unroll
         for (int b = 0; b < NU; ++b) t += AB_[a * NA + NX + b] * Ld[RF_DV + b];
-        Q.dx[A.node_x_off[cn] + a] = t;
+        Q.dx[node_xoff_child0(A, n) + a] = t;
       } else {
         t = Ld[RF_DV + a - NX];
       }
@@ -141,7 +140,7 @@
       double t = PV_[a];
 #pragma unroll
       for (int b = 0; b < NA; ++b) t += PC_[a * NA + b] * Ld[RF_DXN + b];
-      Q.dlam[A.edge_row0[e] + NW + a] = t;
+      Q.dlam[node_row0_child0(A, n) + NW + a] = t;
     }
     for (int a = lane; a < NA; a += GS) Ld[RF_DX + a] = Ld[RF_DXN + a];
     T.gsync();
@@ -186,11 +185,22 @@
           cn_[q] = A.level_node_start[kq + 1] + scq;
           e_[q] = scq;
         }
-#pragma unroll
-        for (int q = 0; q < 4; ++q) { e_[q] += A.node_child_start[n_[q]]; n_[q] += deep ? s0 : ((q < cw && s0 + q < S) ? s0 + q : S - 1); }
-#pragma unroll
-        for (int q = 0; q < 4; ++q) {
-          uo_[q] = A.node_u_off[n_[q]]; eo_[q] = NS > 0 ? A.node_eps_off[n_[q]] : 0; xoc_[q] = A.node_x_off[cn_[q]]; row0_[q] = A.edge_row0[e_[q]];
+        if (NODE_PACK) {
+#pragma unroll
+          for (int q = 0; q < 4; ++q) n_[q] += deep ? s0 : ((q < cw && s0 + q < S) ? s0 + q : S - 1);
+#pragma unroll
+          for (int q = 0; q < 4; ++q) {
+            const auto* np = A.node_pack + n_[q] * NP_N;
+            e_[q] = np[NP_CHILD_START]; cn_[q] = np[NP_CHILD0];
+            uo_[q] = np[NP_UOFF]; eo_[q] = NS > 0 ? np[NP_EPSOFF] : 0; xoc_[q] = np[NP_XOFF_CHILD0]; row0_[q] = np[NP_ROW0_CHILD0];
+          }
+        } else {
+#pragma unroll
+          for (int q = 0; q < 4; ++q) { e_[q] += A.node_child_start[n_[q]]; n_[q] += deep ? s0 : ((q < cw && s0 + q < S) ? s0 + q : S - 1); }
+#pragma unroll
+          for (int q = 0; q < 4; ++q) {
+            uo_[q] = A.node_u_off[n_[q]]; eo_[q] = NS > 0 ? A.node_eps_off[n_[q]] : 0; xoc_[q] = A.node_x_off[cn_[q]]; row0_[q] = A.edge_row0[e_[q]];
+          }
         }
         auto pick = [&](const int (&a)[4]) { return c4 == 0 ? a[0] : (c4 == 1 ? a[1] : (c4 == 2 ? a[2] : a[3])); };
         const unsigned nd0 = (unsigned)pick(n_) * (unsigned)ND_SIZE, es0 = (unsigned)pick(e_) * (unsigned)ES_SIZE, nc0 = (unsigned)pick(cn_) * (unsigned)ND_SIZE;
diff --git a/do_mpc_amd/csrc/dompc_kargs.h b/do_mpc_amd/csrc/dompc_kargs.h
--- a/do_mpc_amd/csrc/dompc_kargs.h
+++ b/do_mpc_amd/csrc/dompc_kargs.h
@@ -6,6 +6,8 @@
 enum { WIDE_BAR_STRIDE = 64 };
 enum { EP_PARENT = 0, EP_CHILD, EP_LEVEL, EP_WOFF, EP_PIDX, EP_ROW0, EP_XOFF_PARENT, EP_UOFF_PARENT, EP_XOFF_CHILD, EP_EPSOFF_PARENT,
        EP_OMEGA_LO, EP_OMEGA_HI, EP_N = 16 };
+enum { NP_XOFF = 0, NP_UOFF, NP_EPSOFF, NP_INEDGE, NP_NUROW, NP_PARENT, NP_UOFF_PARENT, NP_CHILD_START, NP_CHILD_COUNT, NP_CHILD0,
+       NP_XOFF_CHILD0, NP_ROW0_CHILD0, NP_LEVEL, NP_RW_EDGE, NP_N = 16 };
 #if defined(DOMPC_CONSTANT_TABLES)
 typedef const __attribute__((address_space(4))) int32_t* itab_t;
 typedef const __attribute__((address_space(4))) double* dtab_t;
@@ -20,6 +22,7 @@
   dtab_t edge_omega;
   itab_t dummy_idx;
   itab_t edge_pack;
+  itab_t node_pack;
   int32_t N, n_nodes, n_edges, n_dummy, n_opt_x, n_opt_p, n_g, e_pad;
   int32_t p_off_tvp, p_off_p, p_off_uprev;
   int32_t chain_level;
diff --git a/do_mpc_amd/csrc/dompc_phases.h b/do_mpc_amd/csrc/dompc_phases.h
--- a/do_mpc_amd/csrc/dompc_phases.h
+++ b/do_mpc_amd/csrc/dompc_phases.h
@@ -75,7 +75,7 @@
   wg_reduce(T, r5, ops);
 }
 template <bool FINE>
-DOMPC_DEV inline void eval_trial_pass(const Thr& T, const Prob& Q, double al, double a_z, double mu, double& obj_o, double& th_o, double& bar_o, Comp& Cp) {
+DOMPC_DEV inline void eval_trial_pass(const Thr& T, const Prob& Q, double al, double a_z, double mu, double& obj_o, double& th_o, double& bar_o, Comp& Cp, double& Sy) {
   const KArgs& A = *Q.A;
   const int nX = A.n_opt_x, nSl = A.n_edges * NE;
   const double ks = 1e10;
@@ -141,9 +141,11 @@
   }
   {
     double y_[DOMPC_FW], dy_[DOMPC_FW];
+    double sy = 0.0;
 #define L_(u, g) y_[u] = Q.lam[g]; dy_[u] = Q.dlam[g];
-#define B_(u, g) if (mk_g(A, g)) Q.lamt[g] = y_[u] + al * dy_[u];
+#define B_(u, g) if (mk_g(A, g)) { const double yt_ = y_[u] + al * dy_[u]; Q.lamt[g] = yt_; if (sh_cnt(A, mk_g(A, g))) sy += fabs(yt_); }
     DOMPC_FOR4(A.n_g, L_, B_)
+    Sy = sy;
 #undef L_
 #undef B_
   }
@@ -175,7 +177,7 @@
 }
 struct PhaseRet { unsigned gen, nred, xseq; int rc; };
 struct PhaseRet3 { unsigned gen, nred, xseq; double v0, v1, v2; };
-struct PhaseRet6 { unsigned gen, nred, xseq; double v0, v1, v2, c0, c1, c2; };
+struct PhaseRet6 { unsigned gen, nred, xseq; double v0, v1, v2, c0, c1, c2, sy; };
 #ifndef DOMPC_HOST_EMU
 #define DOMPC_PHASE_PROLOGUE                                                        \
   const KArgs A = kernel_args(kp);                                                  \
@@ -230,15 +232,17 @@
   DOMPC_PHASE_PROLOGUE
   double o = 0.0, th = 0.0, br = 0.0;
   Comp C;
-  eval_trial_pass<false>(T, Q, ufl(al), ufl(a_z), ufl(mu), o, th, br, C);
-  return PhaseRet6{T.gen, T.nred, T.xseq, o, th, br, C.smax, C.smin, C.sum_z};
+  double sy;
+  eval_trial_pass<false>(T, Q, ufl(al), ufl(a_z), ufl(mu), o, th, br, C, sy);
+  return PhaseRet6{T.gen, T.nred, T.xseq, o, th, br, C.smax, C.smin, C.sum_z, sy};
 }
 __device__ __attribute__((noinline)) PhaseRet6 phase_eval_trial_fine(const void* kp, int b, int slot, double sf, double al, double a_z, double mu, unsigned gen, unsigned nred, unsigned xseq) {
   DOMPC_PHASE_PROLOGUE
   double o = 0.0, th = 0.0, br = 0.0;
   Comp C;
-  eval_trial_pass<true>(T, Q, ufl(al), ufl(a_z), ufl(mu), o, th, br, C);
-  return PhaseRet6{T.gen, T.nred, T.xseq, o, th, br, C.smax, C.smin, C.sum_z};
+  double sy;
+  eval_trial_pass<true>(T, Q, ufl(al), ufl(a_z), ufl(mu), o, th, br, C, sy);
+  return PhaseRet6{T.gen, T.nred, T.xseq, o, th, br, C.smax, C.smin, C.sum_z, sy};
 }
 #undef DOMPC_PHASE_PROLOGUE
 #define DOMPC_PHASE_CALL(fn, ...)                                                   \
@@ -293,15 +297,15 @@
   step_rules_pass(T, Q, mu, r5);
 #endif
 }
-DOMPC_DEV inline void run_eval_trial(const Thr& T, const Prob& Q, int b, int slot, double al, double a_z, double mu, double& obj_o, double& th_o, double& bar_o, Comp& Cp) {
-#ifndef DOMPC_HOST_EMU
-  if (fine_items(T, *Q.A)) { DOMPC_PHASE_CALL(phase_eval_trial_fine, al, a_z, mu) obj_o = ufl(r_.v0); th_o = ufl(r_.v1); bar_o = ufl(r_.v2); Cp = Comp{r_.c0, r_.c1, r_.c2}; return; }
+DOMPC_DEV inline void run_eval_trial(const Thr& T, const Prob& Q, int b, int slot, double al, double a_z, double mu, double& obj_o, double& th_o, double& bar_o, Comp& Cp, double& Sy) {
+#ifndef DOMPC_HOST_EMU
+  if (fine_items(T, *Q.A)) { DOMPC_PHASE_CALL(phase_eval_trial_fine, al, a_z, mu) obj_o = ufl(r_.v0); th_o = ufl(r_.v1); bar_o = ufl(r_.v2); Cp = Comp{r_.c0, r_.c1, r_.c2}; Sy = r_.sy; return; }
   if (DOMPC_REPEAT_PHASE & 8) { DOMPC_PHASE_CALL(phase_eval_trial, al, a_z, mu) }
   DOMPC_PHASE_CALL(phase_eval_trial, al, a_z, mu)
-  obj_o = ufl(r_.v0); th_o = ufl(r_.v1); bar_o = ufl(r_.v2); Cp = Comp{r_.c0, r_.c1, r_.c2};
-#else
-  (void)b; (void)slot;
-  if (fine_items(T, *Q.A)) eval_trial_pass<true>(T, Q, al, a_z, mu, obj_o, th_o, bar_o, Cp); else eval_trial_pass<false>(T, Q, al, a_z, mu, obj_o, th_o, bar_o, Cp);
+  obj_o = ufl(r_.v0); th_o = ufl(r_.v1); bar_o = ufl(r_.v2); Cp = Comp{r_.c0, r_.c1, r_.c2}; Sy = r_.sy;
+#else
+  (void)b; (void)slot;
+  if (fine_items(T, *Q.A)) eval_trial_pass<true>(T, Q, al, a_z, mu, obj_o, th_o, bar_o, Cp, Sy); else eval_trial_pass<false>(T, Q, al, a_z, mu, obj_o, th_o, bar_o, Cp, Sy);
 #endif
 }
 DOMPC_DEV inline void run_forward(const Thr& T, const Prob& Q, int b, int slot, double mu, double delta) {
diff --git a/do_mpc_amd/csrc/dompc_quad.h b/do_mpc_amd/csrc/dompc_quad.h
--- a/do_mpc_amd/csrc/dompc_quad.h
+++ b/do_mpc_amd/csrc/dompc_quad.h
@@ -275,7 +275,6 @@
 #pragma unroll
     for (int s = 0; s < M; ++s) {
       const int gi = pk.woff + s * NX + (int)b;
-      Q.gf[gi] = 0.0;
       Q.rd[gi] = RDv[s];
     }
     double* ew = Q.ew + (int64_t)e * EW_SIZE;
diff --git a/do_mpc_amd/csrc/dompc_riccati.h b/do_mpc_amd/csrc/dompc_riccati.h
--- a/do_mpc_amd/csrc/dompc_riccati.h
+++ b/do_mpc_amd/csrc/dompc_riccati.h
@@ -40,11 +40,11 @@
 
 DOMPC_DEV inline void node_prefetch(const Prob& Q, int n, double delta, int lane, int GS, NodePre& R) {
   const KArgs& A = *Q.A;
-  const int e = A.node_child_start[n];
+  const int e = node_cstart(A, n);
   const double* S_ = Q.ES(e);
-  const int xo = A.node_x_off[n], uo = A.node_u_off[n];
-  const int eo = NS > 0 ? A.node_eps_off[n] : -1;
-  const int ie = A.node_in_edge[n], pn = A.node_parent[n];
+  const int xo = node_xoff(A, n), uo = node_uoff(A, n);
+  const int eo = NS > 0 ? node_epsoff(A, n) : -1;
+  const int nurow = node_nurow(A, n), upo = node_uoff_parent(A, n);
   (void)delta;
 #pragma unroll
   for (int q = 0; q < RN_IPL; ++q) {
@@ -66,10 +66,10 @@
     R.pv[v][2] = Q.ub[g];
     R.pv[v][3] = Q.zl[g];
     R.pv[v][4] = Q.zu[g];
-    R.pv[v][5] = (i < NX) ? ((ie >= 0) ? Q.lam[A.edge_row0[ie] + NW + i] : Q.lam[i]) : 0.0;
+    R.pv[v][5] = (i < NX) ? Q.lam[nurow + i] : 0.0;
     const int iu = is_up ? i - NX : (i >= NA && i < NA + NU ? i - NA : 0);
     const bool hu = i >= NX && i < NA + NU;
-    R.pv[v][6] = hu ? (pn >= 0 ? Q.x[A.node_u_off[pn] + iu] : Q.P[A.p_off_uprev + iu] / DOMPC_SU[iu]) : 0.0;
+    R.pv[v][6] = hu ? (upo >= 0 ? Q.x[upo + iu] : Q.P[A.p_off_uprev + iu] / DOMPC_SU[iu]) : 0.0;
     R.pv[v][7] = 0.0;
     R.pv[v][8] = yi >= 0 ? S_[ES_QV + yi] : 0.0;
     R.pv[v][9] = 0.0;
@@ -95,7 +95,7 @@
   using namespace rb;
   const KArgs& A = *Q.A;
   double* Nd = Q.ND(n);
-  const int cs = A.node_child_start[n], cc = A.node_child_count[n];
+  const int cs = node_cstart(A, n), cc = node_ccount(A, n);
   const double rw = node_rweight(Q, n);
   const double rwh = (Q.soc & 2) ? 0.0 : rw;
   long long pc0 = prof_clock();
@@ -137,7 +137,7 @@
     } else {
       dg = sigma_of(xv, lo, hi, zlo, zhi) + delta;
       gv = bar_grad(xv, lo, hi, mu, !(Q.soc & 2));
-      if (i < NX) gv += (A.node_in_edge[n] >= 0) ? -R.pv[v][5] : R.pv[v][5];
+      if (i < NX) gv += (node_inedge(A, n) >= 0) ? -R.pv[v][5] : R.pv[v][5];
       else if (i < NA + NU) {
         if (!RT_CUSTOM) {
           dg += 2.0 * rwh * DOMPC_RTERM[i - NA];
@@ -673,9 +673,8 @@
       const int r = it % (NA * (NA + 1));
       const int i = r / (NA + 1), j = r % (NA + 1);
       double* Nd = Q.ND(n);
-      const int ie = A.node_in_edge[n];
-      const double* S_ = Q.ES(ie);
-      const int xo = A.node_x_off[n];
+      const double* S_ = Q.ES(node_inedge(A, n));
+      const int xo = node_xoff(A, n);
       if (j < NA) {
         double v = 0.0;
         if (i < NX && j < NX) {
@@ -686,7 +685,7 @@
       } else {
         double v = 0.0;
         if (i < NX)
-          v = S_[ES_MG + i] - Q.lam[A.edge_row0[ie] + NW + i] + bar_grad(Q.x[xo + i], Q.lb[xo + i], Q.ub[xo + i], mu, !(Q.soc & 2));
+          v = S_[ES_MG + i] - Q.lam[node_nurow(A, n) + i] + bar_grad(Q.x[xo + i], Q.lb[xo + i], Q.ub[xo + i], mu, !(Q.soc & 2));
         Nd[ND_PV + i] = v;
       }
     }
diff --git a/do_mpc_amd/csrc/dompc_riccati16.h b/do_mpc_amd/csrc/dompc_riccati16.h
--- a/do_mpc_amd/csrc/dompc_riccati16.h
+++ b/do_mpc_amd/csrc/dompc_riccati16.h
@@ -75,27 +75,26 @@
   }
   return V;
 }
-__device__ inline void store_val(const Prob& Q, int n, const Val& V, int lane) {
+__device__ inline void store_val(const Prob& Q, int n, const Val& V, int lane, int rows) {
   const int g = lane >> 4, j = lane & 15;
   double* Nd = Q.ND(n);
 #pragma unroll
   for (int r = 0; r < 4; ++r) {
     const int i = g + 4 * r;
-    if (i < NA && j < NA) Nd[ND_P + i * NA + j] = V[r];
-    if (i < NA && j == NA) Nd[ND_PV + i] = V[r];
+    if (i < rows && j < NA) Nd[ND_P + i * NA + j] = V[r];
+    if (i < rows && j == NA) Nd[ND_PV + i] = V[r];
   }
 }
 
 __device__ inline Val leaf(const Prob& Q, int n, double mu, double delta, int lane) {
   const KArgs& A = *Q.A;
   const int g = lane >> 4, j = lane & 15;
-  const int ie = A.node_in_edge[n];
-  const double* S_ = Q.ES(ie);
-  const int xo = A.node_x_off[n];
+  const double* S_ = Q.ES(node_inedge(A, n));
+  const int xo = node_xoff(A, n);
   const int jj = j < NX ? j : 0;
   const double xv = Q.x[xo + jj], lo = Q.lb[xo + jj], hi = Q.ub[xo + jj];
   const double dg = sigma_of(xv, lo, hi, Q.zl[xo + jj], Q.zu[xo + jj]) + delta;
-  const double gv = (j < NX) ? S_[ES_MG + jj] - Q.lam[A.edge_row0[ie] + NW + jj] + bar_grad(xv, lo, hi, mu, !(Q.soc & 2)) : 0.0;
+  const double gv = (j < NX) ? S_[ES_MG + jj] - Q.lam[node_nurow(A, n) + jj] + bar_grad(xv, lo, hi, mu, !(Q.soc & 2)) : 0.0;
   Val V = col_to_tile(gv, lane, NA, NX);
 #pragma unroll
   for (int r = 0; r < 4; ++r) {
@@ -124,17 +123,17 @@
 __device__ inline void load_node(const Prob& Q, int n, int lane, NodeIn& R) {
   const KArgs& A = *Q.A;
   const int j = lane & 15;
-  const int xo = A.node_x_off[n], uo = A.node_u_off[n];
-  const int ie = A.node_in_edge[n], pn = A.node_parent[n];
+  const int xo = node_xoff(A, n), uo = node_uoff(A, n);
+  const int upo = node_uoff_parent(A, n);
   const bool is_up = (j >= NX && j < NA);
   const int jj = j < NYT ? j : 0;
-  const int eo = NS > 0 ? A.node_eps_off[n] : 0;
+  const int eo = NS > 0 ? node_epsoff(A, n) : 0;
   const bool is_eps = NS > 0 && jj >= NA + NU;
   const int gi = (jj < NX) ? xo + jj : (is_up ? uo + (jj - NX) : (is_eps ? eo + (jj - NA - NU) : uo + (jj - NA)));
   R.xv = Q.x[gi]; R.lo = Q.lb[gi]; R.hi = Q.ub[gi]; R.zlo = Q.zl[gi]; R.zhi = Q.zu[gi];
   const int iu = is_up ? jj - NX : ((jj >= NA && !is_eps) ? jj - NA : 0);
-  R.upv = (jj >= NX && !is_eps) ? (pn >= 0 ? Q.x[A.node_u_off[pn] + iu] : Q.P[A.p_off_uprev + iu] / tab_sel(DOMPC_SU, iu)) : 0.0;
-  R.nu = (jj < NX) ? ((ie >= 0) ? Q.lam[A.edge_row0[ie] + NW + jj] : Q.lam[jj]) : 0.0;
+  R.upv = (jj >= NX && !is_eps) ? (upo >= 0 ? Q.x[upo + iu] : Q.P[A.p_off_uprev + iu] / tab_sel(DOMPC_SU, iu)) : 0.0;
+  R.nu = (jj < NX) ? Q.lam[node_nurow(A, n) + jj] : 0.0;
 }
 __device__ inline void staged_tiles(const ldsd* Ls, int lane, d4& qt, d4& F, d4& cvr, double& fu, double& qv) {
   const int g = lane >> 4, j = lane & 15;
@@ -163,10 +162,10 @@
   qv = (yjj >= 0) ? Ls[ES_QV + (yjj >= 0 ? yjj : 0)] : 0.0;
 }
 
-__device__ inline int node(const Prob& Q, int n, double mu, double delta, int lane, const NodeIn& R, const ldsd* Ls, const Val* first, Val& out) {
+__device__ inline int node(const Prob& Q, int n, double mu, double delta, int lane, const NodeIn& R, const ldsd* Ls, const Val* first, int val_rows, Val& out) {
   const KArgs& A = *Q.A;
   const int g = lane >> 4, j = lane & 15;
-  const int cs = A.node_child_start[n], cc = A.node_child_count[n];
+  const int cs = node_cstart(A, n), cc = node_ccount(A, n);
   const double rw = node_rweight(Q, n);
   const double rwh = (Q.soc & 2) ? 0.0 : rw;
   long long pc0 = prof_clock();
@@ -181,7 +180,7 @@
   R16_PN(12)
   double dg = 0.0, gv = 0.0;
   {
-    const int ie = A.node_in_edge[n];
+    const int ie = node_inedge(A, n);
     const bool is_up = (j >= NX && j < NA);
     const int jj = j < NYT ? j : 0;
     const bool is_eps = NS > 0 && jj >= NA + NU;
@@ -369,7 +368,7 @@
   if (lane == 0)
 #pragma unroll
     for (int u = 0; u < NV; ++u) Nd[ND_KV + u] = kv[u];
-  store_val(Q, n, out, lane);
+  store_val(Q, n, out, lane, val_rows);
   R16_PN(26)
 #undef R16_PN
   return bad;
@@ -388,10 +387,10 @@
     if (A.N - 1 >= cl) {
       const int n1 = A.level_node_start[A.N - 1] + s_;
       load_node(Q, n1, lane, in);
-      stage_edge(Q, A.node_child_start[n1], lane, Ld);
+      stage_edge(Q, node_cstart(A, n1), lane, Ld);
     }
     Val V = leaf(Q, A.level_node_start[A.N] + s_, mu, delta, lane);
-    store_val(Q, A.level_node_start[A.N] + s_, V, lane);
+    store_val(Q, A.level_node_start[A.N] + s_, V, lane, A.N - 1 >= cl ? NX : NA);
     staged_ready();
     for (int k = A.N - 1; k >= cl; --k) {
       NodeIn nx;
@@ -401,13 +400,13 @@
       if (k > cl) {
         const int np = A.level_node_start[k - 1] + s_;
         load_node(Q, np, lane, nx);
-        stage_edge(Q, A.node_child_start[np], lane, Ld + (buf ^ 1) * ES_STAGE);
+        stage_edge(Q, node_cstart(A, np), lane, Ld + (buf ^ 1) * ES_STAGE);
       }
 #if DOMPC_PROFILE
       if (threadIdx.x == 0) lds_prof[27] += prof_clock() - pcl;
 #endif
       Val Vn;
-      if (node(Q, A.level_node_start[k] + s_, mu, delta, lane, in, Ld + buf * ES_STAGE, &V, Vn)) { T.fset(0, FSET); break; }
+      if (node(Q, A.level_node_start[k] + s_, mu, delta, lane, in, Ld + buf * ES_STAGE, &V, k > cl ? NX : NA, Vn)) { T.fset(0, FSET); break; }
       V = Vn;
       if (k > cl) in = nx;
       buf ^= 1;
@@ -420,10 +419,10 @@
     for (int n = n0 + gid; n < n1; n += ng) {
       NodeIn in;
       load_node(Q, n, lane, in);
-      stage_edge(Q, A.node_child_start[n], lane, Ld);
+      stage_edge(Q, node_cstart(A, n), lane, Ld);
       staged_ready();
       Val Vn;
-      if (node(Q, n, mu, delta, lane, in, Ld, nullptr, Vn)) T.fset(0, FSET);
+      if (node(Q, n, mu, delta, lane, in, Ld, nullptr, NA, Vn)) T.fset(0, FSET);
     }
     T.sync();
     if ((T.fget(0) == FSET)) return 1;
diff --git a/do_mpc_amd/csrc/dompc_runtime.cpp b/do_mpc_amd/csrc/dompc_runtime.cpp
--- a/do_mpc_amd/csrc/dompc_runtime.cpp
+++ b/do_mpc_amd/csrc/dompc_runtime.cpp
@@ -339,6 +339,22 @@
       q[dompc::EP_OMEGA_LO] = (int32_t)(uint32_t)(ob & 0xffffffffll); q[dompc::EP_OMEGA_HI] = (int32_t)(uint32_t)((uint64_t)ob >> 32);
     }
     if (upload(h, &A.edge_pack, pack.data(), pack.size())) return fail(1);
+  }
+  {
+    const int32_t nw = (int32_t)info[21];
+    std::vector<int32_t> pack((size_t)d.n_nodes * dompc::NP_N, 0);
+    for (int n = 0; n < d.n_nodes; ++n) {
+      int32_t* q = pack.data() + (size_t)n * dompc::NP_N;
+      const int ie = d.node_in_edge[n], pn = d.node_parent[n], cs = d.node_child_start[n], cc = d.node_child_count[n];
+      const int c0 = cc > 0 ? d.edge_child[cs] : -1;
+      q[dompc::NP_XOFF] = d.node_x_off[n]; q[dompc::NP_UOFF] = d.node_u_off[n]; q[dompc::NP_EPSOFF] = d.node_eps_off[n];
+      q[dompc::NP_INEDGE] = ie; q[dompc::NP_NUROW] = ie >= 0 ? d.edge_row0[ie] + nw : 0;
+      q[dompc::NP_PARENT] = pn; q[dompc::NP_UOFF_PARENT] = pn >= 0 ? d.node_u_off[pn] : -1;
+      q[dompc::NP_CHILD_START] = cs; q[dompc::NP_CHILD_COUNT] = cc; q[dompc::NP_CHILD0] = c0;
+      q[dompc::NP_XOFF_CHILD0] = cc > 0 ? d.node_x_off[c0] : -1; q[dompc::NP_ROW0_CHILD0] = cc > 0 ? d.edge_row0[cs] : -1;
+      q[dompc::NP_LEVEL] = d.node_level[n]; q[dompc::NP_RW_EDGE] = cc > 0 ? cs : -1;
+    }
+    if (upload(h, &A.node_pack, pack.data(), pack.size())) return fail(1);
   }
   A.N = d.N; A.n_nodes = d.n_nodes; A.n_edges = d.n_edges; A.n_dummy = d.n_dummy;
   A.n_opt_x = d.n_opt_x; A.n_opt_p = d.n_opt_p; A.n_g = d.n_g; A.e_pad = h->e_pad;
diff --git a/do_mpc_amd/csrc/dompc_sweep.h b/do_mpc_amd/csrc/dompc_sweep.h
--- a/do_mpc_amd/csrc/dompc_sweep.h
+++ b/do_mpc_amd/csrc/dompc_sweep.h
@@ -150,8 +150,9 @@
   }
 
 struct Errs { double e_d, e_p, sum_y, obj, theta; Comp C; };
-DOMPC_PHASE Errs measure(const Thr& T, const Prob& Q, const Comp* pre) {
+DOMPC_PHASE Errs measure(const Thr& T, const Prob& Q, const Comp* pre, double pre_sy = 0.0) {
   const KArgs& A = *Q.A;
+  const bool sy_pre = pre && !sh_on(A);
   double v[8] = {0, 0, 0, 0, 0, 0, 0, 0};
   Comp C = pre ? *pre : Comp{-INFINITY, INFINITY, 0.0};
   if (pre) {
@@ -186,7 +187,15 @@
       if (u < INFINITY) comp_add(C, (u - Q.s[si]) * Q.zsu[si], Q.zsu[si]);
     }
   }
-  {
+  if (sy_pre) {
+    double c_[DOMPC_FW];
+    v[2] = pre_sy;
+#define L_(u, g) c_[u] = Q.c[g];
+#define B_(u, g) if (sh_cnt(A, mk_g(A, g))) { v[1] = fmax(v[1], fabs(c_[u])); v[4] += fabs(c_[u]); }
+    DOMPC_FOR4(A.n_g, L_, B_)
+#undef L_
+#undef B_
+  } else {
     double c_[DOMPC_FW], y_[DOMPC_FW];
 #define L_(u, g) c_[u] = Q.c[g]; y_[u] = Q.lam[g];
 #define B_(u, g) if (sh_cnt(A, mk_g(A, g))) { v[1] = fmax(v[1], fabs(c_[u])); v[2] += fabs(y_[u]); v[4] += fabs(c_[u]); }
```

Result: faster. 10460 (median of 6 runs) (+1.5%).
